# ylsung/vl-merging

Hardware: AMD Instinct MI355X
Metric: VL samples/sec (fwd+bwd) base_vl 384^2 at 1/2/4/8 GPUs; merge GB/s vs HBM peak (higher is better)
Workload: dtype bf16

## Files before the change

include/vlm_hip.h:

```cpp
#ifndef VLM_HIP_H
#define VLM_HIP_H
#include <stddef.h>
#include <stdint.h>

#ifdef __cplusplus
extern "C" {
#endif

#define VLM_OK 0
#define VLM_ERR_ARG (-1)
#define VLM_ERR_LAUNCH (-2)
#define VLM_ERR_WORKSPACE (-3)
#define VLM_ERR_UNSUPPORTED (-4)

#define VLM_ABI_VERSION 11
int vlm_abi_version(void);
int vlm_device_cus(void);
int vlm_set_cu_budget(int cus);
int vlm_debug_occupy(int workgroups, int threads, int lds_bytes, int microseconds, void* stream);

#define VLM_MERGE_LERP 0
#define VLM_MERGE_TASKVEC 1
#define VLM_MERGE_MEAN 2
#define VLM_MERGE_MAX_SRC 4
// ... 258 lines not shown

typedef struct {
  void* dst;
  const void* base;
  const void* src[VLM_MERGE_MAX_SRC];
  void* coef_out;
  double w[VLM_MERGE_MAX_SRC];
  uint64_t n_elem;
  uint32_t row_len;
  int32_t n_src;
  float lam;
  uint32_t reserved;
} vlm_sphere_job_t;

typedef struct {
  uint64_t n_jobs, n_chunks, n_tiles;
  uint64_t jobs_off;
  uint64_t chunks_off;
  uint64_t tiles_off;
  uint64_t first_off;
  uint64_t records_off;
  uint64_t results_off;
} vlm_sphere_header_t;

typedef struct {
  double sq[VLM_MERGE_MAX_SRC];
  double dot[6];
  double coef64[VLM_MERGE_MAX_SRC];
  double rho;
  double resid;
  float coef32[VLM_MERGE_MAX_SRC];
  uint32_t status;
  uint32_t reserved;
  uint64_t rows_linear;
  uint64_t rows_zero;
  double resid_max;
} vlm_sphere_result_t;

size_t vlm_sphere_plan_bytes(int n_jobs, uint64_t total_elems);
int vlm_sphere_plan_upload(const vlm_sphere_job_t* jobs_host, int n_jobs, void* workspace, size_t workspace_bytes, void* stream);
int vlm_sphere_run(void* workspace, void* stream);

#define VLM_TALL_CONSENSUS 0
#define VLM_TALL_RESTORE 1

typedef struct {
  void* dst;
  const void* base;
  const void* src[VLM_MERGE_MAX_SRC];
  void* mask[VLM_MERGE_MAX_SRC];
  uint64_t n_elem;
  int32_t n_src;
  int32_t op;
  int32_t k;
  float tall_lambda;
  float lam;
  uint32_t reserved;
} vlm_tall_job_t;

typedef struct {
  uint64_t n_jobs, n_chunks;
  uint64_t jobs_off;
  uint64_t chunks_off;
  uint64_t counters_off;
} vlm_tall_header_t;
#define VLM_TALL_COUNTERS (VLM_MERGE_MAX_SRC + 2)

size_t vlm_tall_plan_bytes(int n_jobs, uint64_t total_elems);
int vlm_tall_plan_upload(const vlm_tall_job_t* jobs_host, int n_jobs, void* workspace, size_t workspace_bytes, void* stream);
int vlm_tall_run(void* workspace, void* stream);

#define VLM_EMR_MERGE 0
#define VLM_EMR_RESTORE 1

typedef struct {
  void* dst;
  const void* base;
  const void* src[VLM_MERGE_MAX_SRC];
  void* mask[VLM_MERGE_MAX_SRC];
  uint64_t n_elem;
  int32_t n_src;
  int32_t op;
  float lam;
  float rescale;
} vlm_emr_job_t;

typedef struct {
  uint64_t n_jobs, n_chunks;
  uint64_t jobs_off;
  uint64_t chunks_off;
  uint64_t first_off;
  uint64_t records_off;
  uint64_t results_off;
} vlm_emr_header_t;
#define VLM_EMR_SUMS (3 * VLM_MERGE_MAX_SRC + 2)

typedef struct {
  double abs_sum[VLM_MERGE_MAX_SRC];
  double uni_sum[VLM_MERGE_MAX_SRC];
  uint64_t kept[VLM_MERGE_MAX_SRC];
  uint64_t zero;
  uint64_t conflict;
  float rescale[VLM_MERGE_MAX_SRC];
} vlm_emr_result_t;

size_t vlm_emr_plan_bytes(int n_jobs, uint64_t total_elems);
int vlm_emr_plan_upload(const vlm_emr_job_t* jobs_host, int n_jobs, void* workspace, size_t workspace_bytes, void* stream);
int vlm_emr_run(void* workspace, void* stream);

#define VLM_ACT_NONE 0
#define VLM_ACT_GELU 1
#define VLM_ACT_GELU_BWD 2
#define VLM_ACT_GELU_DERIV 3
#define VLM_ACT_MUL_AUX 4

typedef struct {
  const float* bias;
  const float* col_scale;
  const float* row_scale;
  const float* residual;
  int64_t ld_res;
  void* aux;
  int64_t ld_aux;
  int32_t act;
  float alpha;
  int32_t accumulate;
  int32_t reserved;
  float* col_sum;
  float* col_sum_ws;
  float* splitk_ws;
  uint64_t splitk_ws_bytes;
} vlm_epilogue_t;

int vlm_gemm_bf16(int ta, int tb, int M, int N, int K, const void* A, int lda, const void* B, int ldb, void* C,
                  int ldc, int c_is_f32, const vlm_epilogue_t* epi, void* stream);
int vlm_gemm_bf16_live(int ta, int tb, int M, int N, int K, const void* A, int lda, const void* B, int ldb, void* C,
                       int ldc, int c_is_f32, const vlm_epilogue_t* epi, const float* row_live, void* stream);
#define VLM_GEMM_MAX_GROUPS 4
typedef struct {
  int32_t row0, rows;
  const void* B;
  int32_t ldb;
  int32_t reserved;
  const float* bias;
  float* col_sum;
  float* col_sum_ws;
} vlm_gemm_group_t;
int vlm_gemm_bf16_grouped(int n_groups, const vlm_gemm_group_t* groups, int N, int K, const void* A, int lda, void* C,
                          int ldc, int c_is_f32, const vlm_epilogue_t* epi, void* stream);
typedef struct {
  int32_t row0, rows;
  float* C;
  int32_t accumulate;
  int32_t reserved;
} vlm_wgrad_group_t;
int vlm_gemm_wgrad_grouped(int n_groups, const vlm_wgrad_group_t* groups, int M, int N, const void* A, int lda,
                           const void* B, int ldb, int ldc, float* splitk_ws, uint64_t splitk_ws_bytes, void* stream);
typedef struct {
  const void* dy;
  int32_t ld_dy, M;
  const void* x;
  int32_t ld_x, N;
  float* dW;
  int32_t ldc, accumulate;
} vlm_wgrad_problem_t;
int vlm_gemm_wgrad_batch(int n, const vlm_wgrad_problem_t* problems, int T, float* splitk_ws, uint64_t splitk_ws_bytes,
                         void* stream);
int vlm_gemm_set_big_tile_mode(int mode);

int vlm_layernorm_fwd(const float* x, int ldx, int M, int D, const float* gamma, const float* beta, float eps,
                      void* y, int ldy, int y_is_f32, float* stats, void* stream);
#define VLM_ROW_WS_BYTES(D) ((size_t)1536 * 2 * (size_t)(D) * sizeof(float))
int vlm_layernorm_bwd(const void* dy, int lddy, int dy_is_f32, const float* x, int ldx, const float* stats,
                      const float* gamma, int M, int D, const float* dres, int lddres, float* dx, int lddx,
                      float* dgamma, float* dbeta, float* workspace, size_t workspace_bytes, int* deferred_blocks,
                      void* stream);
typedef struct {
  const void* y;
  int32_t ldy;
  const float* gamma;
  const float* row_scale;
  void* dy;
  int32_t lddy;
  float* dgamma;
  float* dbias;
  float* workspace;
  size_t workspace_bytes;
} vlm_layerscale_t;
int vlm_layernorm_bwd_scale(const void* dy, int lddy, int dy_is_f32, const float* x, int ldx, const float* stats,
                            const float* gamma, int M, int D, const float* dres, int lddres, float* dx, int lddx,
                            float* dgamma, float* dbeta, float* workspace, size_t workspace_bytes,
                            const vlm_layerscale_t* scale, int* deferred_blocks, void* stream);
#define VLM_MAX_FOLD_JOBS 16
typedef struct {
  const float* partials;
  int32_t nblocks;
  int32_t D;
  float* out0;
  float* out1;
} vlm_fold_job_t;
int vlm_colreduce_batch(const vlm_fold_job_t* jobs_host, int n_jobs, void* stream);
int vlm_layerscale_bwd(const float* dx, int lddx, const void* y_bf16, int ldy, const float* gamma,
                       const float* row_scale, int M, int D, void* dy_bf16, int lddy, float* dgamma, float* dbias,
                       float* workspace, size_t workspace_bytes, int* deferred_blocks, void* stream);
#define VLM_MAX_LAYERSCALE_JOBS 32
typedef struct {
  const float* weight;
  const float* gamma;
  const float* bias;
  void* shadow;
  float* bias_out;
  float* raw_w;
  float* raw_b;
  float* dweight;
  float* dbias;
  float* dgamma;
  int32_t N, K;
} vlm_layerscale_job_t;
int vlm_layerscale_fold(const vlm_layerscale_job_t* jobs_host, int n_jobs, void* stream);
int vlm_layerscale_finish(const vlm_layerscale_job_t* jobs_host, int n_jobs, void* stream);
int vlm_colsum_bf16(const void* a, int lda, int M, int N, float* out, void* stream);

int vlm_cross_entropy_fwd(const void* logits_bf16, int ld, int rows, int V, const int64_t* labels, int64_t ignore_index,
                          float* loss_rows, float* lse, void* stream);
int vlm_cross_entropy_bwd(const void* logits_bf16, int ld, int rows, int V, const int64_t* labels, int64_t ignore_index,
                          const float* lse, const float* scale_dev, void* dlogits_bf16, int ld_d, void* stream);

int vlm_l2norm_fwd(const void* x, int x_is_bf16, int ld, int rows, int D, float* y, float* inv_norm, void* stream);
int vlm_l2norm_bwd(const float* g, const float* y, const float* inv_norm, int rows, int D, void* dx, int dx_is_bf16, int ld, void* stream);
size_t vlm_contrastive_ws_floats(int n);
int vlm_contrastive(const float* all_img, const float* all_txt, int n, int B, int D, const float* log_scale, float* logits, float* out3,
                    float* d_img, float* d_txt, float* ws, void* stream);
int vlm_small_cross_entropy(const void* logits, int is_bf16, int ld, int rows, int V, const int64_t* labels, float* loss, float* dlogits,
                            void* stream);
int vlm_cross_entropy_reduce(const float* loss_rows, const int64_t* labels, int rows, int V, int64_t ignore_index, float* out2, void* stream);
int vlm_scale_by_scalar(const float* const* in, float* const* out, const int* n, int count, const float* scalar_dev, void* stream);

int vlm_text_rows_fwd(const int64_t* ids, int n, const float* word, int ld_word, const float* add0, const float* gamma, const float* beta,
                      float eps, const float* u, float p, float scale, const float* add1, float* out, int ld_out, float* stats, int D,
                      void* stream);
size_t vlm_text_rows_bwd_ws_floats(int D);
int vlm_text_rows_bwd(const float* g, int ld_g, const int64_t* ids, int n, const float* word, int ld_word, const float* add0,
                      const float* gamma, const float* stats, const float* u, float p, float scale, int D, float* d_word,
                      int64_t padding_idx, float* d_add1, float* d_beta, float* d_gamma, float* d_add0, float* ws, void* stream);
int vlm_image_rows_prep(const float* conv_bias, const float* type_row, const float* cls, int D, float* out2, void* stream);
int vlm_image_lead_rows(float* x, int ld_x, int B, int rows, int D, const float* lead, void* stream);
size_t vlm_image_rows_bwd_ws_floats(int D);
int vlm_image_rows_bwd(const float* g, int ld_g, int B, int rows, int D, void* g16, float* d_bias, float* d_type_row, float* d_cls, float* ws,
                       void* stream);
int vlm_tanh_fwd(const void* x_bf16, int ld_x, int M, int N, float* y, void* stream);
int vlm_act_bwd(const void* g, int g_is_f32, int ld_g, const void* saved, int ld_saved, int mode, int M, int N, int Np, void* dy_bf16,
                void* stream);
int vlm_colsum_small(const void* a_bf16, int lda, int M, int N, float* out, void* stream);
int vlm_sample_negatives(const float* sim_a, int a_row_stride, int a_col_stride, const float* sim_b, int b_row_stride, int b_col_stride, int B,
                         int n, const float* u, int64_t* idx, void* stream);
int vlm_weighted_sum(const float* const* terms, const float* weights, int count, float* out, void* stream);

typedef struct {
  const void* g;
  int g_is_f32;
  int ld;
  int first_row, row_step, count;
} vlm_scatter_src_t;
int vlm_scatter_rows(void* dx, int dx_is_f32, int ld_dx, int R, int D, const vlm_scatter_src_t* src, int n_src, void* stream);

int vlm_adamw_step(float* p, float* g, float* m, float* v, void* p_bf16, uint64_t n, float lr, float beta1,
                   float beta2, float eps, float weight_decay, float step_size, float grad_scale, int zero_grad,
                   void* stream);
int vlm_cast_f32_bf16(const float* src, void* dst_bf16, uint64_t n, void* stream);
int vlm_embedding_bwd(const float* gy, int ld, const int64_t* ids, int64_t n, int D, int64_t padding_idx, float* dW, int ld_w,
                      int64_t vocab, void* stream);
typedef struct {
  uint64_t src;
  uint64_t dst;
  int32_t rows, cols;
  int32_t tile_row, tile_col;
} vlm_transpose_tile_t;
int vlm_transpose_bf16_tiles(const vlm_transpose_tile_t* tiles_dev, int n_tiles, void* stream);

int vlm_droppath_rows(const float* u, float keep, int B, int n0, int n1, int base0, int base1, float* out, void* stream);
int vlm_droppath_sites(const float* u0, const float* u1, const float* keep, int n_sites, int B, int n0, int n1, int base0,
                       int base1, int rows, float* out, void* stream);
int vlm_patch_im2col(const float* image, void* patches_bf16, int B, int H, int W, int P, int lead_rows, void* stream);
int vlm_accumulate_f32_f64(const float* src, double* dst_f64, uint64_t n, void* stream);
int vlm_gram_f64(const void* x, int ldx, int M, int D, int x_is_f32, double* gram, void* stream);
int vlm_gemm_f64(int ta, int tb, int M, int N, int K, double alpha, const void* A, int lda, int a_is_f32, const double* B,
                 int ldb, double beta, double* C, int ldc, void* stream);
int vlm_scale_gram_f64(const double* src, double* dst, int n, double alpha, int accumulate, void* stream);
int vlm_cholesky_f64(double* A, int n, int* status, void* stream);
int vlm_solve_spd_right_f64(const double* chol, int n, double* rhs, int ld, int rows, void* stream);
int vlm_gemm_f64_batched(int ta, int tb, int M, int N, int K, double alpha, const void* const* A_list, int lda, int a_is_f32,
                         const double* const* B_list, int ldb, double beta, double* const* C_list, int ldc, int count, void* stream);
int vlm_cholesky_f64_batched(double* const* A_list, int count, int n, int* status, void* stream);
int vlm_solve_spd_right_f64_batched(double* const* chol_list, int n, double* const* rhs_list, int ld, int rows, int count, void* stream);

#define VLM_ISO_HEAD 64
#define VLM_ISO_MAX_STEPS 40
#define VLM_ISO_PHASE_NUCLEAR 1
#define VLM_ISO_PHASE_APPLY 2
int vlm_iso_parts(int m, int n);
int vlm_iso_delta(const float* const* c_list, const float* const* src_list, int S, int m, int n, double* const* work_list,
                  double* partials, int count, void* stream);
int vlm_iso_gram(double* const* work_list, int rows, int cols, int first, double c, double* const* Z_list, int count, void* stream);
int vlm_iso_step(double* const* work_list, int rows, int cols, int first, double p, double q, int k, double* partials, int count,
                 void* stream);
int vlm_iso_finish(double* const* work_list, const float* const* c_list, float* const* dst_list, int m, int n, double lam,
                   double* partials, int count, int phases, void* stream);

#define VLM_WUDI_HEAD 16
int vlm_wudi_parts(int m, int n);
size_t vlm_wudi_work_doubles(int m, int n);
size_t vlm_wudi_state_offset(int m, int n, int iters);
int vlm_wudi_prepare(const float* const* c_list, const float* const* src_list, int S, int m, int n, double* const* work_list,
                     double* partials, int count, void* stream);
int vlm_wudi_step(double* const* work_list, int m, int n, int t, double step, double bc2s, double beta1, double beta2, double eps,
                  double* partials, int count, void* stream);
int vlm_wudi_finish(double* const* work_list, const float* const* c_list, float* const* dst_list, int S, int m, int n, int iters,
                    double lam, double* partials, int count, void* stream);

#define VLM_SVD_HEAD 64
#define VLM_SVD_MAX_SWEEPS 30
size_t vlm_svd_work_doubles(int p, int q);
int vlm_svd_steps(int p);
int vlm_svd_reset(double* const* work_list, int p, int q, int count, void* stream);
int vlm_svd_sweep(double* const* work_list, int p, int q, int sweep, int count, void* stream);
int vlm_svd_finish(double* const* work_list, int p, int q, double floor_rel, int count, void* stream);
int vlm_tsv_delta(const float* const* c_list, const float* const* src_list, int m, int n, double* const* work_list, int count,
                  void* stream);
int vlm_tsv_gather(const double* const* src_work_list, int S, int p, int q, int k, int side, double* const* dst_work_list,
                   double* const* scat_list, int count, void* stream);
int vlm_tsv_apply(const double* const* pu_list, const double* const* pv_list, const double* const* scat_list,
                  const float* const* c_list, float* const* dst_list, double* const* t_list, int m, int n, int kS, double lam, int count,
                  void* stream);

#define VLM_ATTN_JOINT 0
#define VLM_ATTN_SEPARATE 1

typedef struct {
  const void* qkv;
  int32_t ld_qkv;
  int32_t H;
  int32_t total_rows;
  int32_t R;
  const float* bias_t;
  const int16_t* rel_index;
  const int16_t* rel_index_t;
  int32_t ld_index;
  int32_t index_rows;
  int32_t ld_index_t;
  int32_t index_t_rows;
  int32_t head_row0;
  int32_t mode;
  const uint8_t* keep0;
  const uint8_t* keep1;
  int32_t B, n0, n1, base0, base1, pos1;
  float scale;
  int32_t q_keep0;
  const void* bias_dense;
  const void* bias_dense_t;
  int32_t dense_tiles;
  int32_t q_keep1;
} vlm_attn_desc_t;

int vlm_attention_qkeep_served(const vlm_attn_desc_t* d, int with_dbias);

size_t vlm_bias_dense_bytes(int n0, int n1, int pos1, int mode);
int vlm_bias_dense(const float* bias_t, int n_cols, int R, const int16_t* index, int ld_index, int n0, int n1, int pos1,
                   int mode, int k_major, void* out_f16, void* stream);

int vlm_attention_fwd(const vlm_attn_desc_t* d, void* out_bf16, int ld_out, float* lse, void* stream);
typedef struct {
  float* dq[2];
  float* dv[2];
} vlm_attn_colsum_t;

size_t vlm_attention_bwd_ws_floats(const vlm_attn_desc_t* d, int with_dbias);
int vlm_attention_bwd(const vlm_attn_desc_t* d, const void* out_bf16, int ld_out, const void* dout_bf16, int ld_dout,
                      const float* lse, float* delta_ws, size_t ws_floats, void* dqkv_bf16, int ld_dqkv, float* dbias_t,
                      const vlm_attn_colsum_t* colsum, void* stream);
int vlm_attention_bwd_live(const vlm_attn_desc_t* d, const void* out_bf16, int ld_out, const void* dout_bf16, int ld_dout,
                           const float* lse, float* delta_ws, size_t ws_floats, void* dqkv_bf16, int ld_dqkv, float* dbias_t,
                           const vlm_attn_colsum_t* colsum, const float* row_live, void* stream);

#ifdef __cplusplus
}
#endif
#endif
```

vl-merging_amd/_lib.py:

```python
import ctypes
import os

_HERE = os.path.dirname(os.path.abspath(__file__))
LIB_PATH = os.environ.get("VLM_LIB_PATH") or os.path.join(_HERE, "lib", "libvlm_hip.so")
_lib = None

c_void_p = ctypes.c_void_p
c_int = ctypes.c_int
c_float = ctypes.c_float
c_size_t = ctypes.c_size_t
c_u64 = ctypes.c_uint64

MERGE_LERP, MERGE_TASKVEC, MERGE_MEAN = 0, 1, 2
MERGE_MAX_SRC = 4


class MergeJob(ctypes.Structure):
    _fields_ = [
        ("dst", c_void_p),
        ("base", c_void_p),
        ("src", c_void_p * MERGE_MAX_SRC),
        ("ratio", c_float * MERGE_MAX_SRC),
        ("n_src", ctypes.c_int32),
        ("mode", ctypes.c_int32),
# ... 146 lines not shown

class PairStatsJob(ctypes.Structure):
    _fields_ = [
        ("base", c_void_p),
        ("src", c_void_p * MERGE_MAX_SRC),
        ("n_elem", c_u64),
        ("tkey", ctypes.c_uint32 * MERGE_MAX_SRC),
        ("n_src", ctypes.c_int32),
        ("reserved", ctypes.c_int32),
    ]


class PairStatsHeader(ctypes.Structure):
    _fields_ = [(n, c_u64) for n in ("n_jobs", "n_chunks", "jobs_off", "chunks_off", "first_off", "records_off", "results_off")]


class PairStatsResult(ctypes.Structure):
    _fields_ = ([("sq", ctypes.c_double * MERGE_MAX_SRC)]
                + [(n, ctypes.c_double * PAIRSTATS_PAIRS) for n in ("dot", "dist2", "ssd", "tssd")]
                + [("nnz", c_u64 * MERGE_MAX_SRC)]
                + [(n, c_u64 * PAIRSTATS_PAIRS) for n in ("live", "conflict", "tlive", "tconflict")])


STOCK_SUMS = MERGE_MAX_SRC + PAIRSTATS_PAIRS


class StockJob(ctypes.Structure):
    _fields_ = [
        ("dst", c_void_p),
        ("base", c_void_p),
        ("src", c_void_p * MERGE_MAX_SRC),
        ("n_elem", c_u64),
        ("n_src", ctypes.c_int32),
        ("reserved", ctypes.c_int32),
    ]


class StockHeader(ctypes.Structure):
    _fields_ = list(PairStatsHeader._fields_)


class StockResult(ctypes.Structure):
    _fields_ = [("sq", ctypes.c_double * MERGE_MAX_SRC), ("dot", ctypes.c_double * PAIRSTATS_PAIRS),
                ("cos_pair", ctypes.c_double * PAIRSTATS_PAIRS), ("cos", ctypes.c_double), ("t", ctypes.c_double),
                ("scale", c_float), ("reserved", ctypes.c_uint32)]


EMR_MERGE, EMR_RESTORE = 0, 1
EMR_SUMS = 3 * MERGE_MAX_SRC + 2


class EmrJob(ctypes.Structure):
    _fields_ = [
        ("dst", c_void_p),
        ("base", c_void_p),
        ("src", c_void_p * MERGE_MAX_SRC),
        ("mask", c_void_p * MERGE_MAX_SRC),
        ("n_elem", c_u64),
        ("n_src", ctypes.c_int32),
        ("op", ctypes.c_int32),
        ("lam", c_float),
        ("rescale", c_float),
    ]


class EmrHeader(ctypes.Structure):
    _fields_ = list(PairStatsHeader._fields_)


class EmrResult(ctypes.Structure):
    _fields_ = [("abs_sum", ctypes.c_double * MERGE_MAX_SRC), ("uni_sum", ctypes.c_double * MERGE_MAX_SRC),
                ("kept", c_u64 * MERGE_MAX_SRC), ("zero", c_u64), ("conflict", c_u64), ("rescale", c_float * MERGE_MAX_SRC)]


SCE_COUNTERS = 3


class SceJob(ctypes.Structure):
    _fields_ = [
        ("dst", c_void_p),
        ("base", c_void_p),
        ("src", c_void_p * MERGE_MAX_SRC),
        ("k", c_u64),
        ("n_elem", c_u64),
        ("n_src", ctypes.c_int32),
        ("lam", c_float),
    ]


class SceHeader(ctypes.Structure):
    _fields_ = list(TiesHeader._fields_) + [(n, c_u64) for n in ("first_off", "records_off")]


class SceResult(ctypes.Structure):
    _fields_ = [("key", ctypes.c_uint32), ("reserved", ctypes.c_uint32), ("rank", c_u64), ("sq", ctypes.c_double * MERGE_MAX_SRC),
                ("tot", ctypes.c_double), ("w", c_float * MERGE_MAX_SRC)]


SPHERE_OK, SPHERE_LINEAR, SPHERE_ZERO = 0, 1, 2
SPHERE_ITERS = 24


class SphereJob(ctypes.Structure):
    _fields_ = [
        ("dst", c_void_p),
        ("base", c_void_p),
        ("src", c_void_p * MERGE_MAX_SRC),
        ("coef_out", c_void_p),
        ("w", ctypes.c_double * MERGE_MAX_SRC),
        ("n_elem", c_u64),
        ("row_len", ctypes.c_uint32),
        ("n_src", ctypes.c_int32),
        ("lam", c_float),
        ("reserved", ctypes.c_uint32),
    ]


class SphereHeader(ctypes.Structure):
    _fields_ = [(n, c_u64) for n in ("n_jobs", "n_chunks", "n_tiles", "jobs_off", "chunks_off", "tiles_off", "first_off",
                                     "records_off", "results_off")]


class SphereResult(ctypes.Structure):
    _fields_ = [("sq", ctypes.c_double * MERGE_MAX_SRC), ("dot", ctypes.c_double * PAIRSTATS_PAIRS),
                ("coef64", ctypes.c_double * MERGE_MAX_SRC), ("rho", ctypes.c_double), ("resid", ctypes.c_double),
                ("coef32", c_float * MERGE_MAX_SRC), ("status", ctypes.c_uint32), ("reserved", ctypes.c_uint32),
                ("rows_linear", c_u64), ("rows_zero", c_u64), ("resid_max", ctypes.c_double)]


class ScatterSrc(ctypes.Structure):
    _fields_ = [("g", c_void_p), ("g_is_f32", ctypes.c_int32), ("ld", ctypes.c_int32), ("first_row", ctypes.c_int32),
                ("row_step", ctypes.c_int32), ("count", ctypes.c_int32)]


class Epilogue(ctypes.Structure):
    _fields_ = [
        ("bias", c_void_p), ("col_scale", c_void_p), ("row_scale", c_void_p), ("residual", c_void_p),
        ("ld_res", ctypes.c_int64), ("aux", c_void_p), ("ld_aux", ctypes.c_int64), ("act", ctypes.c_int32),
        ("alpha", c_float), ("accumulate", ctypes.c_int32), ("reserved", ctypes.c_int32), ("col_sum", c_void_p),
        ("col_sum_ws", c_void_p), ("splitk_ws", c_void_p), ("splitk_ws_bytes", ctypes.c_uint64),
    ]


GEMM_MAX_GROUPS = 4


class GemmGroup(ctypes.Structure):
    _fields_ = [("row0", ctypes.c_int32), ("rows", ctypes.c_int32), ("B", c_void_p), ("ldb", ctypes.c_int32),
                ("reserved", ctypes.c_int32), ("bias", c_void_p), ("col_sum", c_void_p), ("col_sum_ws", c_void_p)]


class WgradGroup(ctypes.Structure):
    _fields_ = [("row0", ctypes.c_int32), ("rows", ctypes.c_int32), ("C", c_void_p), ("accumulate", ctypes.c_int32),
                ("reserved", ctypes.c_int32)]


class WgradProblem(ctypes.Structure):
    _fields_ = [("dy", c_void_p), ("ld_dy", ctypes.c_int32), ("M", ctypes.c_int32), ("x", c_void_p), ("ld_x", ctypes.c_int32),
                ("N", ctypes.c_int32), ("dW", c_void_p), ("ldc", ctypes.c_int32), ("accumulate", ctypes.c_int32)]


class FoldJob(ctypes.Structure):
    _fields_ = [("partials", c_void_p), ("nblocks", ctypes.c_int32), ("D", ctypes.c_int32), ("out0", c_void_p),
                ("out1", c_void_p)]


class LayerScale(ctypes.Structure):
    _fields_ = [("y", c_void_p), ("ldy", ctypes.c_int32), ("gamma", c_void_p), ("row_scale", c_void_p), ("dy", c_void_p),
                ("lddy", ctypes.c_int32), ("dgamma", c_void_p), ("dbias", c_void_p), ("workspace", c_void_p),
                ("workspace_bytes", c_size_t)]


class AttnColsum(ctypes.Structure):
    _fields_ = [("dq", c_void_p * 2), ("dv", c_void_p * 2)]


ACT_NONE, ACT_GELU, ACT_GELU_BWD, ACT_GELU_DERIV, ACT_MUL_AUX = 0, 1, 2, 3, 4
ATTN_JOINT, ATTN_SEPARATE = 0, 1


class AttnDesc(ctypes.Structure):
    _fields_ = [
        ("qkv", c_void_p), ("ld_qkv", ctypes.c_int32), ("H", ctypes.c_int32), ("total_rows", ctypes.c_int32),
        ("R", ctypes.c_int32), ("bias_t", c_void_p), ("rel_index", c_void_p), ("rel_index_t", c_void_p),
        ("ld_index", ctypes.c_int32), ("index_rows", ctypes.c_int32), ("ld_index_t", ctypes.c_int32),
        ("index_t_rows", ctypes.c_int32), ("head_row0", ctypes.c_int32), ("mode", ctypes.c_int32),
        ("keep0", c_void_p), ("keep1", c_void_p),
        ("B", ctypes.c_int32), ("n0", ctypes.c_int32), ("n1", ctypes.c_int32), ("base0", ctypes.c_int32),
        ("base1", ctypes.c_int32), ("pos1", ctypes.c_int32), ("scale", c_float), ("q_keep0", ctypes.c_int32),
        ("bias_dense", c_void_p), ("bias_dense_t", c_void_p), ("dense_tiles", ctypes.c_int32), ("q_keep1", ctypes.c_int32),
    ]


class LayerScaleJob(ctypes.Structure):
    _fields_ = [("weight", c_void_p), ("gamma", c_void_p), ("bias", c_void_p), ("shadow", c_void_p), ("bias_out", c_void_p),
                ("raw_w", c_void_p), ("raw_b", c_void_p), ("dweight", c_void_p), ("dbias", c_void_p), ("dgamma", c_void_p),
                ("N", ctypes.c_int32), ("K", ctypes.c_int32)]


MAX_LAYERSCALE_JOBS = 32


class VlmError(RuntimeError):
    pass


_ERR = {-1: "VLM_ERR_ARG", -2: "VLM_ERR_LAUNCH", -3: "VLM_ERR_WORKSPACE", -4: "VLM_ERR_UNSUPPORTED"}

SIGNATURES = {
    "vlm_abi_version": (c_int, []),
    "vlm_device_cus": (c_int, []),
    "vlm_set_cu_budget": (c_int, [c_int]),
    "vlm_debug_occupy": (c_int, [c_int, c_int, c_int, c_int, c_void_p]),
    "vlm_layerscale_fold": (c_int, [ctypes.POINTER(LayerScaleJob), c_int, c_void_p]),
    "vlm_layerscale_finish": (c_int, [ctypes.POINTER(LayerScaleJob), c_int, c_void_p]),
    "vlm_merge_plan_bytes": (c_size_t, [c_int, c_u64]),
    "vlm_merge_plan_upload": (c_int, [ctypes.POINTER(MergeJob), c_int, c_void_p, c_size_t, c_void_p]),
    "vlm_merge_run": (c_int, [c_void_p, c_void_p]),
    "vlm_ties_plan_bytes": (c_size_t, [c_int, c_u64]),
    "vlm_ties_plan_upload": (c_int, [ctypes.POINTER(TiesJob), c_int, c_void_p, c_size_t, c_void_p]),
    "vlm_ties_run": (c_int, [c_void_p, c_void_p]),
    "vlm_dare_plan_bytes": (c_size_t, [c_int, c_u64]),
    "vlm_dare_plan_upload": (c_int, [ctypes.POINTER(DareJob), c_int, c_void_p, c_size_t, c_void_p]),
    "vlm_dare_run": (c_int, [c_void_p, c_void_p]),
    "vlm_band_plan_bytes": (c_size_t, [c_int, c_u64]),
    "vlm_band_plan_upload": (c_int, [ctypes.POINTER(BandJob), c_int, c_void_p, c_size_t, c_void_p]),
    "vlm_band_run": (c_int, [c_void_p, c_void_p]),
    "vlm_della_plan_bytes": (c_size_t, [c_int, c_u64]),
    "vlm_della_plan_upload": (c_int, [ctypes.POINTER(DellaJob), c_int, c_void_p, c_size_t, c_void_p]),
    "vlm_della_run": (c_int, [c_void_p, c_void_p]),
    "vlm_pairstats_plan_bytes": (c_size_t, [c_int, c_u64]),
    "vlm_pairstats_plan_upload": (c_int, [ctypes.POINTER(PairStatsJob), c_int, c_void_p, c_size_t, c_void_p]),
    "vlm_pairstats_run": (c_int, [c_void_p, c_void_p]),
    "vlm_stock_plan_bytes": (c_size_t, [c_int, c_u64]),
    "vlm_stock_plan_upload": (c_int, [ctypes.POINTER(StockJob), c_int, c_void_p, c_size_t, c_void_p]),
    "vlm_stock_run": (c_int, [c_void_p, c_void_p]),
    "vlm_sce_plan_bytes": (c_size_t, [c_int, c_u64]),
    "vlm_sce_plan_upload": (c_int, [ctypes.POINTER(SceJob), c_int, c_void_p, c_size_t, c_void_p]),
    "vlm_sce_run": (c_int, [c_void_p, c_void_p]),
    "vlm_sphere_plan_bytes": (c_size_t, [c_int, c_u64]),
    "vlm_sphere_plan_upload": (c_int, [ctypes.POINTER(SphereJob), c_int, c_void_p, c_size_t, c_void_p]),
    "vlm_sphere_run": (c_int, [c_void_p, c_void_p]),
    "vlm_tall_plan_bytes": (c_size_t, [c_int, c_u64]),
    "vlm_tall_plan_upload": (c_int, [ctypes.POINTER(TallJob), c_int, c_void_p, c_size_t, c_void_p]),
    "vlm_tall_run": (c_int, [c_void_p, c_void_p]),
    "vlm_emr_plan_bytes": (c_size_t, [c_int, c_u64]),
    "vlm_emr_plan_upload": (c_int, [ctypes.POINTER(EmrJob), c_int, c_void_p, c_size_t, c_void_p]),
    "vlm_emr_run": (c_int, [c_void_p, c_void_p]),
    "vlm_gemm_bf16": (c_int, [c_int, c_int, c_int, c_int, c_int, c_void_p, c_int, c_void_p, c_int, c_void_p, c_int,
                              c_int, ctypes.POINTER(Epilogue), c_void_p]),
    "vlm_gemm_bf16_live": (c_int, [c_int, c_int, c_int, c_int, c_int, c_void_p, c_int, c_void_p, c_int, c_void_p, c_int,
                                   c_int, ctypes.POINTER(Epilogue), c_void_p, c_void_p]),
    "vlm_gemm_bf16_grouped": (c_int, [c_int, ctypes.POINTER(GemmGroup), c_int, c_int, c_void_p, c_int, c_void_p, c_int, c_int,
                                      ctypes.POINTER(Epilogue), c_void_p]),
    "vlm_gemm_wgrad_grouped": (c_int, [c_int, ctypes.POINTER(WgradGroup), c_int, c_int, c_void_p, c_int, c_void_p, c_int, c_int,
                                       c_void_p, c_u64, c_void_p]),
    "vlm_gemm_wgrad_batch": (c_int, [c_int, ctypes.POINTER(WgradProblem), c_int, c_void_p, c_u64, c_void_p]),
    "vlm_attention_fwd": (c_int, [ctypes.POINTER(AttnDesc), c_void_p, c_int, c_void_p, c_void_p]),
    "vlm_attention_bwd_ws_floats": (c_size_t, [ctypes.POINTER(AttnDesc), c_int]),
    "vlm_attention_qkeep_served": (c_int, [ctypes.POINTER(AttnDesc), c_int]),
    "vlm_attention_bwd": (c_int, [ctypes.POINTER(AttnDesc), c_void_p, c_int, c_void_p, c_int, c_void_p, c_void_p, c_size_t,
                                  c_void_p, c_int, c_void_p, c_void_p, c_void_p]),
    "vlm_attention_bwd_live": (c_int, [ctypes.POINTER(AttnDesc), c_void_p, c_int, c_void_p, c_int, c_void_p, c_void_p, c_size_t,
                                       c_void_p, c_int, c_void_p, c_void_p, c_void_p, c_void_p]),
    "vlm_layernorm_fwd": (c_int, [c_void_p, c_int, c_int, c_int, c_void_p, c_void_p, c_float, c_void_p, c_int, c_int,
                                  c_void_p, c_void_p]),
    "vlm_layernorm_bwd": (c_int, [c_void_p, c_int, c_int, c_void_p, c_int, c_void_p, c_void_p, c_int, c_int, c_void_p,
                                  c_int, c_void_p, c_int, c_void_p, c_void_p, c_void_p, c_size_t,
                                  ctypes.POINTER(c_int), c_void_p]),
    "vlm_layernorm_bwd_scale": (c_int, [c_void_p, c_int, c_int, c_void_p, c_int, c_void_p, c_void_p, c_int, c_int, c_void_p,
                                        c_int, c_void_p, c_int, c_void_p, c_void_p, c_void_p, c_size_t,
                                        ctypes.POINTER(LayerScale), ctypes.POINTER(c_int), c_void_p]),
    "vlm_layerscale_bwd": (c_int, [c_void_p, c_int, c_void_p, c_int, c_void_p, c_void_p, c_int, c_int, c_void_p, c_int,
                                   c_void_p, c_void_p, c_void_p, c_size_t, ctypes.POINTER(c_int), c_void_p]),
    "vlm_colreduce_batch": (c_int, [ctypes.POINTER(FoldJob), c_int, c_void_p]),
    "vlm_gemm_set_big_tile_mode": (c_int, [c_int]),
    "vlm_colsum_bf16": (c_int, [c_void_p, c_int, c_int, c_int, c_void_p, c_void_p]),
    "vlm_adamw_step": (c_int, [c_void_p, c_void_p, c_void_p, c_void_p, c_void_p, c_u64, c_float, c_float, c_float,
                               c_float, c_float, c_float, c_float, c_int, c_void_p]),
    "vlm_accumulate_f32_f64": (c_int, [c_void_p, c_void_p, c_u64, c_void_p]),
    "vlm_gram_f64": (c_int, [c_void_p, c_int, c_int, c_int, c_int, c_void_p, c_void_p]),
    "vlm_gemm_f64": (c_int, [c_int, c_int, c_int, c_int, c_int, ctypes.c_double, c_void_p, c_int, c_int, c_void_p, c_int,
                             ctypes.c_double, c_void_p, c_int, c_void_p]),
    "vlm_scale_gram_f64": (c_int, [c_void_p, c_void_p, c_int, ctypes.c_double, c_int, c_void_p]),
    "vlm_cholesky_f64": (c_int, [c_void_p, c_int, c_void_p, c_void_p]),
    "vlm_solve_spd_right_f64": (c_int, [c_void_p, c_int, c_void_p, c_int, c_int, c_void_p]),
    "vlm_gemm_f64_batched": (c_int, [c_int, c_int, c_int, c_int, c_int, ctypes.c_double, ctypes.POINTER(c_void_p), c_int, c_int,
                                     ctypes.POINTER(c_void_p), c_int, ctypes.c_double, ctypes.POINTER(c_void_p), c_int, c_int, c_void_p]),
    "vlm_cholesky_f64_batched": (c_int, [ctypes.POINTER(c_void_p), c_int, c_int, c_void_p, c_void_p]),
    "vlm_solve_spd_right_f64_batched": (c_int, [ctypes.POINTER(c_void_p), c_int, ctypes.POINTER(c_void_p), c_int, c_int, c_int, c_void_p]),
    "vlm_iso_parts": (c_int, [c_int, c_int]),
    "vlm_iso_delta": (c_int, [ctypes.POINTER(c_void_p), ctypes.POINTER(c_void_p), c_int, c_int, c_int, ctypes.POINTER(c_void_p),
                              c_void_p, c_int, c_void_p]),
    "vlm_iso_gram": (c_int, [ctypes.POINTER(c_void_p), c_int, c_int, c_int, ctypes.c_double, ctypes.POINTER(c_void_p), c_int, c_void_p]),
    "vlm_iso_step": (c_int, [ctypes.POINTER(c_void_p), c_int, c_int, c_int, ctypes.c_double, ctypes.c_double, c_int, c_void_p, c_int,
                             c_void_p]),
    "vlm_iso_finish": (c_int, [ctypes.POINTER(c_void_p), ctypes.POINTER(c_void_p), ctypes.POINTER(c_void_p), c_int, c_int,
                               ctypes.c_double, c_void_p, c_int, c_int, c_void_p]),
    "vlm_wudi_parts": (c_int, [c_int, c_int]),
    "vlm_wudi_work_doubles": (ctypes.c_size_t, [c_int, c_int]),
    "vlm_wudi_state_offset": (ctypes.c_size_t, [c_int, c_int, c_int]),
    "vlm_wudi_prepare": (c_int, [ctypes.POINTER(c_void_p), ctypes.POINTER(c_void_p), c_int, c_int, c_int, ctypes.POINTER(c_void_p),
                                 c_void_p, c_int, c_void_p]),
    "vlm_wudi_step": (c_int, [ctypes.POINTER(c_void_p), c_int, c_int, c_int, ctypes.c_double, ctypes.c_double, ctypes.c_double,
                              ctypes.c_double, ctypes.c_double, c_void_p, c_int, c_void_p]),
    "vlm_wudi_finish": (c_int, [ctypes.POINTER(c_void_p), ctypes.POINTER(c_void_p), ctypes.POINTER(c_void_p), c_int, c_int, c_int, c_int,
                                ctypes.c_double, c_void_p, c_int, c_void_p]),
    "vlm_svd_work_doubles": (ctypes.c_size_t, [c_int, c_int]),
    "vlm_svd_steps": (c_int, [c_int]),
    "vlm_svd_reset": (c_int, [ctypes.POINTER(c_void_p), c_int, c_int, c_int, c_void_p]),
    "vlm_svd_sweep": (c_int, [ctypes.POINTER(c_void_p), c_int, c_int, c_int, c_int, c_void_p]),
    "vlm_svd_finish": (c_int, [ctypes.POINTER(c_void_p), c_int, c_int, ctypes.c_double, c_int, c_void_p]),
    "vlm_tsv_delta": (c_int, [ctypes.POINTER(c_void_p), ctypes.POINTER(c_void_p), c_int, c_int, ctypes.POINTER(c_void_p), c_int, c_void_p]),
    "vlm_tsv_gather": (c_int, [ctypes.POINTER(c_void_p), c_int, c_int, c_int, c_int, c_int, ctypes.POINTER(c_void_p),
                               ctypes.POINTER(c_void_p), c_int, c_void_p]),
    "vlm_tsv_apply": (c_int, [ctypes.POINTER(c_void_p), ctypes.POINTER(c_void_p), ctypes.POINTER(c_void_p), ctypes.POINTER(c_void_p),
                              ctypes.POINTER(c_void_p), ctypes.POINTER(c_void_p), c_int, c_int, c_int, ctypes.c_double, c_int, c_void_p]),
    "vlm_cross_entropy_fwd": (c_int, [c_void_p, c_int, c_int, c_int, c_void_p, ctypes.c_int64, c_void_p, c_void_p, c_void_p]),
    "vlm_cross_entropy_bwd": (c_int, [c_void_p, c_int, c_int, c_int, c_void_p, ctypes.c_int64, c_void_p, c_void_p, c_void_p, c_int,
                                      c_void_p]),
    "vlm_l2norm_fwd": (c_int, [c_void_p, c_int, c_int, c_int, c_int, c_void_p, c_void_p, c_void_p]),
    "vlm_l2norm_bwd": (c_int, [c_void_p, c_void_p, c_void_p, c_int, c_int, c_void_p, c_int, c_int, c_void_p]),
    "vlm_contrastive_ws_floats": (c_size_t, [c_int]),
    "vlm_contrastive": (c_int, [c_void_p, c_void_p, c_int, c_int, c_int, c_void_p, c_void_p, c_void_p, c_void_p, c_void_p, c_void_p,
                                c_void_p]),
    "vlm_small_cross_entropy": (c_int, [c_void_p, c_int, c_int, c_int, c_int, c_void_p, c_void_p, c_void_p, c_void_p]),
    "vlm_cross_entropy_reduce": (c_int, [c_void_p, c_void_p, c_int, c_int, ctypes.c_int64, c_void_p, c_void_p]),
    "vlm_scale_by_scalar": (c_int, [ctypes.POINTER(c_void_p), ctypes.POINTER(c_void_p), ctypes.POINTER(c_int), c_int, c_void_p, c_void_p]),
    "vlm_text_rows_fwd": (c_int, [c_void_p, c_int, c_void_p, c_int, c_void_p, c_void_p, c_void_p, c_float, c_void_p, c_float, c_float,
                                  c_void_p, c_void_p, c_int, c_void_p, c_int, c_void_p]),
    "vlm_text_rows_bwd_ws_floats": (c_size_t, [c_int]),
    "vlm_text_rows_bwd": (c_int, [c_void_p, c_int, c_void_p, c_int, c_void_p, c_int, c_void_p, c_void_p, c_void_p, c_void_p, c_float, c_float,
                                  c_int, c_void_p, ctypes.c_int64, c_void_p, c_void_p, c_void_p, c_void_p, c_void_p, c_void_p]),
    "vlm_image_rows_prep": (c_int, [c_void_p, c_void_p, c_void_p, c_int, c_void_p, c_void_p]),
    "vlm_image_lead_rows": (c_int, [c_void_p, c_int, c_int, c_int, c_int, c_void_p, c_void_p]),
    "vlm_image_rows_bwd_ws_floats": (c_size_t, [c_int]),
    "vlm_image_rows_bwd": (c_int, [c_void_p, c_int, c_int, c_int, c_int, c_void_p, c_void_p, c_void_p, c_void_p, c_void_p, c_void_p]),
    "vlm_tanh_fwd": (c_int, [c_void_p, c_int, c_int, c_int, c_void_p, c_void_p]),
    "vlm_act_bwd": (c_int, [c_void_p, c_int, c_int, c_void_p, c_int, c_int, c_int, c_int, c_int, c_void_p, c_void_p]),
    "vlm_colsum_small": (c_int, [c_void_p, c_int, c_int, c_int, c_void_p, c_void_p]),
    "vlm_sample_negatives": (c_int, [c_void_p, c_int, c_int, c_void_p, c_int, c_int, c_int, c_int, c_void_p, c_void_p, c_void_p]),
    "vlm_weighted_sum": (c_int, [ctypes.POINTER(c_void_p), ctypes.POINTER(c_float), c_int, c_void_p, c_void_p]),
    "vlm_scatter_rows": (c_int, [c_void_p, c_int, c_int, c_int, c_int, c_void_p, c_int, c_void_p]),
    "vlm_cast_f32_bf16": (c_int, [c_void_p, c_void_p, c_u64, c_void_p]),
    "vlm_embedding_bwd": (c_int, [c_void_p, c_int, c_void_p, ctypes.c_int64, c_int, ctypes.c_int64, c_void_p, c_int,
                                  ctypes.c_int64, c_void_p]),
    "vlm_bias_dense_bytes": (c_size_t, [c_int, c_int, c_int, c_int]),
    "vlm_bias_dense": (c_int, [c_void_p, c_int, c_int, c_void_p, c_int, c_int, c_int, c_int, c_int, c_int, c_void_p,
                               c_void_p]),
    "vlm_transpose_bf16_tiles": (c_int, [c_void_p, c_int, c_void_p]),
    "vlm_droppath_sites": (c_int, [c_void_p, c_void_p, c_void_p, c_int, c_int, c_int, c_int, c_int, c_int, c_int, c_void_p,
                                   c_void_p]),
    "vlm_droppath_rows": (c_int, [c_void_p, c_float, c_int, c_int, c_int, c_int, c_int, c_void_p, c_void_p]),
    "vlm_patch_im2col": (c_int, [c_void_p, c_void_p, c_int, c_int, c_int, c_int, c_int, c_void_p]),
}


def get_lib():
    global _lib
    if _lib is None:
        if not os.path.exists(LIB_PATH):
            raise VlmError(
                f"{LIB_PATH} is missing: build it with `python -c 'import __graft_entry__ as g; g.build()'` "
                "(hipcc --offload-arch=gfx950).  There is no CPU fallback for the hot path.")
        import torch
        lib = ctypes.CDLL(LIB_PATH)
        for name, (res, args) in SIGNATURES.items():
            fn = getattr(lib, name)
            fn.restype = res
            fn.argtypes = args
        _lib = lib
    return _lib


def check(rc, what):
    if rc != 0:
        raise VlmError(f"{what} failed: {_ERR.get(rc, rc)}")


def stream_ptr():
    import torch
    return c_void_p(torch.cuda.current_stream().cuda_stream)


def ptr(t):
    return c_void_p(t.data_ptr()) if t is not None else c_void_p(0)


def require_cuda(*tensors):
    for t in tensors:
        if t is not None and not t.is_cuda:
            raise VlmError("vl_merging_amd ops run on the GPU only (tensor on %s); there is no CPU path" % t.device)
```

vl-merging_amd/csrc/elementwise.hip:

```cpp
#include "vlm_common.h"

#define EW_THREADS 256
#ifndef EW_NT
#define EW_NT true
#endif

static int ew_grid(size_t n_vec) {
  int cus = vlm_device_cus();
  if (cus <= 0) cus = 256;
  size_t want = (n_vec + EW_THREADS - 1) / EW_THREADS;
  size_t cap = (size_t)cus * 8;
  if (want < 1) want = 1;
  return (int)(want < cap ? want : cap);
}

__global__ __launch_bounds__(EW_THREADS) void adamw_kernel(float* __restrict__ p, float* __restrict__ g,
                                                           float* __restrict__ m, float* __restrict__ v,
                                                           bf16_t* __restrict__ pb, size_t n4, float lr, float b1,
                                                           float b2, float eps, float wd, float step_size,
                                                           float grad_scale, int zero_grad) {
  for (size_t i = (size_t)blockIdx.x * EW_THREADS + threadIdx.x; i < n4; i += (size_t)gridDim.x * EW_THREADS) {
    f32x4 pp = reinterpret_cast<f32x4*>(p)[i];
    f32x4 gg = EW_NT ? __builtin_nontemporal_load(reinterpret_cast<f32x4*>(g) + i) : reinterpret_cast<f32x4*>(g)[i];
    f32x4 mm = EW_NT ? __builtin_nontemporal_load(reinterpret_cast<f32x4*>(m) + i) : reinterpret_cast<f32x4*>(m)[i];
    f32x4 vv = EW_NT ? __builtin_nontemporal_load(reinterpret_cast<f32x4*>(v) + i) : reinterpret_cast<f32x4*>(v)[i];
#pragma unroll
    for (int r = 0; r < 4; ++r) {
      const float gr = gg[r] * grad_scale;
      mm[r] = b1 * mm[r] + (1.0f - b1) * gr;
      vv[r] = b2 * vv[r] + (1.0f - b2) * gr * gr;
      const float denom = sqrtf(vv[r]) + eps;
      float x = pp[r] - step_size * (mm[r] / denom);
      if (wd != 0.0f) x = x - lr * wd * x;
      pp[r] = x;
    }
    reinterpret_cast<f32x4*>(p)[i] = pp;
    if (EW_NT) {
      __builtin_nontemporal_store(mm, reinterpret_cast<f32x4*>(m) + i);
      __builtin_nontemporal_store(vv, reinterpret_cast<f32x4*>(v) + i);
    } else {
      reinterpret_cast<f32x4*>(m)[i] = mm;
      reinterpret_cast<f32x4*>(v)[i] = vv;
    }
    if (zero_grad) reinterpret_cast<f32x4*>(g)[i] = (f32x4){0.f, 0.f, 0.f, 0.f};
    if (pb) {
      bf16x4 h = {(bf16_t)pp[0], (bf16_t)pp[1], (bf16_t)pp[2], (bf16_t)pp[3]};
      reinterpret_cast<bf16x4*>(pb)[i] = h;
    }
  }
}

__global__ __launch_bounds__(EW_THREADS) void cast_kernel(const float* __restrict__ src, bf16_t* __restrict__ dst,
                                                          size_t n4) {
  for (size_t i = (size_t)blockIdx.x * EW_THREADS + threadIdx.x; i < n4; i += (size_t)gridDim.x * EW_THREADS) {
    const f32x4 s = reinterpret_cast<const f32x4*>(src)[i];
    bf16x4 h = {(bf16_t)s[0], (bf16_t)s[1], (bf16_t)s[2], (bf16_t)s[3]};
    reinterpret_cast<bf16x4*>(dst)[i] = h;
  }
}

__global__ __launch_bounds__(EW_THREADS) void im2col_kernel(const float* __restrict__ img, bf16_t* __restrict__ out,
                                                            int B, int H, int W, int P, int lead) {
  const int gh = H / P, gw = W / P;
  const int K = 3 * P * P;
  const int k8 = K / 8;
  const int rows = lead + gh * gw;
  const size_t total = (size_t)B * rows * k8;
  for (size_t i = (size_t)blockIdx.x * EW_THREADS + threadIdx.x; i < total; i += (size_t)gridDim.x * EW_THREADS) {
    const int kk = (int)(i % k8) * 8;
    const size_t rr = i / k8;
    const int r = (int)(rr % rows);
    const int b = (int)(rr / rows);
    bf16x8 h;
    if (r < lead) {
#pragma unroll
      for (int e = 0; e < 8; ++e) h[e] = (bf16_t)0.0f;
    } else {
      const int pidx = r - lead;
      const int py = pidx / gw, px = pidx % gw;
      const int c = kk / (P * P), ij = kk % (P * P);
      const int ii = ij / P, jj = ij % P;
      const float* s = img + (((size_t)b * 3 + c) * H + (py * P + ii)) * W + px * P + jj;
      const f32x4 a = *reinterpret_cast<const f32x4*>(s);
      const f32x4 c2 = *reinterpret_cast<const f32x4*>(s + 4);
      h = (bf16x8){(bf16_t)a[0], (bf16_t)a[1], (bf16_t)a[2], (bf16_t)a[3],
                   (bf16_t)c2[0], (bf16_t)c2[1], (bf16_t)c2[2], (bf16_t)c2[3]};
    }
    *reinterpret_cast<bf16x8*>(out + rr * K + kk) = h;
  }
}

__global__ __launch_bounds__(EW_THREADS) void acc_f64_kernel(const float* __restrict__ src, double* __restrict__ dst,
                                                             size_t n4) {
  for (size_t i = (size_t)blockIdx.x * EW_THREADS + threadIdx.x; i < n4; i += (size_t)gridDim.x * EW_THREADS) {
    const f32x4 s = reinterpret_cast<const f32x4*>(src)[i];
    double* d = dst + 4 * i;
    d[0] += (double)s[0];
    d[1] += (double)s[1];
    d[2] += (double)s[2];
    d[3] += (double)s[3];
  }
}

extern "C" int vlm_accumulate_f32_f64(const float* src, double* dst, uint64_t n, void* stream) {
  if (n == 0) return VLM_OK;
  if (!src || !dst || (n & 3) || ((uintptr_t)src & 15) || ((uintptr_t)dst & 31)) return VLM_ERR_ARG;
  const size_t n4 = n >> 2;
  hipLaunchKernelGGL(acc_f64_kernel, dim3(ew_grid(n4)), dim3(EW_THREADS), 0, (hipStream_t)stream, src, dst, n4);
  VLM_CHECK_LAUNCH();
  return VLM_OK;
}

extern "C" int vlm_adamw_step(float* p, float* g, float* m, float* v, void* p_bf16, uint64_t n, float lr,
                              float beta1, float beta2, float eps, float weight_decay, float step_size,
                              float grad_scale, int zero_grad, void* stream) {
  if (n == 0) return VLM_OK;
  if (!p || !g || !m || !v || (n & 3)) return VLM_ERR_ARG;
  if (((uintptr_t)p | (uintptr_t)g | (uintptr_t)m | (uintptr_t)v) & 15) return VLM_ERR_ARG;
  if (p_bf16 && ((uintptr_t)p_bf16 & 7)) return VLM_ERR_ARG;
  const size_t n4 = n >> 2;
  hipLaunchKernelGGL(adamw_kernel, dim3(ew_grid(n4)), dim3(EW_THREADS), 0, (hipStream_t)stream, p, g, m, v,
                     (bf16_t*)p_bf16, n4, lr, beta1, beta2, eps, weight_decay, step_size, grad_scale, zero_grad);
  VLM_CHECK_LAUNCH();
  return VLM_OK;
}

extern "C" int vlm_cast_f32_bf16(const float* src, void* dst, uint64_t n, void* stream) {
  if (n == 0) return VLM_OK;
  if (!src || !dst || (n & 3) || ((uintptr_t)src & 15) || ((uintptr_t)dst & 7)) return VLM_ERR_ARG;
  const size_t n4 = n >> 2;
  hipLaunchKernelGGL(cast_kernel, dim3(ew_grid(n4)), dim3(EW_THREADS), 0, (hipStream_t)stream, src, (bf16_t*)dst, n4);
  VLM_CHECK_LAUNCH();
  return VLM_OK;
}

__global__ __launch_bounds__(EW_THREADS) void embedding_bwd_kernel(const float* __restrict__ gy, int ld, const int64_t* __restrict__ ids,
                                                                   int64_t n, int D, int64_t pad, float* __restrict__ dW, int ld_w,
                                                                   int64_t vocab) {
  const int lane = threadIdx.x & 63, wave = threadIdx.x >> 6;
  for (int64_t t = (int64_t)blockIdx.x * (EW_THREADS / 64) + wave; t < n; t += (int64_t)gridDim.x * (EW_THREADS / 64)) {
    const int64_t id = ids[t];
    if (id == pad || id < 0 || id >= vocab) continue;
    const float* src = gy + t * ld;
    float* dst = dW + id * ld_w;
    for (int c = lane; c < D; c += 64) atomicAdd(dst + c, src[c]);
  }
}

extern "C" int vlm_embedding_bwd(const float* gy, int ld, const int64_t* ids, int64_t n, int D, int64_t padding_idx, float* dW,
                                 int ld_w, int64_t vocab, void* stream) {
  if (n == 0 || D == 0) return VLM_OK;
  if (!gy || !ids || !dW || n < 0 || D < 0 || ld < D || ld_w < D || vocab <= 0) return VLM_ERR_ARG;
  int64_t blocks = (n + (EW_THREADS / 64) - 1) / (EW_THREADS / 64);
  if (blocks > 4096) blocks = 4096;
  hipLaunchKernelGGL(embedding_bwd_kernel, dim3((unsigned)blocks), dim3(EW_THREADS), 0, (hipStream_t)stream, gy, ld, ids, n, D,
                     padding_idx, dW, ld_w, vocab);
  VLM_CHECK_LAUNCH();
  return VLM_OK;
}

__global__ __launch_bounds__(EW_THREADS) void droppath_rows_kernel(const float* __restrict__ u, float keep, float inv_keep,
                                                                   int B, int n0, int n1, int base0, int base1,
                                                                   float* __restrict__ out) {
  const int nt = B * n0, total = nt + B * n1;
  for (int i = blockIdx.x * EW_THREADS + threadIdx.x; i < total; i += gridDim.x * EW_THREADS) {
    int b, row;
    if (i < nt) {
      b = i / n0;
      row = base0 + i;
    } else {
      const int j = i - nt;
      b = j / n1;
      row = base1 + j;
    }
    out[row] = u[b] < keep ? inv_keep : 0.0f;
  }
}

extern "C" int vlm_droppath_rows(const float* u, float keep, int B, int n0, int n1, int base0, int base1, float* out,
                                 void* stream) {
  if (B <= 0 || n0 + n1 <= 0) return VLM_OK;
  if (!u || !out || n0 < 0 || n1 < 0 || base0 < 0 || base1 < 0 || !(keep > 0.0f) || keep > 1.0f) return VLM_ERR_ARG;
  const size_t total = (size_t)B * (n0 + n1);
  hipLaunchKernelGGL(droppath_rows_kernel, dim3(ew_grid(total)), dim3(EW_THREADS), 0, (hipStream_t)stream, u, keep,
                     1.0f / keep, B, n0, n1, base0, base1, out);
  VLM_CHECK_LAUNCH();
  return VLM_OK;
}

__global__ __launch_bounds__(EW_THREADS) void droppath_sites_kernel(const float* __restrict__ u0, const float* __restrict__ u1,
                                                                    const float* __restrict__ keep, int B, int n0, int n1,
                                                                    int base0, int base1, int rows, float* __restrict__ out) {
  const int site = blockIdx.y;
  const float kp = keep[site], inv = 1.0f / kp;
  const float* ua = u0 + (size_t)site * B;
  const float* ub = (u1 ? u1 : u0) + (size_t)site * B;
  float* o = out + (size_t)site * rows;
  const int nt = B * n0, total = nt + B * n1;
  for (int i = blockIdx.x * EW_THREADS + threadIdx.x; i < total; i += gridDim.x * EW_THREADS) {
    if (i < nt) {
      o[base0 + i] = ua[i / n0] < kp ? inv : 0.0f;
    } else {
      const int j = i - nt;
      o[base1 + j] = ub[j / n1] < kp ? inv : 0.0f;
    }
  }
}

extern "C" int vlm_droppath_sites(const float* u0, const float* u1, const float* keep, int n_sites, int B, int n0, int n1,
                                  int base0, int base1, int rows, float* out, void* stream) {
  if (n_sites <= 0 || B <= 0 || n0 + n1 <= 0) return VLM_OK;
  if (!u0 || !keep || !out || n0 < 0 || n1 < 0 || base0 < 0 || base1 < 0 || rows < base0 + B * n0 || rows < base1 + B * n1)
    return VLM_ERR_ARG;
  const size_t total = (size_t)B * (n0 + n1);
  int gx = (int)((total + EW_THREADS - 1) / EW_THREADS);
  if (gx > 64) gx = 64;
  hipLaunchKernelGGL(droppath_sites_kernel, dim3(gx, n_sites), dim3(EW_THREADS), 0, (hipStream_t)stream, u0, u1, keep, B,
                     n0, n1, base0, base1, rows, out);
  VLM_CHECK_LAUNCH();
  return VLM_OK;
}

__global__ __launch_bounds__(256) void transpose_tiles_kernel(const vlm_transpose_tile_t* __restrict__ tiles, int n_tiles) {
  __shared__ bf16_t tile[64][66];
  for (int t = blockIdx.x; t < n_tiles; t += gridDim.x) {
    const vlm_transpose_tile_t j = tiles[t];
    const bf16_t* src = reinterpret_cast<const bf16_t*>(j.src);
    bf16_t* dst = reinterpret_cast<bf16_t*>(j.dst);
    const int r0 = j.tile_row * 64, c0 = j.tile_col * 64;
    const int lr = threadIdx.x >> 2, lc = (threadIdx.x & 3) * 16;
    const bool fast = r0 + 64 <= j.rows && c0 + 64 <= j.cols && (j.cols & 7) == 0 && (j.rows & 7) == 0 &&
                      ((j.src | j.dst) & 15) == 0;
    if (fast) {
      const bf16x8* sp = reinterpret_cast<const bf16x8*>(src + (size_t)(r0 + lr) * j.cols + c0 + lc);
      const bf16x8 v0 = sp[0], v1 = sp[1];
#pragma unroll
      for (int e = 0; e < 8; ++e) {
        tile[lr][lc + e] = v0[e];
        tile[lr][lc + 8 + e] = v1[e];
      }
    } else {
      const int r = r0 + lr;
#pragma unroll
      for (int e = 0; e < 16; ++e) {
        const int c = c0 + lc + e;
        tile[lr][lc + e] = (r < j.rows && c < j.cols) ? src[(size_t)r * j.cols + c] : (bf16_t)0.0f;
      }
    }
    __syncthreads();
    const int c = c0 + lr;
    if (fast) {
      bf16x8 o0, o1;
#pragma unroll
      for (int e = 0; e < 8; ++e) {
        o0[e] = tile[lc + e][lr];
        o1[e] = tile[lc + 8 + e][lr];
      }
      bf16x8* dp = reinterpret_cast<bf16x8*>(dst + (size_t)c * j.rows + r0 + lc);
      dp[0] = o0;
      dp[1] = o1;
    } else if (c < j.cols) {
#pragma unroll
      for (int e = 0; e < 16; ++e) {
        const int r = r0 + lc + e;
        if (r < j.rows) dst[(size_t)c * j.rows + r] = tile[lc + e][lr];
      }
    }
    __syncthreads();
  }
}

extern "C" int vlm_transpose_bf16_tiles(const vlm_transpose_tile_t* tiles_dev, int n_tiles, void* stream) {
  if (n_tiles == 0) return VLM_OK;
  if (!tiles_dev || n_tiles < 0) return VLM_ERR_ARG;
  int cus = vlm_device_cus();
  if (cus <= 0) cus = 256;
  const int grid = n_tiles < cus * 16 ? n_tiles : cus * 16;
  hipLaunchKernelGGL(transpose_tiles_kernel, dim3(grid), dim3(256), 0, (hipStream_t)stream, tiles_dev, n_tiles);
  VLM_CHECK_LAUNCH();
  return VLM_OK;
}

extern "C" int vlm_patch_im2col(const float* image, void* patches, int B, int H, int W, int P, int lead_rows,
                                void* stream) {
  if (B == 0) return VLM_OK;
  if (!image || !patches || B < 0 || P <= 0 || (P & 7) || (H % P) || (W % P) || (W & 3) || lead_rows < 0)
    return VLM_ERR_ARG;
  if (((uintptr_t)image & 15) || ((uintptr_t)patches & 15)) return VLM_ERR_ARG;
  const size_t total = (size_t)B * (lead_rows + (H / P) * (W / P)) * (3 * P * P / 8);
  hipLaunchKernelGGL(im2col_kernel, dim3(ew_grid(total)), dim3(EW_THREADS), 0, (hipStream_t)stream, image,
                     (bf16_t*)patches, B, H, W, P, lead_rows);
  VLM_CHECK_LAUNCH();
  return VLM_OK;
}
```

vl-merging_amd/csrc/gemm.hip:

```cpp
#include "vlm_common.h"
#include "vlm_diag.h"
#include "wgrad_plan.h"
#include <atomic>

#define GEMM_BM 128
#define GEMM_BN 128
#define GEMM_BK 64
#define GEMM_THREADS 256
#define GEMM_TILE_BYTES (GEMM_BM * GEMM_BK * 2)

typedef __attribute__((address_space(3))) s16x4 lds_s16x4;

__device__ __forceinline__ float gelu_cdf(float x, float& ez2) {
  const float t = __builtin_amdgcn_rcpf(fmaf(0.3275911f * 0.70710678118654752440f, fabsf(x), 1.0f));
  ez2 = __builtin_amdgcn_exp2f((x * x) * (-0.5f * 1.4426950408889634f));
  float poly = fmaf(t, 0.5f * 1.061405429f, 0.5f * -1.453152027f);
  poly = fmaf(t, poly, 0.5f * 1.421413741f);
  poly = fmaf(t, poly, 0.5f * -0.284496736f);
  poly = fmaf(t, poly, 0.5f * 0.254829592f);
  const float e = fmaf(-(poly * t), ez2, 0.5f);
  return 0.5f + copysignf(e, x);
}
__device__ __forceinline__ float gelu_erf(float x) {
  float ez2;
  return x * gelu_cdf(x, ez2);
}
__device__ __forceinline__ float gelu_erf_grad(float x) {
  float ez2;
  const float cdf = gelu_cdf(x, ez2);
  return fmaf(x * 0.39894228040143267794f, ez2, cdf);
}
__device__ __forceinline__ float gelu_erf_both(float x, float& deriv) {
  float ez2;
  const float cdf = gelu_cdf(x, ez2);
  deriv = fmaf(x * 0.39894228040143267794f, ez2, cdf);
  return x * cdf;
}
__device__ __forceinline__ float act_bwd_factor(int act, float saved) {
  return act == VLM_ACT_MUL_AUX ? saved : gelu_erf_grad(saved);
}

template <bool KSTRIDED>
__device__ __forceinline__ void stage_load(u32x4 (&r)[4], __amdgpu_buffer_rsrc_t rsrc, uint32_t row0, uint32_t k0,
                                           uint32_t ld, int tid) {
#pragma unroll
  for (int u = 0; u < 4; ++u) {
    const uint32_t p = tid + 256 * u;
    uint32_t off;
    if (!KSTRIDED) {
      const uint32_t row = p >> 3, chunk = p & 7;
      off = ((row0 + row) * ld + k0 + chunk * 8) * 2;
    } else {
      const uint32_t krow = p >> 4, c16 = p & 15;
      off = ((k0 + krow) * ld + row0 + c16 * 8) * 2;
    }
    r[u] = __builtin_amdgcn_raw_buffer_load_b128(rsrc, off, 0, 0);
  }
}

template <bool KSTRIDED>
__device__ __forceinline__ void stage_store(const u32x4 (&r)[4], unsigned char* lds, int tid) {
#pragma unroll
  for (int u = 0; u < 4; ++u) {
    const uint32_t p = tid + 256 * u;
    uint32_t byte;
    if (!KSTRIDED) {
      const uint32_t row = p >> 3, chunk = p & 7;
      byte = row * 128 + ((chunk ^ (row & 7)) << 4);
    } else {
      const uint32_t krow = p >> 4, c16 = p & 15;
      const uint32_t c32 = (c16 >> 1) ^ (krow & 3) ^ (((krow >> 3) & 1) << 2);
      byte = krow * 256 + c32 * 32 + (c16 & 1) * 16;
    }
    *reinterpret_cast<u32x4*>(lds + byte) = r[u];
  }
}

typedef __attribute__((address_space(3))) void lds_void;
__device__ __forceinline__ void stage_dma(__amdgpu_buffer_rsrc_t rsrc, unsigned char* tile, uint32_t row0, uint32_t k0,
                                          uint32_t ld, int wave, int lane) {
#pragma unroll
  for (int u = 0; u < 4; ++u) {
    const int j = wave + 4 * u;
    const uint32_t row = j * 8 + (lane >> 3), chunk = (lane & 7) ^ (row & 7);
    const uint32_t off = ((row0 + row) * ld + k0 + chunk * 8) * 2;
    __builtin_amdgcn_raw_ptr_buffer_load_lds(rsrc, (lds_void*)(tile + j * 1024), 16, off, 0, 0, 0);
  }
}

template <bool KSTRIDED>
__device__ __forceinline__ bf16x8 frag_load(const unsigned char* lds, int xblk , int ksub,
                                            int lane) {
  if (!KSTRIDED) {
    const uint32_t row = xblk * 16 + (lane & 15);
    const uint32_t chunk = ksub * 4 + (lane >> 4);
    const uint32_t byte = row * 128 + ((chunk ^ (row & 7)) << 4);
    return *reinterpret_cast<const bf16x8*>(lds + byte);
  } else {
    const uint32_t g = lane >> 4, q = (lane & 15) >> 2, p = lane & 3;
    const uint32_t row = ksub * 32 + 8 * g + q;
    const uint32_t c32 = ((uint32_t)xblk ^ q ^ ((g & 1) << 2));
    const uint32_t byte = row * 256 + c32 * 32 + 8 * p;
    s16x4 lo = __builtin_amdgcn_ds_read_tr16_b64_v4i16((lds_s16x4*)(lds + byte));
    s16x4 hi = __builtin_amdgcn_ds_read_tr16_b64_v4i16((lds_s16x4*)(lds + byte + 4 * 256));
    s16x8 v = {lo[0], lo[1], lo[2], lo[3], hi[0], hi[1], hi[2], hi[3]};
    return __builtin_bit_cast(bf16x8, v);
  }
}

struct gemm_group_t {
  const void* B;
  const float* bias;
  float* col_sum;
  float* col_sum_ws;
  int ldb, row0, row_end, tile0;
};

struct gemmT_group_t {
  const void* A;
  const void* B;
  int lda, ldb, M, N, tiles_n, ntile;
  int row0, row_end, item0, kps;
  uint32_t ws_base;
};

struct gemm_params_t {
  const void* A;
  const void* B;
  void* C;
  int M, N, K;
  int lda, ldb, ldc;
  vlm_epilogue_t epi;
  int tiles_m, tiles_n;
  int group_m;
  int splits, ksteps_per_split;
  int n_groups;
  gemm_group_t grp[VLM_GEMM_MAX_GROUPS];
  gemmT_group_t grpT[VLM_GEMM_MAX_GROUPS];
  const float* row_live = nullptr;
  VLM_DIAG_GEMM_FIELD
};

__device__ __forceinline__ void lane16_swap(float& x, float& y) {
  asm volatile("s_nop 1\n\tv_permlane16_swap_b32 %0, %1" : "+v"(x), "+v"(y));
}

template <bool OUT_F32, bool LEAN = false>
__device__ __forceinline__ int gemm_epilogue(const gemm_params_t& p, const f32x4 (&acc)[4][4], int mw0, int nw0, int lane,
                                             float* red = nullptr, int red_off = 0) {
  const vlm_epilogue_t& e = p.epi;
  const bool vec_ok = ((p.ldc & 3) == 0) && (!e.aux || (e.ld_aux & 3) == 0) && (!e.residual || (e.ld_res & 3) == 0);
  const bool vec8_ok = vec_ok && (OUT_F32 || (p.ldc & 7) == 0) && (!e.aux || ((e.ld_aux & 7) == 0 && ((uintptr_t)e.aux & 15) == 0)) &&
                       (!e.residual || ((uintptr_t)e.residual & 15) == 0) && (!e.bias || ((uintptr_t)e.bias & 15) == 0) &&
                       (!e.col_scale || ((uintptr_t)e.col_scale & 15) == 0);
  if (vec8_ok && mw0 + 64 <= p.M && nw0 + 64 <= p.N) {
    const bool has_res = e.residual != nullptr, bwd = e.act == VLM_ACT_GELU_BWD || e.act == VLM_ACT_MUL_AUX, accum = OUT_F32 && e.accumulate;
    const int g = lane >> 4;
    const int nl = nw0 + (g & 1) * 16 + (g >> 1) * 8;
    float bia[2][8], gam[2][8], csum[2][8];
#pragma unroll
    for (int jp = 0; jp < 2; ++jp)
#pragma unroll
      for (int r = 0; r < 8; ++r) csum[jp][r] = 0.f;
#define EPI_LOAD_COL_VECTORS()                                                                                          \
  _Pragma("unroll") for (int jp = 0; jp < 2; ++jp) _Pragma("unroll") for (int q = 0; q < 2; ++q) {                    \
    const f32x4 b4 = e.bias ? *reinterpret_cast<const f32x4*>(e.bias + nl + jp * 32 + q * 4) : (f32x4){0.f, 0.f, 0.f, 0.f}; \
    const f32x4 g4 =                                                                                                    \
        e.col_scale ? *reinterpret_cast<const f32x4*>(e.col_scale + nl + jp * 32 + q * 4) : (f32x4){1.f, 1.f, 1.f, 1.f}; \
    _Pragma("unroll") for (int r = 0; r < 4; ++r) {                                                                     \
      bia[jp][q * 4 + r] = b4[r];                                                                                       \
      gam[jp][q * 4 + r] = g4[r];                                                                                       \
    }                                                                                                                   \
  }
    if (!LEAN) { EPI_LOAD_COL_VECTORS() }
#pragma unroll
    for (int hf = 0; hf < 4; ++hf) {
      f32x4 rsd[1][2][2], old[1][2][2];
      bf16x8 hx[1][2];
      float rs[1];
      if (LEAN) { EPI_LOAD_COL_VECTORS() }
#pragma unroll
      for (int ii = 0; ii < 1; ++ii) {
        const size_t m = mw0 + (hf + ii) * 16 + (lane & 15);
        rs[ii] = e.row_scale ? e.row_scale[m] : 1.0f;
#pragma unroll
        for (int jp = 0; jp < 2; ++jp) {
          const int n = nl + jp * 32;
          if (has_res) {
            rsd[ii][jp][0] = *reinterpret_cast<const f32x4*>(e.residual + m * e.ld_res + n);
            rsd[ii][jp][1] = *reinterpret_cast<const f32x4*>(e.residual + m * e.ld_res + n + 4);
          }
          if (bwd) hx[ii][jp] = *reinterpret_cast<const bf16x8*>(reinterpret_cast<const bf16_t*>(e.aux) + m * e.ld_aux + n);
          if (accum) {
            old[ii][jp][0] = *reinterpret_cast<const f32x4*>(reinterpret_cast<const float*>(p.C) + m * p.ldc + n);
            old[ii][jp][1] = *reinterpret_cast<const f32x4*>(reinterpret_cast<const float*>(p.C) + m * p.ldc + n + 4);
          }
        }
      }
#pragma unroll
      for (int ii = 0; ii < 1; ++ii) {
        const size_t m = mw0 + (hf + ii) * 16 + (lane & 15);
#pragma unroll
        for (int jp = 0; jp < 2; ++jp) {
          const int n = nl + jp * 32;
          float v[8];
#pragma unroll
          for (int r = 0; r < 4; ++r) {
            float x = acc[hf + ii][2 * jp][r] * e.alpha, y = acc[hf + ii][2 * jp + 1][r] * e.alpha;
            lane16_swap(x, y);
            v[r] = x;
            v[4 + r] = y;
          }
#pragma unroll
          for (int r = 0; r < 8; ++r) v[r] += bia[jp][r];
          if (bwd) {
#pragma unroll
            for (int r = 0; r < 8; ++r) v[r] *= act_bwd_factor(e.act, (float)hx[ii][jp][r]);
          } else if (e.act == VLM_ACT_GELU_DERIV) {
            bf16x8 h;
#pragma unroll
            for (int r = 0; r < 8; ++r) {
              float dg;
              v[r] = gelu_erf_both(v[r], dg);
              h[r] = (bf16_t)dg;
            }
            *reinterpret_cast<bf16x8*>(reinterpret_cast<bf16_t*>(e.aux) + m * e.ld_aux + n) = h;
          } else {
            if (e.aux) {
              bf16x8 h;
#pragma unroll
              for (int r = 0; r < 8; ++r) h[r] = (bf16_t)v[r];
              *reinterpret_cast<bf16x8*>(reinterpret_cast<bf16_t*>(e.aux) + m * e.ld_aux + n) = h;
            }
            if (e.act == VLM_ACT_GELU) {
#pragma unroll
              for (int r = 0; r < 8; ++r) v[r] = gelu_erf(v[r]);
            }
          }
          if (e.col_scale) {
#pragma unroll
            for (int r = 0; r < 8; ++r) v[r] *= gam[jp][r];
          }
          if (e.row_scale) {
#pragma unroll
            for (int r = 0; r < 8; ++r) v[r] *= rs[ii];
          }
          if (has_res) {
#pragma unroll
            for (int r = 0; r < 8; ++r) v[r] += rsd[ii][jp][r >> 2][r & 3];
          }
          if (OUT_F32 && accum) {
#pragma unroll
            for (int r = 0; r < 8; ++r) v[r] += old[ii][jp][r >> 2][r & 3];
          }
          if (!LEAN && e.col_sum) {
#pragma unroll
            for (int r = 0; r < 8; ++r) csum[jp][r] += v[r];
          }
          if (OUT_F32) {
            float* c = reinterpret_cast<float*>(p.C) + m * p.ldc + n;
            *reinterpret_cast<f32x4*>(c) = (f32x4){v[0], v[1], v[2], v[3]};
            *reinterpret_cast<f32x4*>(c + 4) = (f32x4){v[4], v[5], v[6], v[7]};
          } else {
            bf16x8 o;
#pragma unroll
            for (int r = 0; r < 8; ++r) o[r] = (bf16_t)v[r];
            *reinterpret_cast<bf16x8*>(reinterpret_cast<bf16_t*>(p.C) + m * p.ldc + n) = o;
          }
        }
      }
    }
    if (!LEAN && e.col_sum) {
#pragma unroll
      for (int jp = 0; jp < 2; ++jp)
#pragma unroll
        for (int r = 0; r < 8; ++r) {
// ... 554 lines not shown
      acc01[i][j] = (f32x4){0.f, 0.f, 0.f, 0.f};
      acc10[i][j] = (f32x4){0.f, 0.f, 0.f, 0.f};
      acc11[i][j] = (f32x4){0.f, 0.f, 0.f, 0.f};
    }

#define BIG_PIN_ACC()                                                                                   \
  _Pragma("unroll") for (int i = 0; i < 4; ++i) _Pragma("unroll") for (int j = 0; j < 4; ++j) {         \
    asm volatile("" : "+a"(acc00[i][j]), "+a"(acc01[i][j]), "+a"(acc10[i][j]), "+a"(acc11[i][j]));      \
  }
  constexpr bool DEEP = AUX == 2 && !RES;
  constexpr int AHEAD = 6;
  if constexpr (DEEP) { BIG_PIN_ACC() }

  const int nk = p.K / BIG_BK;
  const uint32_t mw0 = m0 + wm * 128, nw0 = n0 + wn * 128;
  unsigned char* const wl = epl + wave * EPIL_WAVE_BYTES;
#define EPIL_SETUP()                                       \
  big_epilogue_t<OUT_F32, RES, AUX> ep(p, wl, mw0, nw0, lane); \
  epil_in_t inA, inB;                                      \
  ep.load_inputs(inA, 0);
  bf16x8 fa0[8], fb0[8], fa1[8], fb1[8];

#define BIG_READ(FA, FB, SA, SB)                                                         \
  _Pragma("unroll") for (int i = 0; i < 8; ++i) {                                        \
    FA[i] = *reinterpret_cast<const bf16x8*>((SA) + rda + i * 1024);                     \
    FB[i] = *reinterpret_cast<const bf16x8*>((SB) + rdb + i * 1024);                     \
  }
#define BIG_MFMA_Q(ACC, FA, FB, I0, J0)                                                                                \
  _Pragma("unroll") for (int i = 0; i < 4; ++i) _Pragma("unroll") for (int j = 0; j < 4; ++j)                         \
      ACC[i][j] = __builtin_amdgcn_mfma_f32_16x16x32_bf16(FB[(J0) + j], FA[(I0) + i], ACC[i][j], 0, 0, 0);
#define BIG_MFMA(FA, FB)        \
  BIG_MFMA_Q(acc00, FA, FB, 0, 0) \
  BIG_MFMA_Q(acc01, FA, FB, 0, 4) \
  BIG_MFMA_Q(acc11, FA, FB, 4, 4) \
  BIG_MFMA_Q(acc10, FA, FB, 4, 0)
  uint32_t wr_off[4];
  {
    const uint32_t slot = (lane & 3) ^ big_swz(lane >> 4);
#pragma unroll
    for (int u = 0; u < 4; ++u) wr_off[u] = ((wave + 4 * u) * 16 + (lane >> 2)) * 64 + slot * 16;
  }
  {
    const uint32_t unswz = (((lane & 3) ^ big_swz(lane >> 4)) - (lane & 3)) * 16;
#pragma unroll
    for (int u = 0; u < 4; ++u) { offa[u] -= unswz; offb[u] -= unswz; }
  }
  u32x4 ra0[4], rb0[4], ra1[4], rb1[4];
#define BIG_GLOAD(RA_, RB_, S)                                                                        \
  _Pragma("unroll") for (int u = 0; u < 4; ++u) {                                                     \
    RA_[u] = __builtin_amdgcn_raw_buffer_load_b128(ra, offa[u], (S) * (BIG_BK * 2), 0);               \
    RB_[u] = __builtin_amdgcn_raw_buffer_load_b128(rb, offb[u], (S) * (BIG_BK * 2), 0);               \
  }
#define BIG_LWRITE(RA_, RB_, SA, SB)                                                                  \
  _Pragma("unroll") for (int u = 0; u < 4; ++u) {                                                     \
    *reinterpret_cast<u32x4*>((SA) + wr_off[u]) = RA_[u];                                             \
    *reinterpret_cast<u32x4*>((SB) + wr_off[u]) = RB_[u];                                             \
  }
#define BIG_STEP(K, GL, WR, RD, FCA, FCB, FNA, FNB, RSA, RSB, BUFA_W, BUFB_W, BUFA_R, BUFB_R)   \
  {                                                                                      \
    if (RD) {                                                                            \
      asm volatile("s_waitcnt lgkmcnt(0)" ::: "memory");                                 \
      __builtin_amdgcn_s_barrier();                                                      \
    }                                                                                    \
    __builtin_amdgcn_sched_barrier(0);                                                   \
    if (WR) { BIG_LWRITE(RSA, RSB, BUFA_W, BUFB_W) }                                     \
    if (GL) { BIG_GLOAD(RSA, RSB, (K) + 4) }                                             \
    if (RD) { BIG_READ(FNA, FNB, BUFA_R, BUFB_R) }                                       \
    BIG_MFMA(FCA, FCB)                                                                   \
    _Pragma("unroll") for (int g = 0; g < 16; ++g) {                                     \
      __builtin_amdgcn_sched_group_barrier(0x008, 2, 0);                                 \
      __builtin_amdgcn_sched_group_barrier(0x100, 1, 0);                                 \
    }                                                                                    \
    _Pragma("unroll") for (int g = 0; g < 8; ++g) {                                      \
      __builtin_amdgcn_sched_group_barrier(0x008, 2, 0);                                 \
      __builtin_amdgcn_sched_group_barrier(0x200, 1, 0);                                 \
      __builtin_amdgcn_sched_group_barrier(0x008, 2, 0);                                 \
      __builtin_amdgcn_sched_group_barrier(0x020, 1, 0);                                 \
    }                                                                                    \
    __builtin_amdgcn_sched_barrier(0);                                                   \
  }

  BIG_GLOAD(ra0, rb0, 0)
  BIG_GLOAD(ra1, rb1, 1)
  if (SKIPS && p.row_live && __builtin_amdgcn_ballot_w64(lv[0] != 0.0f || lv[1] != 0.0f || lv[2] != 0.0f || lv[3] != 0.0f) == 0) {
    int lane_d = lane;
    asm volatile("" : "+v"(lane_d));
    big_epilogue_t<OUT_F32, RES, AUX> ep(p, wl, mw0, nw0, lane_d);
    unsigned char* const wz = wl + (lane_d & 15) * EPIL_PITCH + (lane_d >> 4) * 16;
#pragma unroll
    for (int j = 0; j < 8; ++j) *reinterpret_cast<f32x4*>(wz + 64 * j) = (f32x4){0.f, 0.f, 0.f, 0.f};
#pragma unroll 1
    for (int i = 0; i < 8; ++i) {
      epil_in_t in;
      ep.load_inputs(in, i);
      ep.process(in, i, 0);
    }
    ep.finish(lane_d, (p.epi.col_sum_ws && mw0 + 128 <= (uint32_t)p.M) ? p.epi.col_sum_ws + ((size_t)(tm_ws * 2 + wm) * 2) * p.N : nullptr);
    GEMM_STAMP_END()
    return;
  }
  BIG_LWRITE(ra0, rb0, sA0, sB0)
  BIG_GLOAD(ra0, rb0, 2)
  BIG_LWRITE(ra1, rb1, sA1, sB1)
  BIG_GLOAD(ra1, rb1, 3)
  asm volatile("s_waitcnt lgkmcnt(0)" ::: "memory");
  __builtin_amdgcn_s_barrier();
  BIG_READ(fa0, fb0, sA0, sB0)
  GEMM_STAMP(1)

  int kt = 0;
  for (; kt < nk - 4; kt += 2) {
    BIG_STEP(kt + 0, 1, 1, 1, fa0, fb0, fa1, fb1, ra0, rb0, sA0, sB0, sA1, sB1)
    BIG_STEP(kt + 1, 1, 1, 1, fa1, fb1, fa0, fb0, ra1, rb1, sA1, sB1, sA0, sB0)
  }
#define BIG_TAIL_STEPS()                                                               \
  BIG_STEP(kt + 0, 0, 1, 1, fa0, fb0, fa1, fb1, ra0, rb0, sA0, sB0, sA1, sB1)          \
  BIG_STEP(kt + 1, 0, 1, 1, fa1, fb1, fa0, fb0, ra1, rb1, sA1, sB1, sA0, sB0)          \
  BIG_STEP(kt + 2, 0, 0, 1, fa0, fb0, fa1, fb1, ra0, rb0, sA0, sB0, sA1, sB1)          \
  BIG_STEP(kt + 3, 0, 0, 0, fa1, fb1, fa0, fb0, ra1, rb1, sA1, sB1, sA0, sB0)
  if constexpr (DEEP) {
    BIG_TAIL_STEPS()
    GEMM_STAMP(2)
    big_epilogue_t<OUT_F32, RES, AUX> ep(p, wl, mw0, nw0, lane);
    float* ws_row = (p.epi.col_sum_ws && mw0 + 128 <= (uint32_t)p.M) ? p.epi.col_sum_ws + ((size_t)(tm_ws * 2 + wm) * 2) * p.N : nullptr;
    BIG_EPILOGUE_LOOP_DEEP(AHEAD)
    ep.finish(lane, ws_row);
  } else {
    EPIL_SETUP()
    BIG_TAIL_STEPS()
    GEMM_STAMP(2)
    float* ws_row = (p.epi.col_sum_ws && mw0 + 128 <= (uint32_t)p.M) ? p.epi.col_sum_ws + ((size_t)(tm_ws * 2 + wm) * 2) * p.N : nullptr;
    BIG_EPILOGUE_LOOP()
    ep.finish(lane, ws_row);
  }
  GEMM_STAMP_END()
}

template <bool GROUPED = false>
__global__ __launch_bounds__(GEMM_THREADS, 1) void vlm_gemm_bigT_kernel(const gemm_params_t p) {
  __shared__ __attribute__((aligned(1024))) unsigned char sA0[BIG_OP_BYTES], sA1[BIG_OP_BYTES], sB0[BIG_OP_BYTES], sB1[BIG_OP_BYTES];
  __shared__ __attribute__((aligned(16))) unsigned char epl[4 * EPIL_WAVE_BYTES];
  const int tid = threadIdx.x;
  const int lane = tid & 63;
  const int wave = __builtin_amdgcn_readfirstlane(tid >> 6);
  const int wm = wave >> 1, wn = wave & 1;
  uint32_t ntile = p.tiles_m * p.tiles_n, tiles_n = (uint32_t)p.tiles_n;
  const uint32_t q8 = gridDim.x >> 3, r8 = gridDim.x & 7, xcd = blockIdx.x & 7;
  uint32_t item = (xcd < r8 ? xcd * (q8 + 1) : r8 * (q8 + 1) + (xcd - r8) * q8) + (blockIdx.x >> 3);
  uint32_t k_base = 0, k_end = (uint32_t)p.K, ws_base = 0;
  int nk = p.ksteps_per_split;
  const void *A = p.A, *B = p.B;
  uint32_t lda = (uint32_t)p.lda, ldb = (uint32_t)p.ldb;
  int M = p.M, N = p.N;
  if constexpr (GROUPED) {
    int g = 0;
#pragma unroll
    for (int i = 1; i < VLM_GEMM_MAX_GROUPS; ++i)
      if (i < p.n_groups && item >= (uint32_t)p.grpT[i].item0) g = i;
    const gemmT_group_t G = p.grpT[g];
    item -= (uint32_t)G.item0;
    k_base = (uint32_t)G.row0;
    k_end = (uint32_t)G.row_end;
    nk = G.kps;
    ws_base = G.ws_base;
    A = G.A; B = G.B;
    lda = (uint32_t)G.lda; ldb = (uint32_t)G.ldb;
    M = G.M; N = G.N;
    ntile = (uint32_t)G.ntile; tiles_n = (uint32_t)G.tiles_n;
  }
  const uint32_t split = item / ntile, tile = item - split * ntile;
  const uint32_t tm = tile / tiles_n, tn = tile - tm * tiles_n;
  const uint32_t m0 = tm * BIG_BM, n0 = tn * BIG_BN;
  const uint32_t k_first = k_base + split * (uint32_t)nk * BIG_BK;
  const __amdgpu_buffer_rsrc_t ra =
      __builtin_amdgcn_make_buffer_rsrc(const_cast<void*>(A), 0, (int)((uint64_t)k_end * lda * 2), 0x00020000);
  const __amdgpu_buffer_rsrc_t rb =
      __builtin_amdgcn_make_buffer_rsrc(const_cast<void*>(B), 0, (int)((uint64_t)k_end * ldb * 2), 0x00020000);

  uint32_t offa[4], offb[4], wr_off[4];
#pragma unroll
  for (int u = 0; u < 4; ++u) {
    const uint32_t row = 2 * (wave + 4 * u) + (lane >> 5), c16 = lane & 31;
    offa[u] = ((k_first + row) * lda + m0 + c16 * 8) * 2;
    offb[u] = ((k_first + row) * ldb + n0 + c16 * 8) * 2;
    wr_off[u] = row * 512 + (((c16 >> 1) ^ ((row & 3) | (((row >> 3) & 1) << 2))) << 5) + (c16 & 1) * 16;
  }
  uint32_t rda[8], rdb[8];
  {
    const uint32_t g = lane >> 4, q = (lane & 15) >> 2, pp = lane & 3, sw = q | ((g & 1) << 2);
#pragma unroll
    for (int i = 0; i < 8; ++i) {
      rda[i] = (8 * g + q) * 512 + wm * 256 + ((i ^ sw) << 5) + 8 * pp;
      rdb[i] = (8 * g + q) * 512 + wn * 256 + ((i ^ sw) << 5) + 8 * pp;
    }
  }
  f32x4 acc00[4][4], acc01[4][4], acc10[4][4], acc11[4][4];
#pragma unroll
  for (int i = 0; i < 4; ++i)
#pragma unroll
    for (int j = 0; j < 4; ++j) {
      acc00[i][j] = (f32x4){0.f, 0.f, 0.f, 0.f};
      acc01[i][j] = (f32x4){0.f, 0.f, 0.f, 0.f};
      acc10[i][j] = (f32x4){0.f, 0.f, 0.f, 0.f};
      acc11[i][j] = (f32x4){0.f, 0.f, 0.f, 0.f};
    }
  const uint32_t stepa = BIG_BK * lda * 2, stepb = BIG_BK * ldb * 2;
  bf16x8 fa0[8], fb0[8], fa1[8], fb1[8];
  u32x4 ra0[4], rb0[4], ra1[4], rb1[4];
#define BIGT_TR(PTR) __builtin_amdgcn_ds_read_tr16_b64_v4i16((lds_s16x4*)(PTR))
#define BIGT_READ(FA, FB, SA, SB)                                                                    \
  _Pragma("unroll") for (int i = 0; i < 8; ++i) {                                                    \
    const s16x4 al = BIGT_TR((SA) + rda[i]), ah = BIGT_TR((SA) + rda[i] + 4 * 512);                  \
    const s16x4 bl = BIGT_TR((SB) + rdb[i]), bh = BIGT_TR((SB) + rdb[i] + 4 * 512);                  \
    FA[i] = __builtin_bit_cast(bf16x8, (s16x8){al[0], al[1], al[2], al[3], ah[0], ah[1], ah[2], ah[3]}); \
    FB[i] = __builtin_bit_cast(bf16x8, (s16x8){bl[0], bl[1], bl[2], bl[3], bh[0], bh[1], bh[2], bh[3]}); \
  }
#define BIGT_GLOAD(RA_, RB_, S)                                                                      \
  _Pragma("unroll") for (int u = 0; u < 4; ++u) {                                                    \
    RA_[u] = __builtin_amdgcn_raw_buffer_load_b128(ra, offa[u], (S) * stepa, 0);                     \
    RB_[u] = __builtin_amdgcn_raw_buffer_load_b128(rb, offb[u], (S) * stepb, 0);                     \
  }
#define BIGT_LWRITE(RA_, RB_, SA, SB)                                                                \
  _Pragma("unroll") for (int u = 0; u < 4; ++u) {                                                    \
    *reinterpret_cast<u32x4*>((SA) + wr_off[u]) = RA_[u];                                            \
    *reinterpret_cast<u32x4*>((SB) + wr_off[u]) = RB_[u];                                            \
  }
#define BIGT_STEP(K, GL, WR, RD, FCA, FCB, FNA, FNB, RSA, RSB, BUFA_W, BUFB_W, BUFA_R, BUFB_R)      \
  {                                                                                      \
    if (RD) {                                                                            \
      asm volatile("s_waitcnt lgkmcnt(0)" ::: "memory");                                 \
      __builtin_amdgcn_s_barrier();                                                      \
    }                                                                                    \
    __builtin_amdgcn_sched_barrier(0);                                                   \
    if (WR) { BIGT_LWRITE(RSA, RSB, BUFA_W, BUFB_W) }                                    \
    if (GL) { BIGT_GLOAD(RSA, RSB, (K) + 4) }                                            \
    if (RD) { BIGT_READ(FNA, FNB, BUFA_R, BUFB_R) }                                      \
    BIG_MFMA(FCA, FCB)                                                                   \
    _Pragma("unroll") for (int g = 0; g < 32; ++g) {                                     \
      __builtin_amdgcn_sched_group_barrier(0x008, 1, 0);                                 \
      __builtin_amdgcn_sched_group_barrier(0x100, 1, 0);                                 \
    }                                                                                    \
    _Pragma("unroll") for (int g = 0; g < 8; ++g) {                                      \
      __builtin_amdgcn_sched_group_barrier(0x008, 2, 0);                                 \
      __builtin_amdgcn_sched_group_barrier(0x200, 1, 0);                                 \
      __builtin_amdgcn_sched_group_barrier(0x008, 2, 0);                                 \
      __builtin_amdgcn_sched_group_barrier(0x020, 1, 0);                                 \
    }                                                                                    \
    __builtin_amdgcn_sched_barrier(0);                                                   \
  }
  BIGT_GLOAD(ra0, rb0, 0)
  BIGT_GLOAD(ra1, rb1, 1)
  BIGT_LWRITE(ra0, rb0, sA0, sB0)
  BIGT_GLOAD(ra0, rb0, 2)
  BIGT_LWRITE(ra1, rb1, sA1, sB1)
  BIGT_GLOAD(ra1, rb1, 3)
  asm volatile("s_waitcnt lgkmcnt(0)" ::: "memory");
  __builtin_amdgcn_s_barrier();
  BIGT_READ(fa0, fb0, sA0, sB0)
  int kt = 0;
  for (; kt < nk - 4; kt += 2) {
    BIGT_STEP(kt + 0, 1, 1, 1, fa0, fb0, fa1, fb1, ra0, rb0, sA0, sB0, sA1, sB1)
    BIGT_STEP(kt + 1, 1, 1, 1, fa1, fb1, fa0, fb0, ra1, rb1, sA1, sB1, sA0, sB0)
  }
  BIGT_STEP(kt + 0, 0, 1, 1, fa0, fb0, fa1, fb1, ra0, rb0, sA0, sB0, sA1, sB1)
  BIGT_STEP(kt + 1, 0, 1, 1, fa1, fb1, fa0, fb0, ra1, rb1, sA1, sB1, sA0, sB0)
  BIGT_STEP(kt + 2, 0, 0, 1, fa0, fb0, fa1, fb1, ra0, rb0, sA0, sB0, sA1, sB1)
  BIGT_STEP(kt + 3, 0, 0, 0, fa1, fb1, fa0, fb0, ra1, rb1, sA1, sB1, sA0, sB0)

  gemm_params_t pl = p;
  pl.C = reinterpret_cast<float*>(p.C) + ws_base + (size_t)split * M * N;
  pl.M = M;
  pl.N = N;
  pl.ldc = N;
  const uint32_t mw0 = m0 + wm * 128, nw0 = n0 + wn * 128;
  unsigned char* const wl = epl + wave * EPIL_WAVE_BYTES;
  big_epilogue_t<true, false, 0, 128, 0, true> ep(pl, wl, mw0, nw0, lane);
  epil_in_t inA, inB;
  ep.load_inputs(inA, 0);
  BIG_EPILOGUE_LOOP()
}

__global__ __launch_bounds__(256) void splitk_reduce_kernel(const float* __restrict__ ws, int splits, int M, int N, float* __restrict__ C,
                                                            int ldc, int accumulate) {
  const size_t i = (size_t)blockIdx.x * 256 + threadIdx.x, per = (size_t)M * N / 4;
  if (i >= per) return;
  const size_t e = i * 4, m = e / N, n = e - m * N;
  f32x4 t = accumulate ? *reinterpret_cast<const f32x4*>(C + m * ldc + n) : (f32x4){0.f, 0.f, 0.f, 0.f};
  for (int s = 0; s < splits; ++s) t += *reinterpret_cast<const f32x4*>(ws + (size_t)s * M * N + e);
  *reinterpret_cast<f32x4*>(C + m * ldc + n) = t;
}

struct splitk_groups_t {
  float* C[VLM_GEMM_MAX_GROUPS];
  int M[VLM_GEMM_MAX_GROUPS], N[VLM_GEMM_MAX_GROUPS], ldc[VLM_GEMM_MAX_GROUPS];
  uint32_t ws_base[VLM_GEMM_MAX_GROUPS];
  int splits[VLM_GEMM_MAX_GROUPS], accumulate[VLM_GEMM_MAX_GROUPS];
};
__global__ __launch_bounds__(256) void splitk_reduce_grouped_kernel(const float* __restrict__ ws, const splitk_groups_t g) {
  const int gi = blockIdx.y;
  const int N = g.N[gi], ldc = g.ldc[gi];
  const size_t i = (size_t)blockIdx.x * 256 + threadIdx.x, mn = (size_t)g.M[gi] * N;
  if (i >= mn / 4) return;
  float* const C = g.C[gi];
  const float* const w = ws + g.ws_base[gi];
  const size_t e = i * 4, m = e / N, n = e - m * N;
  f32x4 t = g.accumulate[gi] ? *reinterpret_cast<const f32x4*>(C + m * ldc + n) : (f32x4){0.f, 0.f, 0.f, 0.f};
  for (int s = 0; s < g.splits[gi]; ++s) t += *reinterpret_cast<const f32x4*>(w + (size_t)s * mn + e);
  *reinterpret_cast<f32x4*>(C + m * ldc + n) = t;
}

static int plan_cus() {
  const int cus = vlm_device_cus();
  return cus > 0 ? cus : 256;
}

static bool epi_vec8(const vlm_epilogue_t* e, int ldc, int c_is_f32) {
  const bool v4 = ((ldc & 3) == 0) && (!e->aux || (e->ld_aux & 3) == 0) && (!e->residual || (e->ld_res & 3) == 0);
  return v4 && (c_is_f32 || (ldc & 7) == 0) && (!e->aux || ((e->ld_aux & 7) == 0 && ((uintptr_t)e->aux & 15) == 0)) &&
         (!e->residual || ((uintptr_t)e->residual & 15) == 0) && (!e->bias || ((uintptr_t)e->bias & 15) == 0) &&
         (!e->col_scale || ((uintptr_t)e->col_scale & 15) == 0);
}

static bool epi_off32(const vlm_epilogue_t* e, int M, int lda, int ldc) {
  return (uint64_t)M * ldc * 4 < (1ull << 31) && (!e->residual || (uint64_t)M * e->ld_res * 4 < (1ull << 31)) &&
         (!e->aux || (uint64_t)M * e->ld_aux * 2 < (1ull << 31)) && (uint64_t)M * lda * 2 < (1ull << 31);
}

static int launch_gemm_bigT(gemm_params_t p, const vlm_epilogue_t* epi, hipStream_t stream) {
  if (!epi->splitk_ws || (p.N % BIG_BN) || (p.ldc % 4)) return 1;
  if ((uint64_t)p.M * p.N * 4 >= (1ull << 31)) return 1;
  p.tiles_m = (p.M + BIG_BM - 1) / BIG_BM;
  p.tiles_n = (p.N + BIG_BN - 1) / BIG_BN;
  const int ntile = p.tiles_m * p.tiles_n, nk = (p.K + BIG_BK - 1) / BIG_BK;
  int splits = plan_cus() / ntile;
  if (splits < 1) splits = 1;
  if (splits > nk / 16) splits = nk / 16;
  if (splits < 1) return 1;
  int kps = (nk + splits - 1) / splits;
  kps += kps & 1;
  if (kps < 4) kps = 4;
  splits = (nk + kps - 1) / kps;
  if ((size_t)splits * p.M * p.N * 4 > (size_t)epi->splitk_ws_bytes) return 1;
  p.ksteps_per_split = kps;
  p.splits = splits;
  float* const out = reinterpret_cast<float*>(p.C);
  const int ldc = p.ldc;
  p.C = epi->splitk_ws;
  hipLaunchKernelGGL(vlm_gemm_bigT_kernel<false>, dim3(ntile * splits), dim3(GEMM_THREADS), 0, stream, p);
  VLM_CHECK_LAUNCH();
  const size_t per = (size_t)p.M * p.N / 4;
  hipLaunchKernelGGL(splitk_reduce_kernel, dim3((unsigned)((per + 255) / 256)), dim3(256), 0, stream,
                     reinterpret_cast<const float*>(epi->splitk_ws), splits, p.M, p.N, out, ldc, epi->accumulate);
  VLM_CHECK_LAUNCH();
  return VLM_OK;
}

template <bool OUT_F32, bool RES, int AUX, bool GROUPED = false>
static int launch_gemm_big(gemm_params_t p, hipStream_t stream) {
  if (!GROUPED) p.tiles_m = (p.M + BIG_BM - 1) / BIG_BM;
  p.tiles_n = (p.N + BIG_BN - 1) / BIG_BN;
  p.group_m = p.tiles_n >= 6 ? 4 : 1;
  GEMM_STAMP_ARM(p)
  hipLaunchKernelGGL((vlm_gemm_big_kernel<OUT_F32, RES, AUX, GROUPED>), dim3(p.tiles_m * p.tiles_n), dim3(GEMM_THREADS), 0, stream, p);
  VLM_CHECK_LAUNCH();
  return VLM_OK;
}

template <bool GROUPED = false>
static int launch_gemm_big_variant(const gemm_params_t& p, bool c_is_f32, hipStream_t s) {
  const vlm_epilogue_t& e = p.epi;
  const bool res = e.residual != nullptr;
  const int aux = e.aux ? ((e.act == VLM_ACT_GELU_BWD || e.act == VLM_ACT_MUL_AUX) ? 2 : 1) : 0;
  if (e.row_scale && !res) return 1;
  {
    bool any_cs = e.col_sum != nullptr;
    if (GROUPED)
      for (int g = 0; g < p.n_groups; ++g) any_cs = any_cs || p.grp[g].col_sum != nullptr;
    if (e.alpha != 1.0f || (e.col_scale && !res) || (any_cs && aux != 2)) return 1;
  }
  if (!c_is_f32 && !res) {
    if (aux == 0) return launch_gemm_big<false, false, 0, GROUPED>(p, s);
    if (aux == 1) return launch_gemm_big<false, false, 1, GROUPED>(p, s);
    return launch_gemm_big<false, false, 2, GROUPED>(p, s);
  }
  if (c_is_f32 && aux != 2) {
    if (res && aux) return launch_gemm_big<true, true, 1, GROUPED>(p, s);
    if (res) return launch_gemm_big<true, true, 0, GROUPED>(p, s);
    if (GROUPED) return 1;
    if (aux == 0) return launch_gemm_big<true, false, 0>(p, s);
  }
  return 1;
}

static std::atomic<int> g_big_mode{1};
static int gemm_big_mode() { return g_big_mode.load(std::memory_order_relaxed); }
extern "C" int vlm_gemm_set_big_tile_mode(int mode) {
  if (mode < -1 || mode > 2) return VLM_ERR_ARG;
  g_big_mode.store(mode < 0 ? 1 : mode, std::memory_order_relaxed);
  return VLM_OK;
}


static int gemm_bf16(int ta, int tb, int M, int N, int K, const void* A, int lda, const void* B, int ldb, void* C, int ldc,
                     int c_is_f32, const vlm_epilogue_t* epi, const float* row_live, void* stream) {
  if (M < 0 || N < 0 || K < 0 || !C) return VLM_ERR_ARG;
  if (M == 0 || N == 0) return VLM_OK;
  if (!A || !B || !epi) return VLM_ERR_ARG;
  if ((lda & 7) || (ldb & 7) || ((uintptr_t)A & 15) || ((uintptr_t)B & 15)) return VLM_ERR_ARG;
  if ((!ta || !tb) && (K % GEMM_BK)) return VLM_ERR_UNSUPPORTED;
  if (((ldc & 3) == 0) && ((uintptr_t)C & 15)) return VLM_ERR_ARG;
  if (epi->accumulate && !c_is_f32) return VLM_ERR_ARG;
  if ((epi->act == VLM_ACT_GELU_BWD || epi->act == VLM_ACT_MUL_AUX || epi->act == VLM_ACT_GELU_DERIV) && !epi->aux) return VLM_ERR_ARG;
  if (epi->act < VLM_ACT_NONE || epi->act > VLM_ACT_MUL_AUX) return VLM_ERR_ARG;
  if (epi->col_sum_ws && (!epi->col_sum || (N % GEMM_BN) != 0 || ta)) return VLM_ERR_ARG;
  const uint64_t a_bytes = (uint64_t)(ta ? K : M) * lda * 2, b_bytes = (uint64_t)(tb ? K : N) * ldb * 2;
  if (a_bytes >= (1ull << 31) || b_bytes >= (1ull << 31)) return VLM_ERR_UNSUPPORTED;
  gemm_params_t p;
  p.A = A; p.B = B; p.C = C;
  p.M = M; p.N = N; p.K = K;
  p.lda = lda; p.ldb = ldb; p.ldc = ldc;
  p.epi = *epi;
  p.epi.reserved = epi_vec8(epi, ldc, c_is_f32) ? 1 : 0;
  if (epi->col_sum_ws && !p.epi.reserved) return VLM_ERR_ARG;
  p.tiles_m = (M + GEMM_BM - 1) / GEMM_BM;
  p.tiles_n = (N + GEMM_BN - 1) / GEMM_BN;
  p.splits = 1;
  p.ksteps_per_split = 0;
  p.n_groups = 0;
  p.group_m = p.tiles_n >= 12 ? 8 : 1;
  GEMM_STAMP_ARM(p)
  hipStream_t s = (hipStream_t)stream;
  const int ntile = p.tiles_m * p.tiles_n, nk = (K + GEMM_BK - 1) / GEMM_BK;
  const bool plain_acc = epi->accumulate && c_is_f32 && !epi->bias && !epi->col_scale && !epi->row_scale &&
                         !epi->residual && !epi->aux && !epi->col_sum && epi->act == VLM_ACT_NONE;
  if (gemm_big_mode() > 0 && ta && tb && c_is_f32 && !epi->bias && !epi->col_scale && !epi->row_scale && !epi->residual &&
      !epi->aux && !epi->col_sum && epi->act == VLM_ACT_NONE && K >= 2048) {
    const int rc = launch_gemm_bigT(p, epi, s);
    if (rc <= 0) return rc;
  }
  if (tb && plain_acc && ntile < 512 && nk >= 32) {
    int splits = 2 * plan_cus() / ntile;
    if (splits < 1) splits = 1;
    if (splits > nk / 8) splits = nk / 8;
    if (splits > 1) {
      p.ksteps_per_split = (nk + splits - 1) / splits;
      p.splits = (nk + p.ksteps_per_split - 1) / p.ksteps_per_split;
      p.group_m = p.tiles_n >= 12 ? 1 : 4;
      if (ta) return launch_gemm<true, true, true, true>(p, s);
      return launch_gemm<false, true, true, true>(p, s);
    }
  }
  if (!ta && !tb && (K % (4 * BIG_BK)) == 0 && gemm_big_mode() > 0) {
    const long big_tiles = (long)((M + BIG_BM - 1) / BIG_BM) * ((N + BIG_BN - 1) / BIG_BN);
    const bool ws_ok = (N % BIG_BN) == 0 && p.epi.reserved == 1 && epi_off32(epi, M, lda, ldc) && !epi->accumulate;
    if (ws_ok && (gemm_big_mode() >= 2 || 2 * big_tiles >= plan_cus())) {
      p.row_live = row_live;
      const int rc = launch_gemm_big_variant<>(p, c_is_f32 != 0, s);
      if (rc <= 0) return rc;
      p.row_live = nullptr;
    }
  }
#ifdef GEMM_ONLY_BIG
  return VLM_ERR_UNSUPPORTED;
#endif
  const int key = (ta ? 4 : 0) | (tb ? 2 : 0) | (c_is_f32 ? 1 : 0);
  switch (key) {
    case 0: return launch_gemm<false, false, false, false>(p, s);
    case 1: return launch_gemm<false, false, true, false>(p, s);
    case 2: return launch_gemm<false, true, false, false>(p, s);
    case 3: return launch_gemm<false, true, true, false>(p, s);
    case 4: return launch_gemm<true, false, false, false>(p, s);
    case 5: return launch_gemm<true, false, true, false>(p, s);
    case 6: return launch_gemm<true, true, false, false>(p, s);
    default: return launch_gemm<true, true, true, false>(p, s);
  }
}

extern "C" int vlm_gemm_bf16(int ta, int tb, int M, int N, int K, const void* A, int lda, const void* B, int ldb,
                             void* C, int ldc, int c_is_f32, const vlm_epilogue_t* epi, void* stream) {
  return gemm_bf16(ta, tb, M, N, K, A, lda, B, ldb, C, ldc, c_is_f32, epi, nullptr, stream);
}

extern "C" int vlm_gemm_bf16_live(int ta, int tb, int M, int N, int K, const void* A, int lda, const void* B, int ldb,
                                  void* C, int ldc, int c_is_f32, const vlm_epilogue_t* epi, const float* row_live, void* stream) {
  if (row_live && ((uintptr_t)row_live & 3)) return VLM_ERR_ARG;
  return gemm_bf16(ta, tb, M, N, K, A, lda, B, ldb, C, ldc, c_is_f32, epi, row_live, stream);
}

extern "C" int vlm_gemm_bf16_grouped(int n_groups, const vlm_gemm_group_t* groups, int N, int K, const void* A, int lda, void* C,
                                     int ldc, int c_is_f32, const vlm_epilogue_t* epi, void* stream) {
  if (n_groups < 1 || n_groups > VLM_GEMM_MAX_GROUPS || !groups || N < 0 || K < 0 || !C || !epi) return VLM_ERR_ARG;
  if (epi->bias || epi->col_sum || epi->col_sum_ws || epi->splitk_ws) return VLM_ERR_ARG;
  int prev_end = 0;
  for (int g = 0; g < n_groups; ++g) {
    const vlm_gemm_group_t& G = groups[g];
    if (G.row0 < prev_end || G.rows < 0 || !G.B || (G.col_sum_ws && !G.col_sum)) return VLM_ERR_ARG;
    prev_end = G.row0 + G.rows;
  }
  const int M_total = prev_end;
  if (M_total == 0 || N == 0) return VLM_OK;
  if (!A) return VLM_ERR_ARG;
  hipStream_t s = (hipStream_t)stream;
  bool big = gemm_big_mode() > 0 && (K % (4 * BIG_BK)) == 0 && (N % BIG_BN) == 0 && !epi->accumulate && (lda & 7) == 0 &&
             ((uintptr_t)A & 15) == 0 && ((uintptr_t)C & 15) == 0 && epi_vec8(epi, ldc, c_is_f32) && epi_off32(epi, M_total, lda, ldc);
  gemm_params_t p;
  p.A = A; p.B = nullptr; p.C = C;
  p.M = M_total; p.N = N; p.K = K;
  p.lda = lda; p.ldb = 0; p.ldc = ldc;
  p.epi = *epi;
  p.epi.reserved = 1;
  p.splits = 1;
  p.ksteps_per_split = 0;
  p.n_groups = 0;
  int tiles = 0;
  for (int g = 0; g < n_groups && big; ++g) {
    const vlm_gemm_group_t& G = groups[g];
    if (G.rows == 0) continue;
    if ((G.ldb & 7) || ((uintptr_t)G.B & 15) || (uint64_t)N * G.ldb * 2 >= (1ull << 31) || (G.bias && ((uintptr_t)G.bias & 15))) big = false;
    gemm_group_t& D = p.grp[p.n_groups++];
    D.B = G.B; D.bias = G.bias; D.col_sum = G.col_sum; D.col_sum_ws = G.col_sum_ws;
    D.ldb = G.ldb; D.row0 = G.row0; D.row_end = G.row0 + G.rows; D.tile0 = tiles;
    tiles += (G.rows + BIG_BM - 1) / BIG_BM;
  }
  if (big && p.n_groups >= 1) {
    p.tiles_m = tiles;
    if (gemm_big_mode() >= 2 || 2l * tiles * (N / BIG_BN) >= plan_cus()) {
      const int rc = launch_gemm_big_variant<true>(p, c_is_f32 != 0, s);
      if (rc <= 0) return rc;
    }
  }
  for (int g = 0; g < n_groups; ++g) {
    const vlm_gemm_group_t& G = groups[g];
    if (G.rows == 0) continue;
    vlm_epilogue_t e = *epi;
    const size_t r0 = (size_t)G.row0;
    e.bias = G.bias; e.col_sum = G.col_sum; e.col_sum_ws = G.col_sum_ws;
    if (e.residual) e.residual += r0 * e.ld_res;
    if (e.aux) e.aux = reinterpret_cast<unsigned char*>(e.aux) + r0 * e.ld_aux * 2;
    if (e.row_scale) e.row_scale += r0;
    const int rc = vlm_gemm_bf16(0, 0, G.rows, N, K, reinterpret_cast<const unsigned char*>(A) + r0 * lda * 2, lda, G.B, G.ldb,
                                 reinterpret_cast<unsigned char*>(C) + r0 * ldc * (c_is_f32 ? 4 : 2), ldc, c_is_f32, &e, stream);
    if (rc) return rc;
  }
  return VLM_OK;
}

struct wgradT_problem_t {
  const void* A;
  const void* B;
  int lda, ldb, M, N, row0, row_end;
  float* C;
  int ldc, accumulate;
};
static int launch_gemm_bigT_grouped(int n, const wgradT_problem_t* pr, float* splitk_ws, uint64_t splitk_ws_bytes, hipStream_t s) {
  if (!splitk_ws || ((uintptr_t)splitk_ws & 15) || n < 1 || n > VLM_GEMM_MAX_GROUPS) return 1;
  wgrad_plan_in_t in[VLM_GEMM_MAX_GROUPS];
  for (int g = 0; g < n; ++g) {
    const wgradT_problem_t& P = pr[g];
    if (P.M < 1 || P.N < 1 || (P.N % BIG_BN) || (P.ldc % 4) || P.ldc < P.N || ((uintptr_t)P.C & 15) || ((uintptr_t)P.A & 15) ||
        ((uintptr_t)P.B & 15) || (P.lda & 7) || (P.ldb & 7) || P.lda < P.M || P.ldb < P.N || P.row0 < 0 || P.row_end <= P.row0)
      return 1;
    if ((uint64_t)P.M * P.N * 4 >= (1ull << 31) || (uint64_t)P.row_end * P.lda * 2 >= (1ull << 31) ||
        (uint64_t)P.row_end * P.ldb * 2 >= (1ull << 31))
      return 1;
    in[g] = wgrad_plan_in_t{((P.M + BIG_BM - 1) / BIG_BM) * (P.N / BIG_BN), (P.row_end - P.row0 + BIG_BK - 1) / BIG_BK,
                            (uint64_t)P.M * P.N};
  }
  wgrad_plan_t plan;
  if (wgrad_plan(n, in, plan_cus(), splitk_ws_bytes / 4, &plan)) return 1;
  if (plan.ws_floats >= (1ull << 32)) return 1;
  gemm_params_t p;
  p.A = nullptr; p.B = nullptr; p.C = splitk_ws;
  p.M = 0; p.N = 0; p.K = 0;
  p.lda = 0; p.ldb = 0; p.ldc = 0;
  p.epi = vlm_epilogue_t{};
  p.epi.alpha = 1.0f;
  p.epi.reserved = 1;
  p.tiles_m = 0; p.tiles_n = 0;
  p.group_m = 1;
  p.splits = 1;
  p.ksteps_per_split = 0;
  p.n_groups = n;
  splitk_groups_t rg{};
  size_t per = 0;
  for (int g = 0; g < n; ++g) {
    const wgradT_problem_t& P = pr[g];
    const wgrad_plan_group_t& G = plan.g[g];
    p.grpT[g] = gemmT_group_t{P.A, P.B, P.lda, P.ldb, P.M, P.N, P.N / BIG_BN, in[g].tiles, P.row0, P.row_end, G.item0, G.kps,
                              (uint32_t)G.ws_base};
    rg.C[g] = P.C; rg.M[g] = P.M; rg.N[g] = P.N; rg.ldc[g] = P.ldc;
    rg.ws_base[g] = (uint32_t)G.ws_base; rg.splits[g] = G.splits; rg.accumulate[g] = P.accumulate;
    if ((size_t)P.M * P.N / 4 > per) per = (size_t)P.M * P.N / 4;
  }
  hipLaunchKernelGGL(vlm_gemm_bigT_kernel<true>, dim3(plan.items), dim3(GEMM_THREADS), 0, s, p);
  VLM_CHECK_LAUNCH();
  hipLaunchKernelGGL(splitk_reduce_grouped_kernel, dim3((unsigned)((per + 255) / 256), n), dim3(256), 0, s,
                     reinterpret_cast<const float*>(splitk_ws), rg);
  VLM_CHECK_LAUNCH();
  return VLM_OK;
}

extern "C" int vlm_gemm_wgrad_batch(int n, const vlm_wgrad_problem_t* problems, int T, float* splitk_ws, uint64_t splitk_ws_bytes,
                                    void* stream) {
  if (n < 1 || n > VLM_GEMM_MAX_GROUPS || !problems || T < 1) return VLM_ERR_ARG;
  wgradT_problem_t pr[VLM_GEMM_MAX_GROUPS];
  for (int i = 0; i < n; ++i) {
    const vlm_wgrad_problem_t& P = problems[i];
    if (!P.dy || !P.x || !P.dW || P.M < 1 || P.N < 1) return VLM_ERR_ARG;
    pr[i] = wgradT_problem_t{P.dy, P.x, P.ld_dy, P.ld_x, P.M, P.N, 0, T, P.dW, P.ldc, P.accumulate};
  }
  if (gemm_big_mode() <= 0) return 1;
  return launch_gemm_bigT_grouped(n, pr, splitk_ws, splitk_ws_bytes, (hipStream_t)stream);
}

extern "C" int vlm_gemm_wgrad_grouped(int n_groups, const vlm_wgrad_group_t* groups, int M, int N, const void* A, int lda,
                                      const void* B, int ldb, int ldc, float* splitk_ws, uint64_t splitk_ws_bytes, void* stream) {
  if (n_groups < 1 || n_groups > VLM_GEMM_MAX_GROUPS || !groups || M < 0 || N < 0) return VLM_ERR_ARG;
  int prev_end = 0;
  for (int g = 0; g < n_groups; ++g) {
    if (groups[g].row0 < prev_end || groups[g].rows < 0 || !groups[g].C) return VLM_ERR_ARG;
    prev_end = groups[g].row0 + groups[g].rows;
  }
  if (M == 0 || N == 0) return VLM_OK;
  if (!A || !B || (lda & 7) || (ldb & 7) || ((uintptr_t)A & 15) || ((uintptr_t)B & 15)) return VLM_ERR_ARG;
  hipStream_t s = (hipStream_t)stream;
  for (int g = 0; g < n_groups; ++g)
    if (groups[g].rows == 0 && !groups[g].accumulate &&
        hipMemset2DAsync(groups[g].C, (size_t)ldc * 4, 0, (size_t)N * 4, M, s) != hipSuccess)
      return VLM_ERR_LAUNCH;
  const int K_total = prev_end;
  if (gemm_big_mode() > 0 && (uint64_t)K_total * lda * 2 < (1ull << 31) && (uint64_t)K_total * ldb * 2 < (1ull << 31)) {
    wgradT_problem_t pr[VLM_GEMM_MAX_GROUPS];
    int live = 0;
    for (int g = 0; g < n_groups; ++g) {
      const vlm_wgrad_group_t& G = groups[g];
      if (G.rows > 0) pr[live++] = wgradT_problem_t{A, B, lda, ldb, M, N, G.row0, G.row0 + G.rows, G.C, ldc, G.accumulate};
    }
    if (live == 0) return VLM_OK;
    const int rc = launch_gemm_bigT_grouped(live, pr, splitk_ws, splitk_ws_bytes, s);
    if (rc <= 0) return rc;
  }
  for (int g = 0; g < n_groups; ++g) {
    const vlm_wgrad_group_t& G = groups[g];
    if (G.rows == 0) continue;
    vlm_epilogue_t e{};
    e.alpha = 1.0f;
    e.accumulate = G.accumulate;
    e.splitk_ws = splitk_ws;
    e.splitk_ws_bytes = splitk_ws_bytes;
    const size_t r0 = (size_t)G.row0;
    const int rc = vlm_gemm_bf16(1, 1, M, N, G.rows, reinterpret_cast<const unsigned char*>(A) + r0 * lda * 2, lda,
                                 reinterpret_cast<const unsigned char*>(B) + r0 * ldb * 2, ldb, G.C, ldc, 1, &e, stream);
    if (rc) return rc;
  }
  return VLM_OK;
}
```

vl-merging_amd/engine.py:

```python
import itertools
import math
import os
import weakref
from typing import List, Optional

import torch

from . import _lib as L
from . import ops

BF16, F32 = torch.bfloat16, torch.float32
ALIGN = 64


def _touch_hook(p):
    p._vlm_flat.touched.add(p._vlm_name)


def touch(*params):
    for p in params:
        if p is not None:
            f = getattr(p, "_vlm_flat", None)
            if f is not None:
                f.touched.add(p._vlm_name)
# ... 71 lines not shown
        self._tr_table, self._tr_tiles = ops.transpose_table(pairs) if pairs else (None, 0)

    def refresh_transposed(self):
        self.refresh_folded()
        if getattr(self, "_tr_tiles", 0):
            ops.transpose_tiles(self._tr_table, self._tr_tiles)

    def enable_layerscale_fold(self, entries):
        if self.flat_b is None or not entries:
            return
        seen, total = set(), 0
        uniq = []
        for layer, w, b, g in entries:
            if id(w) in seen:
                continue
            seen.add(id(w))
            uniq.append((layer, w, b, g))
            total += (w.numel() + ALIGN - 1) // ALIGN * ALIGN + 2 * ((w.shape[0] + ALIGN - 1) // ALIGN * ALIGN)
        buf = torch.zeros(total, device=self.flat_p.device, dtype=F32)
        off = 0
        self._ls_jobs = {}

        def take(n, shape):
            nonlocal off
            t = buf[off:off + n].view(shape)
            off += (n + ALIGN - 1) // ALIGN * ALIGN
            return t

        for layer, w, b, g in uniq:
            w._vlm_raw = take(w.numel(), w.shape)
            raw_b = take(w.shape[0], (w.shape[0],))
            folded_b = take(w.shape[0], (w.shape[0],))
            if b is not None:
                b._vlm_raw, b._vlm_folded = raw_b, folded_b
            w._vlm_ls_gamma = g
            self._ls_jobs.setdefault(layer, []).append(dict(
                weight=w.data, gamma=g.data, bias=b.data if b is not None else None, shadow=w._vlm_bf16,
                bias_out=folded_b if b is not None else None, raw_w=w._vlm_raw, raw_b=raw_b if b is not None else None,
                dweight=w.grad, dbias=b.grad if b is not None else None, dgamma=g.grad))
        self._ls_buf = buf
        self.ls_pending = set()

    def shadow_reference(self):
        ref = self.flat_p[:self.numel].to(BF16)
        for jobs in getattr(self, "_ls_jobs", {}).values():
            for j in jobs:
                w = j["weight"]
                o = (w.data_ptr() - self.flat_p.data_ptr()) // 4
                ref[o:o + w.numel()] = (j["gamma"][:, None] * w).to(BF16).reshape(-1)
        return ref

    def refresh_folded(self):
        jobs = getattr(self, "_ls_jobs", None)
        if jobs:
            ops.layerscale_fold([j for layer in sorted(jobs) for j in jobs[layer]])

    def finish_layerscale(self, layer=None):
        pend = getattr(self, "ls_pending", None)
        if not pend:
            return
        layers = sorted(pend) if layer is None else ([layer] if layer in pend else [])
        if not layers:
            return
        jobs = [j for i in layers for j in self._ls_jobs.get(i, ())]
        side = wgrad_stream()
        if side is None:
            ops.layerscale_finish(jobs)
        else:
            side.wait_stream(torch.cuda.current_stream())
            with torch.cuda.stream(side):
                ops.layerscale_finish(jobs)
            if not _WGRAD["pending"]:
                torch.cuda.current_stream().wait_stream(side)
        for i in layers:
            pend.discard(i)

    def zero_grad(self):
        self.flat_g.zero_()
        if getattr(self, "ls_pending", None) or getattr(self, "_ls_armed", False):
            for jobs in getattr(self, "_ls_jobs", {}).values():
                for j in jobs:
                    j["raw_w"].zero_()
                    if j["raw_b"] is not None:
                        j["raw_b"].zero_()
            self.ls_pending.clear()
            self._ls_armed = False

    def slice_of(self, names):
        lo = min(self.offsets[n][0] for n in names)
        hi = max(self.offsets[n][0] + self.extent[n] for n in names)
        return lo, hi


_WGRAD = {"stream": None, "enabled": os.environ.get("VLM_WGRAD_STREAM", "1") != "0", "pending": False}


def wgrad_stream():
    if not _WGRAD["enabled"]:
        return None
    if _WGRAD["stream"] is None:
        _WGRAD["stream"] = torch.cuda.Stream()
    return _WGRAD["stream"]


def sync_wgrad():
    if _WGRAD["stream"] is not None:
        torch.cuda.current_stream().wait_stream(_WGRAD["stream"])
    _WGRAD["pending"] = False


def _arm_wgrad_join():
    if not _WGRAD["pending"]:
        _WGRAD["pending"] = True
        torch.autograd.Variable._execution_engine.queue_callback(sync_wgrad)


class _Side:

    def __init__(self, *tensors):
        self.s = wgrad_stream()
        self.tensors = tensors
        self.ctx = None

    def __enter__(self):
        if self.s is None:
            return self
        self.s.wait_stream(torch.cuda.current_stream())
        for t in self.tensors:
            t.record_stream(self.s)
        _arm_wgrad_join()
        self.ctx = torch.cuda.stream(self.s)
        self.ctx.__enter__()
        return self

    def __exit__(self, *a):
        if self.ctx is not None:
            self.ctx.__exit__(*a)
        return False


def wT16(p):
    s = getattr(p, "_vlm_bf16_t", None)
    if s is None:
        raise L.VlmError("weight has no transposed bf16 shadow: call model.setup_engine() on a CUDA model first")
    return s


_ROWSKIP = {"enabled": True}


_TAILROWS = {"enabled": True}


class KeepRows:

    def __init__(self, seq, q, span, parts):
        self.seq, self.q, self.span, self.parts = seq, q, span, parts
        self.count = sum(c for _, _, c in parts)

    @staticmethod
    def of(seq, keep):
        k0, k1 = min(int(keep[0]), seq.n0), min(int(keep[1]), seq.n1)
        if k0 <= 0 and k1 <= 0:
            return None
        B = seq.B
        if k1 <= 0 and k0 == seq.n0:
            return KeepRows(seq, (k0, 0), (seq.base0, seq.base0 + B * k0), [(seq.base0, 1, B * k0)])
        if k0 <= 0 and k1 == seq.n1:
            return KeepRows(seq, (0, k1), (seq.base1, seq.base1 + B * k1), [(seq.base1, 1, B * k1)])
        if k0 <= 1 and k1 <= 1:
            parts = ([(seq.base0, seq.n0, B)] if k0 else []) + ([(seq.base1, seq.n1, B)] if k1 else [])
            return KeepRows(seq, (max(k0, 0), max(k1, 0)), None, parts)
        return None

    def take(self, t):
        if t is None:
            return None
        if self.span is not None:
            return t[self.span[0]:self.span[1]]
        return torch.cat([t[first::step][:count] for first, step, count in self.parts])

    def put(self, g, rows, dtype):
        src, at = [], 0
        for first, step, count in self.parts:
            src.append((g[at:at + count], first, step))
            at += count
        return ops.scatter_rows(rows, g.shape[1], dtype, src, g.device)

    def ranges(self, ranges):
        out, at = [], 0
        for first, step, count in self.parts:
            last = first + (count - 1) * step
            for r0, r1, e in ranges:
                lo, hi = max(first, r0), min(last + 1, r1)
                if lo >= hi:
                    continue
                if step != 1 and not (r0 <= first and last < r1):
                    return None
                a = at + (lo - first if step == 1 else 0)
                b = at + (hi - first if step == 1 else count)
                if out and out[-1][1] == a and out[-1][2] is e:
                    out[-1] = (out[-1][0], b, e)
                else:
                    out.append((a, b, e))
            at += count
        return out

    def pieces(self, r0, r1):
        k0, k1 = self.span
        cuts = sorted({r0, r1, min(max(k0, r0), r1), min(max(k1, r0), r1)})
        return [(a, b, a - k0 if k0 <= a and b <= k1 else None) for a, b in zip(cuts, cuts[1:]) if a < b]


def _keep_rows(keep, plan, pc, rp, qkv, backward_follows):
    if keep is None or not _TAILROWS["enabled"] or pc.gram is not None:
        return None
    kr = KeepRows.of(pc.seq, keep)
    rg = kr.ranges(plan.ranges) if kr is not None else None
    if rg is None or (kr.span is None and len(rg) > 1):
        return None
    if not backward_follows:
        return kr
    served = pc.__dict__.setdefault("_qkeep_served", {})
    key = (plan.mode, rp is not None and rp.holder.get("dbias_t") is not None)
    if key not in served:
        served[key] = rp is not None and ops.attention_qkeep_served(
            qkv, pc.seq, pc.H, bias_t=rp.bias_t.detach(), head_row0=plan.layer * pc.H, rel_index=rp.index, rel_index_t=rp.index_t,
            keep0=pc.keep0, keep1=pc.keep1, mode=plan.mode, bias_dense=rp.dense_for(pc.seq, plan.mode), with_dbias=key[1])
    return kr if served[key] else None


def _live(rs, plan, pc):
    if not _ROWSKIP["enabled"] or pc.gram is not None or (pc.independent_segments and plan.mode == L.ATTN_JOINT):
        return None
    return rs


def _gemm_rows(a, groups, out, *, act=L.ACT_NONE, aux=None, col_scale=None, row_scale=None, residual=None, col_sum_fold=None,
               row_live=None):
    if len(groups) > 1:
        return ops.gemm_grouped(a, groups, out, act=act, aux=aux, col_scale=col_scale, row_scale=row_scale,
                                residual=residual, col_sum_fold=col_sum_fold)
    (r0, r1, w, bias, col_sum), = groups

    def rows(t):
        return t[r0:r1] if t is not None else None

    return ops.gemm(a[r0:r1], w, out[r0:r1], bias=bias, act=act, aux=rows(aux), col_scale=col_scale,
                    row_scale=rows(row_scale), residual=rows(residual), col_sum=col_sum, col_sum_fold=col_sum_fold,
                    row_live=rows(row_live))


def _wgrad_rows(dy, x, groups):
    if len(groups) > 1:
        return ops.gemm_wgrad_grouped(dy, x, groups)
    (r0, r1, dw), = groups
    return ops.gemm(dy[r0:r1], x[r0:r1], dw, ta=True, tb=True, accumulate=True)


def w16(p):
    s = getattr(p, "_vlm_bf16", None)
    if s is None:
        raise L.VlmError("parameter has no bf16 shadow: call model.setup_engine() on a CUDA model first")
    return s


class RelPos:

    def __init__(self, bias_t, index16, index16_t, holder, cache_tag=None, cache=None):
        self.bias_t = bias_t
        self.index = index16
        self.index_t = index16_t
        self.holder = holder
        self._dense = {}
        self.cache_tag = cache_tag
        self.cache = cache

    def dense_for(self, seq, mode):
        key = (seq.n0, seq.n1, seq.pos1, mode)
        d = self._dense.get(key)
        if d is None:
            ck = self.cache_tag + key if self.cache_tag is not None and self.cache is not None else None
            cache = self.cache
            d = cache.get(ck) if ck is not None else None
            if d is None:
                with torch.no_grad():
                    d = ops.bias_dense(self.bias_t.detach(), self.index, seq, mode)
                _DENSE_STATS["built"] += 1
                if ck is not None:
                    for k in [k for k in cache if k[:2] != ck[:2]]:
                        del cache[k]
                    while len(cache) >= 8:
                        del cache[next(iter(cache))]
                    cache[ck] = d
            else:
                _DENSE_STATS["hits"] += 1
            self._dense[key] = d
        return d

    @property
    def dbias_t(self):
        return self.holder["dbias_t"]


_CONSTS = {}
CONST_MAX = 64


def const(key, build):
    t = _CONSTS.get(key)
    if t is None:
        if len(_CONSTS) >= CONST_MAX:
            del _CONSTS[next(iter(_CONSTS))]
        t = _CONSTS[key] = build()
    return t


_ZERO = {}


def _zero_scalar(dev):
    z = _ZERO.get(str(dev))
    if z is None:
        z = _ZERO[str(dev)] = torch.zeros((), device=dev, dtype=F32)
    return z


class _TableT(torch.autograd.Function):

    @staticmethod
    def forward(ctx, table, holder):
        ctx.holder, ctx.table = holder, table
        flat = getattr(table, "_vlm_flat", None)
        if flat is None or flat.dirty:
            return table.detach().t().contiguous()
        key = (flat.version, table._version, table.data_ptr())
        ent = getattr(flat, "table_t", None)
        if ent is None or ent[0] != key:
            ent = flat.table_t = (key, table.detach().t().contiguous())
        return ent[1].view_as(ent[1])

    @staticmethod
    def backward(ctx, g):
        acc = ctx.holder.pop("dbias_t", None)
        ctx.holder.pop("routed", None)
        table = ctx.table
        z = _ZERO.get(str(g.device))
        placeholder = z is not None and g.data_ptr() == z.data_ptr()
        if acc is None:
            return (None if placeholder else g.t()), None
        if getattr(table, "_vlm_flat", None) is not None and table.requires_grad and table.grad is not None:
            touch(table)
            table.grad.add_(acc.t() if placeholder else (acc + g).t())
            return None, None
        return (acc if placeholder else acc + g).t(), None


_DENSE_STATS = {"built": 0, "hits": 0}


def make_relpos(table, index16, index16_t, index_tag=None):
    holder = {}
    bias_t = _TableT.apply(table, holder)
    if torch.is_grad_enabled() and table.requires_grad:
        holder["dbias_t"] = torch.zeros_like(bias_t)
    flat = getattr(table, "_vlm_flat", None)
    ok = flat is not None and not flat.dirty and index_tag is not None
    tag = (flat.version, table._version, index_tag) if ok else None
    return RelPos(bias_t, index16, index16_t, holder, tag, flat.dense_cache if ok else None)


class PassCtx:

    def __init__(self, seq: ops.Seq, num_heads: int, relpos: Optional[RelPos], keep0=None, keep1=None):
        self.seq = seq
        self.H = num_heads
        self.relpos = relpos
        self.keep0 = keep0
        self.keep1 = keep1
        self.gram = None
        self._row2sample = None
        self._dp_pool, self._dp_next = None, 0
        self._dp_sites, self._dp_all, self._dp_call = None, None, 0
        self.independent_segments = False
        self.uniform_source = None

    def row2sample(self, device):
        if self._row2sample is None:
            s = self.seq
            a = torch.arange(s.B, device=device).repeat_interleave(s.n0)
            b = torch.arange(s.B, device=device).repeat_interleave(s.n1)
            self._row2sample = torch.cat([a, b])
        return self._row2sample

    def plan_drop_path(self, probs):
        self._dp_sites = [float(p) for p in probs]

    def drop_path_rows(self, prob, training, device):
        if not training or prob <= 0.0:
            self._dp_call += 1
            return None
        s = self.seq
        rows = max(s.base0 + s.B * s.n0, s.base1 + s.B * s.n1)
        i = self._dp_call
        self._dp_call += 1
        if self._dp_sites is not None and i < len(self._dp_sites) and abs(self._dp_sites[i] - prob) < 1e-12:
            if self._dp_all is None:
                S = len(self._dp_sites)
                sites = tuple(self._dp_sites)
                keeps = const(("keeps", sites, str(device)),
                              lambda: torch.tensor([1.0 - p if p > 0.0 else 1.0 for p in sites], dtype=F32).to(device))
                streams = 2 if (self.independent_segments and s.n0 and s.n1) else 1
                if self.uniform_source is not None:
                    u = self.uniform_source(self, S, streams).to(device=device, dtype=F32).contiguous()
                    assert u.shape == (streams, S, s.B), (u.shape, streams, S, s.B)
                else:
                    u = torch.rand(streams, S, s.B, device=device, dtype=F32)
                self._dp_all = ops.droppath_sites(u[0], u[1] if u.shape[0] == 2 else None, keeps, s,
                                                  torch.empty(S, rows, device=device, dtype=F32))
            return self._dp_all[i]
        if self._dp_pool is None or self._dp_next + 2 > self._dp_pool.shape[0]:
            self._dp_pool = torch.rand(64, s.B, device=device, dtype=F32)
            self._dp_next = 0
        u = self._dp_pool[self._dp_next]
        self._dp_next += 1
        out = torch.empty(rows, device=device, dtype=F32)
        if self.independent_segments and s.n0 and s.n1:
            u1 = self._dp_pool[self._dp_next]
            self._dp_next += 1
            ops.droppath_rows(u, 1.0 - prob, ops.Seq(s.B, s.n0, 0, base0=s.base0, base1=s.base1), out)
            return ops.droppath_rows(u1, 1.0 - prob, ops.Seq(s.B, 0, s.n1, base0=s.base0, base1=s.base1), out)
        return ops.droppath_rows(u, 1.0 - prob, s, out)


class ExpertWeights:

    __slots__ = ("n1w", "n1b", "qkvw", "qb", "vb", "projw", "projb", "n2w", "n2b", "fc1w", "fc1b", "fc2w", "fc2b",
                 "gram_names")


class GramCapture:

    def __init__(self):
        self.grams = {}

    def add(self, name, x):
        if name is None or x.shape[0] == 0:
            return
        D = x.shape[1]
        g = self.grams.get(name)
        if g is None:
            g = self.grams[name] = torch.zeros(D, D, device=x.device, dtype=torch.float64)
        ops.gram_accumulate(x if x.stride(1) == 1 else x.contiguous(), g)

    def all_reduce(self, group=None):
        import torch.distributed as dist
        if not (dist.is_available() and dist.is_initialized()) or dist.get_world_size(group) == 1:
            return self
        mine = {k: int(v.shape[0]) for k, v in self.grams.items()}
        every = [None] * dist.get_world_size(group)
        dist.all_gather_object(every, mine, group=group)
        dev = next(iter(self.grams.values())).device if self.grams else torch.device("cuda", torch.cuda.current_device())
        for d in every:
            for k, D in d.items():
                if k not in self.grams:
                    self.grams[k] = torch.zeros(D, D, device=dev, dtype=torch.float64)
        for k in sorted(self.grams):
            dist.all_reduce(self.grams[k], group=group)
        return self

    def state_dict(self):
        return {k: v.cpu() for k, v in self.grams.items()}


_DENSE_BIAS = True


def _segment_bias_grads(ranges, seq):
    qb, vb = [None, None], [None, None]
    for sgm, (base, n) in enumerate(((seq.base0, seq.n0), (seq.base1, seq.n1))):
        if n == 0:
            continue
        lo, hi = base, base + seq.B * n
        owner = [e for r0, r1, e in ranges if r0 <= lo and hi <= r1]
        if len(owner) != 1:
            return None, None, False
        if owner[0].qb is not None:
            qb[sgm], vb[sgm] = owner[0].qb.grad, owner[0].vb.grad
    return qb, vb, True


class BlockPlan:

    def __init__(self, ranges, mode, gamma1, gamma2, layer, drop_prob, eps):
        self.ranges = ranges
        self.mode = mode
        self.gamma1, self.gamma2 = gamma1, gamma2
        self.layer = layer
        self.drop_prob = drop_prob
        self.eps = eps


def _qkv_bias(e):
    if e.qb is None:
        return None
    view = getattr(e.qb, "_vlm_qkv_bias", None)
    if view is not None:
        return view
    return torch.cat((e.qb.detach(), torch.zeros_like(e.vb), e.vb.detach()))


_FOLD_LS = os.environ.get("VLM_FOLD_LAYERSCALE", "1") != "0"


def _folded(ranges):
    return _FOLD_LS and all(getattr(e.projw, "_vlm_raw", None) is not None and getattr(e.fc2w, "_vlm_raw", None) is not None
                            for _, _, e in ranges)


def _fb(b):
    return b._vlm_folded if b is not None else None


def _rb(b):
    return b._vlm_raw if b is not None else None


def _arm_layerscale_finish(flat):
    if getattr(flat, "_ls_armed", False):
        return
    flat._ls_armed = True

    def done():
        flat._ls_armed = False
        flat.finish_layerscale()
        sync_wgrad()

    torch.autograd.Variable._execution_engine.queue_callback(done)


def _ln2_bwd_scale1(dln, x1, st2, e, dx1, dx2, y1, g1, rs1, dy1, fold):
    sgamma, dsgamma, dsbias = (None, None, _rb(e.projb)) if y1 is None else (g1, g1.grad, e.projb.grad)
    if x1.shape[1] <= 768:
        ops.layernorm_bwd_scale(dln, x1, st2, e.n2w, dx1, dx2, e.n2w.grad, e.n2b.grad, y=y1, sgamma=sgamma, row_scale=rs1,
                                sdy=dy1, dsgamma=dsgamma, dsbias=dsbias, fold=fold)
    else:
        ops.layernorm_bwd(dln, x1, st2, e.n2w, dx1, dres=dx2, dgamma=e.n2w.grad, dbeta=e.n2b.grad, fold=fold)
        ops.layerscale_bwd(dx1, y1, sgamma, rs1, dy1, dsgamma, dsbias, fold=fold)


class _BlockFn(torch.autograd.Function):

    @staticmethod
    def forward(ctx, x, bias_t, plan: BlockPlan, pc: PassCtx, training: bool, hook, keep=None, recorded=True):
        M, D = x.shape
        dev = x.device
        H = pc.H
        Fdim = plan.ranges[0][2].fc1w.shape[0]
        x = x.contiguous()
        ln1 = torch.empty(M, D, device=dev, dtype=BF16)
        st1 = torch.empty(M, 2, device=dev, dtype=F32)
        qkv = torch.empty(M, 3 * D, device=dev, dtype=BF16)
        rs1 = pc.drop_path_rows(plan.drop_prob, training, dev)
        rs2 = pc.drop_path_rows(plan.drop_prob, training, dev)
        live1, live2 = _live(rs1, plan, pc), _live(rs2, plan, pc)
        rg = plan.ranges
        for r0, r1, e in rg:
            ops.layernorm_fwd(x[r0:r1], e.n1w, e.n1b, plan.eps, ln1[r0:r1], st1[r0:r1])
        _gemm_rows(ln1, [(r0, r1, w16(e.qkvw), _qkv_bias(e), None) for r0, r1, e in rg], qkv, row_live=live1)
        o = torch.empty(M, D, device=dev, dtype=BF16)
        lse = torch.empty(H, M, device=dev, dtype=F32)
        rp = pc.relpos
        kr = _keep_rows(keep, plan, pc, rp, qkv, recorded) if bias_t is not None else None
        ops.attention_fwd(qkv, o, lse, pc.seq, H, bias_t=bias_t, head_row0=plan.layer * H,
                          rel_index=rp.index if rp is not None else None,
                          rel_index_t=rp.index_t if rp is not None else None, keep0=pc.keep0, keep1=pc.keep1,
                          mode=plan.mode, bias_dense=rp.dense_for(pc.seq, plan.mode) if rp is not None else None,
                          q_keep=kr.q if kr is not None else None)
        M_all, x_all, o_all, rs1_all, rs2_all = M, x, o, rs1, rs2
        if kr is not None:
            M, rg = kr.count, kr.ranges(rg)
            x, o, rs1, rs2, live1, live2 = (kr.take(t) for t in (x, o, rs1, rs2, live1, live2))
        x1 = torch.empty(M, D, device=dev, dtype=F32)
        folded = _folded(plan.ranges)
        y1 = torch.empty(M, D, device=dev, dtype=BF16) if not folded else None
        ln2 = torch.empty(M, D, device=dev, dtype=BF16)
        st2 = torch.empty(M, 2, device=dev, dtype=F32)
        h = torch.empty(M, Fdim, device=dev, dtype=BF16)
        a = torch.empty(M, Fdim, device=dev, dtype=BF16)
        x2 = torch.empty(M, D, device=dev, dtype=F32)
        y2 = torch.empty(M, D, device=dev, dtype=BF16) if not folded else None
        cs1, cs2 = (None, None) if folded else (plan.gamma1, plan.gamma2)
        pb = (lambda e: _fb(e.projb)) if folded else (lambda e: e.projb)
        fb2 = (lambda e: _fb(e.fc2b)) if folded else (lambda e: e.fc2b)
        _gemm_rows(o, [(r0, r1, w16(e.projw), pb(e), None) for r0, r1, e in rg], x1, col_scale=cs1, row_scale=rs1,
                   residual=x, aux=y1, row_live=live1)
        for r0, r1, e in rg:
            ops.layernorm_fwd(x1[r0:r1], e.n2w, e.n2b, plan.eps, ln2[r0:r1], st2[r0:r1])
        _gemm_rows(ln2, [(r0, r1, w16(e.fc1w), e.fc1b, None) for r0, r1, e in rg], a, act=L.ACT_GELU_DERIV, aux=h,
                   row_live=live2)
        _gemm_rows(a, [(r0, r1, w16(e.fc2w), fb2(e), None) for r0, r1, e in rg], x2, col_scale=cs2, row_scale=rs2,
                   residual=x1, aux=y2, row_live=live2)
        if pc.gram is not None:
            for r0, r1, e in plan.ranges:
                gn = e.gram_names
                if gn.get("qkv") or gn.get("fc1"):
                    t32 = torch.empty(r1 - r0, D, device=dev, dtype=F32)
                    st = torch.empty(r1 - r0, 2, device=dev, dtype=F32)
                    if gn.get("qkv"):
                        ops.layernorm_fwd(x[r0:r1], e.n1w, e.n1b, plan.eps, t32, st)
                        pc.gram.add(gn.get("qkv"), t32)
                    if gn.get("fc1"):
                        ops.layernorm_fwd(x1[r0:r1], e.n2w, e.n2b, plan.eps, t32, st)
                        pc.gram.add(gn.get("fc1"), t32)
                pc.gram.add(gn.get("proj"), o[r0:r1])
                pc.gram.add(gn.get("fc2"), a[r0:r1])
        ctx.plan, ctx.pc, ctx.hook = plan, pc, hook
        ctx.has_bias = bias_t is not None
        ctx.folded = folded
        ctx.kr = kr
        if kr is None and keep is not None and KeepRows.of(pc.seq, keep) is not None:
            ctx.kr_out = KeepRows.of(pc.seq, keep)
            x2_out = ctx.kr_out.take(x2)
        else:
            ctx.kr_out, x2_out = None, x2
        ctx.save_for_backward(x_all, st1, ln1, qkv, o_all, lse, y1 if y1 is not None else x.new_empty(0), x1, st2, ln2, h, a,
                              y2 if y2 is not None else x.new_empty(0),
                              rs1_all if rs1_all is not None else x.new_empty(0),
                              rs2_all if rs2_all is not None else x.new_empty(0),
                              bias_t if bias_t is not None else x.new_empty(0),
                              o if (kr is not None and kr.span is None) else x.new_empty(0))
        return x2_out

    @staticmethod
    def backward(ctx, dx2):
        plan, pc = ctx.plan, ctx.pc
        x, st1, ln1, qkv, o, lse, y1, x1, st2, ln2, h, a, y2, rs1, rs2, bias_t, ok = ctx.saved_tensors
        kr = ctx.kr
        rs1 = rs1 if rs1.numel() else None
        rs2 = rs2 if rs2.numel() else None
        live_all = _live(rs1, plan, pc)
        if kr is not None:
            rs1, rs2 = kr.take(rs1), kr.take(rs2)
        live1, live2 = _live(rs1, plan, pc), _live(rs2, plan, pc)
        bias_t = bias_t if ctx.has_bias else None
        M_all, D = x.shape
        M = x1.shape[0]
        dev = x.device
        H = pc.H
        Fdim = h.shape[1]
        if ctx.kr_out is not None:
            dx2 = ctx.kr_out.put(dx2.contiguous(), M_all, F32)
        dx2 = dx2.contiguous()
        g1, g2 = plan.gamma1, plan.gamma2
        folded = ctx.folded
        if folded:
            y1 = y2 = None
            flat = plan.ranges[0][2].projw._vlm_flat
            _arm_layerscale_finish(flat)
        wg = (lambda w: w._vlm_raw) if folded else (lambda w: w.grad)
        touch(g1, g2)
        for _, _, e in plan.ranges:
            _touch_expert(e)
        dy2 = torch.empty(M, D, device=dev, dtype=BF16)
        dy1 = torch.empty(M, D, device=dev, dtype=BF16)
        dh = torch.empty(M, Fdim, device=dev, dtype=BF16)
        dln = torch.empty(M, D, device=dev, dtype=BF16)
        dx1 = torch.empty(M, D, device=dev, dtype=F32)
        fold = ops.FoldBatch(dev, D)
        rg_all = plan.ranges
        rg = kr.ranges(rg_all) if kr is not None else rg_all
        if kr is None:
            ok, do_all = o, torch.empty(M_all, D, device=dev, dtype=BF16)
            do = do_all
        elif kr.span is not None:
            ok, do_all = kr.take(o), torch.empty(M_all, D, device=dev, dtype=BF16)
            do = kr.take(do_all)
        else:
            do_all, do = None, torch.empty(M, D, device=dev, dtype=BF16)
        for r0, r1, e in rg:
            rr = slice(r0, r1)
            if folded:
                ops.layerscale_bwd(dx2[rr], None, None, rs2[rr] if rs2 is not None else None, dy2[rr], None, _rb(e.fc2b), fold=fold)
            else:
                ops.layerscale_bwd(dx2[rr], y2[rr], g2, rs2[rr] if rs2 is not None else None, dy2[rr], g2.grad, e.fc2b.grad,
                                   fold=fold)
        _gemm_rows(dy2, [(r0, r1, wT16(e.fc2w), None, e.fc1b.grad) for r0, r1, e in rg], dh, act=L.ACT_MUL_AUX, aux=h,
                   col_sum_fold=fold, row_live=live2)
        tail3 = [(D, Fdim), (Fdim, D), (D, D)]
        batch = wgrad_stream() is not None and len(rg) == 1 and ops.wgrad_batch_serves(
            rg[0][1] - rg[0][0], tail3 + ([(3 * D, D)] if kr is None else []))
        if not batch:
            with _Side(dy2, a, dh, ln2):
                _wgrad_rows(dy2, a, [(r0, r1, wg(e.fc2w)) for r0, r1, e in rg])
                _wgrad_rows(dh, ln2, [(r0, r1, e.fc1w.grad) for r0, r1, e in rg])
        _gemm_rows(dh, [(r0, r1, wT16(e.fc1w), None, None) for r0, r1, e in rg], dln, row_live=live2)
        for r0, r1, e in rg:
            rr = slice(r0, r1)
            _ln2_bwd_scale1(dln[rr], x1[rr], st2[rr], e, dx1[rr], dx2[rr], y1[rr] if y1 is not None else None, g1,
                            rs1[rr] if rs1 is not None else None, dy1[rr], fold)
        _gemm_rows(dy1, [(r0, r1, wT16(e.projw), None, None) for r0, r1, e in rg], do, row_live=live1)
        if not batch:
            with _Side(dy1, ok):
                _wgrad_rows(dy1, ok, [(r0, r1, wg(e.projw)) for r0, r1, e in rg])
        if do_all is None:
            do_all = kr.put(do, M_all, BF16)
        dqkv = torch.empty(M_all, 3 * D, device=dev, dtype=BF16)
        dln1 = torch.empty(M_all, D, device=dev, dtype=BF16)
        rp = pc.relpos
        qb_grads, vb_grads, fused_qv = _segment_bias_grads(rg_all, pc.seq)
        dbias_acc = rp.holder.get("dbias_t") if rp is not None else None
        if kr is not None and dbias_acc is None:
            dbias_acc = torch.zeros_like(bias_t)
        ops.attention_bwd(qkv, o, do_all, lse, dqkv, pc.seq, H, bias_t=bias_t, head_row0=plan.layer * H,
                          rel_index=rp.index if rp is not None else None,
                          rel_index_t=rp.index_t if rp is not None else None, keep0=pc.keep0, keep1=pc.keep1,
                          mode=plan.mode, dbias_t=dbias_acc,
                          dq_colsum=qb_grads, dv_colsum=vb_grads,
                          bias_dense=rp.dense_for(pc.seq, plan.mode) if rp is not None else None, row_live=live_all,
                          q_keep=kr.q if kr is not None else None)
        dx = torch.empty(M_all, D, device=dev, dtype=F32)
        for r0, r1, e in rg_all:
            if e.qb is not None and not fused_qv:
                ops.colsum(dqkv[r0:r1, :D], e.qb.grad)
                ops.colsum(dqkv[r0:r1, 2 * D:], e.vb.grad)
        if batch:
            (r0, r1, e), = rg
            rr = slice(r0, r1)
            with _Side(dy2, a, dh, ln2, dy1, ok, dqkv, ln1):
                tail = [(dy2[rr], a[rr], wg(e.fc2w)), (dh[rr], ln2[rr], e.fc1w.grad), (dy1[rr], ok[rr], wg(e.projw))]
                if kr is None:
                    ops.gemm_wgrad_batch(tail + [(dqkv[rr], ln1[rr], e.qkvw.grad)])
                else:
                    ops.gemm_wgrad_batch(tail)
                    _wgrad_rows(dqkv, ln1, [(q0, q1, eq.qkvw.grad) for q0, q1, eq in rg_all])
        else:
            with _Side(dqkv, ln1):
                _wgrad_rows(dqkv, ln1, [(r0, r1, e.qkvw.grad) for r0, r1, e in rg_all])
        _gemm_rows(dqkv, [(r0, r1, wT16(e.qkvw), None, None) for r0, r1, e in rg_all], dln1, row_live=live_all)
        if kr is not None and kr.span is None:
            dx1 = kr.put(dx1, M_all, F32)
        for r0, r1, e in rg_all:
            for p0, p1, at in ([(r0, r1, r0)] if kr is None or kr.span is None else kr.pieces(r0, r1)):
                rr = slice(p0, p1)
                ops.layernorm_bwd(dln1[rr], x[rr], st1[rr], e.n1w, dx[rr], dres=dx1[at:at + p1 - p0] if at is not None else None,
                                  dgamma=e.n1w.grad, dbeta=e.n1b.grad, fold=fold)
        fold.flush()
        if folded:
            flat.ls_pending.add(plan.layer)
        if ctx.hook is not None:
            ctx.hook(plan.layer)
        dbias = None
        if bias_t is not None and ctx.needs_input_grad[1] and rp is not None and not rp.holder.get("routed"):
            rp.holder["routed"] = True
            dbias = _zero_scalar(dev).expand_as(bias_t)
        return dx, dbias, None, None, None, None, None, None


def run_block(x, plan: BlockPlan, pc: PassCtx, training: bool, hook=None, keep=None):
    bias_t = pc.relpos.bias_t if pc.relpos is not None else None
    if keep is not None and KeepRows.of(pc.seq, keep) is None:
        raise L.VlmError("run_block: keep must name whole segments or first rows, got %r" % (keep,))
    recorded = torch.is_grad_enabled() and (x.requires_grad or (bias_t is not None and bias_t.requires_grad))
    return _BlockFn.apply(x, bias_t, plan, pc, training, hook, keep, recorded)


def _kernel_rows(t, dtypes=(BF16, F32), row_align=1, ptr_align=1, layout=True):
    if not (torch.is_tensor(t) and t.is_cuda and t.dtype in dtypes):
        return False
    return not layout or (t.dim() == 2 and t.stride(1) == 1 and t.stride(0) % row_align == 0 and t.data_ptr() % ptr_align == 0)


def _rows2d(g, D, dtypes=(BF16, F32), contiguous=False):
    g2 = g.reshape(-1, D)
    if g2.dtype not in dtypes:
        g2 = g2.float()
    return g2.contiguous() if contiguous or g2.stride(1) != 1 else g2


class _LinearFn(torch.autograd.Function):

    @staticmethod
    def forward(ctx, x, weight, bias, act):
        x2 = x.reshape(-1, x.shape[-1])
        if x2.dtype != BF16:
            x2 = x2.to(BF16)
        if x2.stride(1) != 1 or (x2.shape[0] > 1 and x2.stride(0) < x2.shape[1]):
            x2 = x2.contiguous()
        M, K = x2.shape
        N = weight.shape[0]
        Np = (N + 63) // 64 * 64
        gelu = act == "gelu"
        buf = torch.empty(M, Np, device=x.device, dtype=BF16)
        pre = torch.empty(M, Np, device=x.device, dtype=BF16) if gelu else None
        ops.gemm(x2, w16(weight), buf[:, :N], bias=bias, act=L.ACT_GELU if gelu else L.ACT_NONE,
                 aux=pre[:, :N] if gelu else None)
        y = ops.tanh_fwd(buf[:, :N]) if act == "tanh" else None
        ctx.save_for_backward(x2, pre if gelu else (y if y is not None else x2.new_empty(0)))
        ctx.weight, ctx.bias, ctx.act, ctx.shape, ctx.N, ctx.Np = weight, bias, act, x.shape, N, Np
        return (y if y is not None else buf[:, :N]).view(*x.shape[:-1], N)

    @staticmethod
    def backward(ctx, gy):
        x2, saved = ctx.saved_tensors
        weight, bias, N, Np, act = ctx.weight, ctx.bias, ctx.N, ctx.Np, ctx.act
        M, K = x2.shape
        gy2 = _rows2d(gy, N)
        if (act is None and gy2.dtype == BF16 and gy2.stride() == (Np, 1) and gy2.storage_offset() == 0
                and _is_padded_grad(gy2, M, Np)):
            dy = torch.as_strided(gy2, (M, Np), (Np, 1))
        elif act is None and Np == N and gy2.dtype == BF16:
            dy = gy2
        else:
            mode = {"gelu": ops.ACT_BWD_GELU, "tanh": ops.ACT_BWD_TANH, None: ops.ACT_BWD_NONE}[act]
            dy = ops.act_bwd(gy2, saved[:, :N] if act is not None else None, mode, Np)
        touch(weight if weight.requires_grad else None, bias if bias is not None and bias.requires_grad else None)
        if bias is not None and bias.requires_grad:
            if N % 8 == 0:
                ops.colsum(dy[:, :N], bias.grad)
            elif N <= 64:
                ops.colsum_small(dy[:, :N], bias.grad)
            elif bias.grad.is_contiguous():
                N8 = N // 8 * 8
                ops.colsum(dy[:, :N8], bias.grad[:N8])
                ops.colsum_small(dy[:, N8:N], bias.grad[N8:])
            else:
                bias.grad.add_(dy[:, :N].float().sum(0))
        if weight.requires_grad:
            ops.gemm(dy[:, :N], x2, weight.grad, ta=True, tb=True, accumulate=True)
        dx = None
        if ctx.needs_input_grad[0]:
            wpad = w16(weight) if Np == N else torch.as_strided(w16(weight), (Np, K), (K, 1))
            if Np >= 8192 and ((M + 127) // 128) * ((K + 127) // 128) <= 128:
                dx32 = torch.zeros(M, K, device=x2.device, dtype=F32)
                ops.gemm(dy, wpad, dx32, tb=True, accumulate=True)
                dx = dx32.to(BF16)
            else:
                dx = torch.empty(M, K, device=x2.device, dtype=BF16)
                ops.gemm(dy, wpad, dx, tb=True)
            dx = dx.view(ctx.shape)
        return dx, None, None, None


def linear(x, weight, bias=None, gelu=False, act=None):
    return _LinearFn.apply(x, weight, bias, "gelu" if gelu else act)


class _L2NormFn(torch.autograd.Function):

    @staticmethod
    def forward(ctx, x):
        y, inv = ops.l2norm_fwd(_rows2d(x, x.shape[-1]))
        ctx.save_for_backward(y, inv)
        ctx.dtype, ctx.shape = x.dtype, x.shape
        return y.view(x.shape)

    @staticmethod
    def backward(ctx, g):
        y, inv = ctx.saved_tensors
        return ops.l2norm_bwd(_rows2d(g, y.shape[1], (F32,), contiguous=True), y, inv, ctx.dtype).view(ctx.shape)


def l2_normalize(x):
    if _kernel_rows(x, layout=False):
        return _L2NormFn.apply(x)
    x = x.float()
    return x / x.norm(dim=-1, keepdim=True)


class _ContrastiveFn(torch.autograd.Function):

    @staticmethod
    def forward(ctx, img, txt, log_scale, gather):
        B = img.shape[0]
        all_img, all_txt = (img, txt) if gather is None else (gather(img), gather(txt))
        ls = log_scale.detach().reshape(1).float()
        out3, logits, d_img, d_txt = ops.contrastive(all_img.contiguous(), all_txt.contiguous(), B, ls)
        ctx.save_for_backward(out3, d_img, d_txt)
        ctx.ls_shape = log_scale.shape
        ctx.mark_non_differentiable(logits)
        ctx.set_materialize_grads(False)
        return out3[0], logits, out3[2]

    @staticmethod
    def backward(ctx, g_loss, _g_logits, g_scale):
        out3, d_img, d_txt = ctx.saved_tensors
        if g_loss is None:
            g_loss = torch.zeros((), device=out3.device, dtype=F32)
        gi, gt, gs = ops.scale_by_scalar([d_img, d_txt, out3[1:2]], g_loss.reshape(1).float())
        gs = gs.view(ctx.ls_shape)
        if g_scale is not None:
# ... 334 lines not shown
```

vl-merging_amd/ops.py:

```python
import ctypes

import torch

from . import _lib as L

BF16 = torch.bfloat16
F32 = torch.float32


def _ld(t):
    if t.dim() != 2 or t.stride(1) != 1:
        raise L.VlmError("expected a 2-D tensor with unit inner stride, got shape %s strides %s"
                         % (tuple(t.shape), t.stride()))
    return t.stride(0) if t.shape[0] > 1 else max(t.stride(0), t.shape[1])


_SCRATCH = {}


def _scratch(kind, floats, device):
    key = (kind, device.index, torch.cuda.current_stream().cuda_stream)
    ws = _SCRATCH.get(key)
    if ws is None or ws.numel() < floats:
        ws = _SCRATCH[key] = torch.empty(floats, device=device, dtype=F32)
    return ws


SPLITK_WS_BYTES = 96 << 20


def _epilogue(N, *, bias=None, col_scale=None, row_scale=None, residual=None, aux=None, act=L.ACT_NONE, alpha=1.0, accumulate=False,
              col_sum=None):
    e = L.Epilogue()
    e.bias = bias.data_ptr() if bias is not None else 0
    e.col_scale = col_scale.data_ptr() if col_scale is not None else 0
    e.row_scale = row_scale.data_ptr() if row_scale is not None else 0
    e.residual = residual.data_ptr() if residual is not None else 0
    e.ld_res = _ld(residual) if residual is not None else 0
    e.aux = aux.data_ptr() if aux is not None else 0
    e.ld_aux = _ld(aux) if aux is not None else 0
    e.act = act
    e.alpha = alpha
    e.accumulate = 1 if accumulate else 0
    e.col_sum = col_sum.data_ptr() if col_sum is not None else 0
    if col_sum is not None and (col_sum.numel() < N or not col_sum.is_contiguous()):
        raise L.VlmError("gemm: col_sum must be a contiguous f32 vector of at least N elements")
    for t, dt in ((bias, F32), (col_scale, F32), (row_scale, F32), (residual, F32), (aux, BF16), (col_sum, F32)):
        if t is not None and t.dtype != dt:
            raise L.VlmError("gemm epilogue tensor has dtype %s, expected %s" % (t.dtype, dt))
    return e


def gemm(a, b, out, ta=False, tb=False, *, bias=None, act=L.ACT_NONE, aux=None, col_scale=None, row_scale=None,
         residual=None, alpha=1.0, accumulate=False, col_sum=None, col_sum_fold=None, row_live=None):
    L.require_cuda(a, b, out, bias, aux, col_scale, row_scale, residual, col_sum, row_live)
    if a.dtype != BF16 or b.dtype != BF16:
        raise L.VlmError("gemm operands must be bfloat16")
    M, N = out.shape
    K = a.shape[0] if ta else a.shape[1]
    if (a.shape[1] if ta else a.shape[0]) != M:
        raise L.VlmError("gemm: A rows %s do not match M=%d" % (tuple(a.shape), M))
    kb, nb = (b.shape[0], b.shape[1]) if tb else (b.shape[1], b.shape[0])
    if nb != N or kb != K:
        raise L.VlmError("gemm: B shape %s incompatible with N=%d K=%d" % (tuple(b.shape), N, K))
    e = _epilogue(N, bias=bias, col_scale=col_scale, row_scale=row_scale, residual=residual, aux=aux, act=act, alpha=alpha,
                  accumulate=accumulate, col_sum=col_sum)
    region = None
    if col_sum is not None and col_sum_fold is not None and not ta and N % 128 == 0 and M >= 128:
        region = col_sum_fold.next_region()
        if region.numel() >= (M // 128) * 2 * N:
            e.col_sum_ws = region.data_ptr()
        else:
            region = None
    if ta and tb and out.dtype == F32 and K >= 2048 and bias is None and col_sum is None:
        ws = _scratch("splitk", SPLITK_WS_BYTES // 4, out.device)
        e.splitk_ws = ws.data_ptr()
        e.splitk_ws_bytes = ws.numel() * 4
    if out.dtype not in (BF16, F32):
        raise L.VlmError("gemm output must be bf16 or f32")
    if row_live is not None:
        if row_live.dtype != F32 or row_live.dim() != 1 or row_live.shape[0] != M or row_live.stride(0) != 1:
            raise L.VlmError("gemm: row_live must be a dense f32 vector of M=%d elements" % M)
        rc = L.get_lib().vlm_gemm_bf16_live(int(ta), int(tb), M, N, K, L.ptr(a), _ld(a), L.ptr(b), _ld(b), L.ptr(out), _ld(out),
                                            int(out.dtype == F32), ctypes.byref(e), L.ptr(row_live), L.stream_ptr())
    else:
        rc = L.get_lib().vlm_gemm_bf16(int(ta), int(tb), M, N, K, L.ptr(a), _ld(a), L.ptr(b), _ld(b), L.ptr(out), _ld(out),
                                       int(out.dtype == F32), ctypes.byref(e), L.stream_ptr())
    L.check(rc, "vlm_gemm_bf16")
    if region is not None:
        col_sum_fold.add(region, M // 128, N, col_sum, None)
    return out


def gemm_grouped(a, groups, out, *, act=L.ACT_NONE, aux=None, col_scale=None, row_scale=None, residual=None, alpha=1.0,
                 col_sum_fold=None):
    L.require_cuda(a, out, aux, col_scale, row_scale, residual)
    if a.dtype != BF16:
        raise L.VlmError("gemm operands must be bfloat16")
    if len(groups) < 1 or len(groups) > L.GEMM_MAX_GROUPS:
        raise L.VlmError("gemm_grouped: 1..%d groups" % L.GEMM_MAX_GROUPS)
    M, N = out.shape
    K = a.shape[1]
    if a.shape[0] != M:
        raise L.VlmError("gemm_grouped: A rows %s do not match M=%d" % (tuple(a.shape), M))
    e = _epilogue(N, col_scale=col_scale, row_scale=row_scale, residual=residual, aux=aux, act=act, alpha=alpha)
    if out.dtype not in (BF16, F32):
        raise L.VlmError("gemm output must be bf16 or f32")
    arr = (L.GemmGroup * len(groups))()
    folds = []
    prev = 0
    if col_sum_fold is not None and len(col_sum_fold.jobs) + len(groups) > col_sum_fold.MAX:
        col_sum_fold.flush()
    for g, (r0, r1, w, bias, col_sum) in zip(arr, groups):
        L.require_cuda(w, bias, col_sum)
        if w.dtype != BF16 or tuple(w.shape) != (N, K) or r0 < prev or r1 < r0 or r1 > M:
            raise L.VlmError("gemm_grouped: group (%d, %d) weight %s for N=%d K=%d M=%d" % (r0, r1, tuple(w.shape), N, K, M))
        prev = r1
        for t in (bias, col_sum):
            if t is not None and (t.dtype != F32 or t.numel() < N or not t.is_contiguous()):
                raise L.VlmError("gemm_grouped: bias / col_sum must be contiguous f32 vectors of at least N elements")
        g.row0, g.rows, g.B, g.ldb = r0, r1 - r0, w.data_ptr(), _ld(w)
        g.bias = bias.data_ptr() if bias is not None else None
        g.col_sum = col_sum.data_ptr() if col_sum is not None else None
        rows = r1 - r0
        if col_sum is not None and col_sum_fold is not None and N % 128 == 0 and rows >= 128:
            region = col_sum_fold.next_region()
            if region.numel() >= (rows // 128) * 2 * N:
                g.col_sum_ws = region.data_ptr()
                col_sum_fold.add(region, rows // 128, N, col_sum, None)
                folds.append(region)
    rc = L.get_lib().vlm_gemm_bf16_grouped(len(groups), arr, N, K, L.ptr(a), _ld(a), L.ptr(out), _ld(out),
                                           int(out.dtype == F32), ctypes.byref(e), L.stream_ptr())
    L.check(rc, "vlm_gemm_bf16_grouped")
    return out


def gemm_wgrad_grouped(dy, x, groups, accumulate=True):
    L.require_cuda(dy, x)
    if dy.dtype != BF16 or x.dtype != BF16 or dy.shape[0] != x.shape[0]:
        raise L.VlmError("gemm_wgrad_grouped: bf16 dy [tokens, M] and x [tokens, N]")
    M, N = dy.shape[1], x.shape[1]
    arr = (L.WgradGroup * len(groups))()
    prev, ldc = 0, None
    for g, (r0, r1, dW) in zip(arr, groups):
        L.require_cuda(dW)
        if dW.dtype != F32 or tuple(dW.shape) != (M, N) or r0 < prev or r1 < r0 or r1 > dy.shape[0]:
            raise L.VlmError("gemm_wgrad_grouped: group (%d, %d) gradient %s for M=%d N=%d" % (r0, r1, tuple(dW.shape), M, N))
        if ldc is not None and _ld(dW) != ldc:
            raise L.VlmError("gemm_wgrad_grouped: the groups' gradients must share one leading dimension")
        ldc = _ld(dW)
        prev = r1
        g.row0, g.rows, g.C, g.accumulate = r0, r1 - r0, dW.data_ptr(), int(bool(accumulate))
    ws = _scratch("splitk", SPLITK_WS_BYTES // 4, dy.device)
    rc = L.get_lib().vlm_gemm_wgrad_grouped(len(groups), arr, M, N, L.ptr(dy), _ld(dy), L.ptr(x), _ld(x), ldc, L.ptr(ws),
                                            ws.numel() * 4, L.stream_ptr())
    L.check(rc, "vlm_gemm_wgrad_grouped")


def wgrad_batch_serves(T, shapes):
    cus = L.get_lib().vlm_device_cus()
    return (T >= 2048 and 1 <= len(shapes) <= L.GEMM_MAX_GROUPS and all(N % 256 == 0 for _, N in shapes)
            and sum(-(-M // 256) * (N // 256) for M, N in shapes) <= (cus if cus > 0 else 256))


def gemm_wgrad_batch(problems, accumulate=True):
    n = len(problems)
    if n < 1 or n > L.GEMM_MAX_GROUPS:
        raise L.VlmError("gemm_wgrad_batch: 1..%d problems" % L.GEMM_MAX_GROUPS)
    acc = [bool(accumulate)] * n if isinstance(accumulate, (bool, int)) else [bool(f) for f in accumulate]
    if len(acc) != n:
        raise L.VlmError("gemm_wgrad_batch: one accumulate flag, or one per problem")
    T = problems[0][0].shape[0]
    arr = (L.WgradProblem * n)()
    for g, (dy, x, dW), f in zip(arr, problems, acc):
        L.require_cuda(dy, x, dW)
        if dy.dtype != BF16 or x.dtype != BF16 or dW.dtype != F32 or dy.dim() != 2 or x.dim() != 2 or dW.dim() != 2:
            raise L.VlmError("gemm_wgrad_batch: bf16 dy [T, M] and x [T, N], f32 dW [M, N]")
        if dy.shape[0] != T or x.shape[0] != T or tuple(dW.shape) != (dy.shape[1], x.shape[1]):
            raise L.VlmError("gemm_wgrad_batch: dy %s, x %s, dW %s over T=%d rows" % (tuple(dy.shape), tuple(x.shape),
                                                                                      tuple(dW.shape), T))
        g.dy, g.ld_dy, g.M = dy.data_ptr(), _ld(dy), dy.shape[1]
        g.x, g.ld_x, g.N = x.data_ptr(), _ld(x), x.shape[1]
        g.dW, g.ldc, g.accumulate = dW.data_ptr(), _ld(dW), int(f)
    rc = 1
    if T >= 2048:
        ws = _scratch("splitk", SPLITK_WS_BYTES // 4, problems[0][0].device)
        rc = L.get_lib().vlm_gemm_wgrad_batch(n, arr, T, L.ptr(ws), ws.numel() * 4, L.stream_ptr())
    if rc == 1:
        for (dy, x, dW), f in zip(problems, acc):
            gemm(dy, x, dW, ta=True, tb=True, accumulate=f)
        return
    L.check(rc, "vlm_gemm_wgrad_batch")


def layernorm_fwd(x, gamma, beta, eps, out, stats=None):
    L.require_cuda(x, gamma, beta, out, stats)
    M, D = x.shape
    rc = L.get_lib().vlm_layernorm_fwd(L.ptr(x), _ld(x), M, D, L.ptr(gamma), L.ptr(beta), eps, L.ptr(out), _ld(out),
                                       int(out.dtype == F32), L.ptr(stats), L.stream_ptr())
    L.check(rc, "vlm_layernorm_fwd")
    return out


def _row_ws_floats(D):
    return 1536 * 2 * max(D, 1024)


class FoldBatch:

    MAX = 16

    def __init__(self, device, D=1024):
        self.region = _row_ws_floats(D)
        self.ws = _scratch("fold", self.MAX * self.region, device)
        self.jobs = []
        self.taken = 0

    def next_region(self):
        return self.next_regions(1)[0]

    def next_regions(self, n):
        if self.taken + n > self.MAX:
            self.flush()
        i = self.taken
        self.taken += n
        return [self.ws[(i + k) * self.region:(i + k + 1) * self.region] for k in range(n)]

    def add(self, region, nblocks, D, out0, out1):
        if nblocks > 0:
            self.jobs.append((region, nblocks, D, out0, out1))

    def flush(self):
        self.taken = 0
        if not self.jobs:
            return
        arr = (L.FoldJob * len(self.jobs))()
        for a, (region, nblocks, D, out0, out1) in zip(arr, self.jobs):
            a.partials, a.nblocks, a.D = region.data_ptr(), nblocks, D
            a.out0 = out0.data_ptr() if out0 is not None else None
            a.out1 = out1.data_ptr() if out1 is not None else None
        L.check(L.get_lib().vlm_colreduce_batch(arr, len(self.jobs), L.stream_ptr()), "vlm_colreduce_batch")
        self.jobs = []


def _row_bwd(name, fold, device, D, head, pairs, sc=None):
    ws = (fold.next_regions(len(pairs)) if fold is not None
          else [_scratch("row%d" % k, _row_ws_floats(D), device) for k in range(len(pairs))])
    nb = ctypes.c_int(0)
    tail = (ctypes.byref(nb) if fold is not None else None, L.stream_ptr())
    if sc is not None:
        sc.workspace, sc.workspace_bytes = L.ptr(ws[1]), ws[1].numel() * 4
        tail = (ctypes.byref(sc),) + tail
    L.check(getattr(L.get_lib(), name)(*head, L.ptr(ws[0]), ws[0].numel() * 4, *tail), name)
    if fold is not None:
        for region, outs in zip(ws, pairs):
            fold.add(region, nb.value if any(o is not None for o in outs) else 0, D, *outs)


def _layernorm_bwd(name, fold, dy, x, stats, gamma, dx, dres, dgamma, dbeta, more_pairs=(), sc=None):
    M, D = x.shape
    _row_bwd(name, fold, x.device, D,
             (L.ptr(dy), _ld(dy), int(dy.dtype == F32), L.ptr(x), _ld(x), L.ptr(stats), L.ptr(gamma), M, D, L.ptr(dres),
              _ld(dres) if dres is not None else 0, L.ptr(dx), _ld(dx), L.ptr(dgamma), L.ptr(dbeta)),
             [(dgamma, dbeta), *more_pairs], sc)
    return dx


def layernorm_bwd(dy, x, stats, gamma, dx, dres=None, dgamma=None, dbeta=None, fold=None):
    L.require_cuda(dy, x, stats, gamma, dx, dres, dgamma, dbeta)
    return _layernorm_bwd("vlm_layernorm_bwd", fold, dy, x, stats, gamma, dx, dres, dgamma, dbeta)


def layernorm_bwd_scale(dy, x, stats, gamma, dx, dres, dgamma, dbeta, *, y, sgamma, row_scale, sdy, dsgamma=None, dsbias=None,
                        fold=None):
    L.require_cuda(dy, x, stats, gamma, dx, dres, dgamma, dbeta, y, sgamma, row_scale, sdy, dsgamma, dsbias)
    sc = L.LayerScale()
    sc.y, sc.ldy, sc.gamma, sc.row_scale = L.ptr(y), _ld(y) if y is not None else 0, L.ptr(sgamma), L.ptr(row_scale)
    sc.dy, sc.lddy, sc.dgamma, sc.dbias = L.ptr(sdy), _ld(sdy), L.ptr(dsgamma), L.ptr(dsbias)
    return _layernorm_bwd("vlm_layernorm_bwd_scale", fold, dy, x, stats, gamma, dx, dres, dgamma, dbeta, [(dsgamma, dsbias)], sc)


def layerscale_bwd(dx, y, gamma, row_scale, dy, dgamma=None, dbias=None, fold=None):
    L.require_cuda(dx, y, gamma, row_scale, dy, dgamma, dbias)
    M, D = dx.shape
    _row_bwd("vlm_layerscale_bwd", fold, dx.device, D,
             (L.ptr(dx), _ld(dx), L.ptr(y), _ld(y) if y is not None else 0, L.ptr(gamma), L.ptr(row_scale), M, D, L.ptr(dy),
              _ld(dy), L.ptr(dgamma), L.ptr(dbias)), [(dgamma, dbias)])
    return dy


def embedding_bwd(gy, ids, dW, padding_idx=-1):
    L.require_cuda(gy, ids, dW)
    n, D = gy.shape
    assert gy.dtype == F32 and dW.dtype == F32 and ids.dtype == torch.int64 and ids.numel() == n and gy.stride(1) == 1
    L.check(L.get_lib().vlm_embedding_bwd(L.ptr(gy), _ld(gy), L.ptr(ids), n, D, int(padding_idx), L.ptr(dW), _ld(dW),
                                          dW.shape[0], L.stream_ptr()), "vlm_embedding_bwd")
    return dW


def cross_entropy_fwd(logits, labels, ignore_index=-100):
    L.require_cuda(logits, labels)
    rows, V = logits.shape
    if logits.dtype != BF16 or labels.dtype != torch.int64 or labels.numel() != rows or not labels.is_contiguous():
        raise L.VlmError("cross_entropy: bf16 logits [rows, V], contiguous int64 labels [rows]")
    loss_rows = torch.empty(rows, device=logits.device, dtype=F32)
    lse = torch.empty(rows, device=logits.device, dtype=F32)
    L.check(L.get_lib().vlm_cross_entropy_fwd(L.ptr(logits), _ld(logits), rows, V, L.ptr(labels), int(ignore_index), L.ptr(loss_rows),
                                              L.ptr(lse), L.stream_ptr()), "vlm_cross_entropy_fwd")
    return loss_rows, lse


def cross_entropy_bwd(logits, labels, lse, scale, ignore_index=-100):
    L.require_cuda(logits, labels, lse, scale)
    rows, V = logits.shape
    Vp = (V + 63) // 64 * 64
    buf = torch.empty(rows, Vp, device=logits.device, dtype=BF16)
    L.check(L.get_lib().vlm_cross_entropy_bwd(L.ptr(logits), _ld(logits), rows, V, L.ptr(labels), int(ignore_index), L.ptr(lse),
                                              L.ptr(scale), L.ptr(buf), Vp, L.stream_ptr()), "vlm_cross_entropy_bwd")
    return buf[:, :V]


def l2norm_fwd(x):
    L.require_cuda(x)
    rows, D = x.shape
    if x.dtype not in (BF16, F32) or x.stride(1) != 1:
        raise L.VlmError("l2norm: bf16 / fp32 [rows, D] with unit column stride")
    y = torch.empty(rows, D, device=x.device, dtype=F32)
    inv = torch.empty(rows, device=x.device, dtype=F32)
    L.check(L.get_lib().vlm_l2norm_fwd(L.ptr(x), int(x.dtype == BF16), _ld(x), rows, D, L.ptr(y), L.ptr(inv), L.stream_ptr()), "vlm_l2norm_fwd")
    return y, inv


def l2norm_bwd(g, y, inv, dtype):
    L.require_cuda(g, y, inv)
    rows, D = y.shape
    if g.dtype != F32 or not g.is_contiguous() or g.shape != y.shape:
# ... 114 lines not shown
    L.check(L.get_lib().vlm_image_lead_rows(L.ptr(x), _ld(x), B, rows, D, _rowvec(lead, D, "lead"), L.stream_ptr()), "vlm_image_lead_rows")


def image_rows_bwd(g, B, rows, d_bias, d_type_row, d_cls):
    L.require_cuda(g, d_bias, d_type_row, d_cls)
    n, D = g.shape
    if g.dtype != F32 or g.stride(1) != 1 or n != B * rows:
        raise L.VlmError("image_rows_bwd: fp32 [B * rows, D] gradient rows")
    g16 = torch.empty(n, D, device=g.device, dtype=BF16)
    ws = _scratch("image_rows", max(1, L.get_lib().vlm_image_rows_bwd_ws_floats(D)), g.device)
    L.check(L.get_lib().vlm_image_rows_bwd(L.ptr(g), _ld(g), B, rows, D, L.ptr(g16), _rowvec(d_bias, D, "d_bias"),
                                           _rowvec(d_type_row, D, "d_type_row"), _rowvec(d_cls.reshape(-1) if d_cls is not None else None, D, "d_cls"),
                                           L.ptr(ws), L.stream_ptr()), "vlm_image_rows_bwd")
    return g16


def tanh_fwd(x):
    L.require_cuda(x)
    M, N = x.shape
    if x.dtype != BF16 or x.stride(1) != 1:
        raise L.VlmError("tanh_fwd: bf16 [M, N] with unit column stride")
    y = torch.empty(M, N, device=x.device, dtype=F32)
    L.check(L.get_lib().vlm_tanh_fwd(L.ptr(x), _ld(x), M, N, L.ptr(y), L.stream_ptr()), "vlm_tanh_fwd")
    return y


ACT_BWD_GELU, ACT_BWD_TANH, ACT_BWD_NONE = 0, 1, 2


def act_bwd(g, saved, mode, Np=None):
    L.require_cuda(g, saved)
    M, N = g.shape
    Np = N if Np is None else Np
    if g.dtype not in (BF16, F32) or g.stride(1) != 1:
        raise L.VlmError("act_bwd: bf16 / fp32 gradient [M, N] with unit column stride")
    if mode != ACT_BWD_NONE:
        if saved.stride(1) != 1 or saved.shape[0] != M or saved.shape[1] < N:
            raise L.VlmError("act_bwd: saved [M, >= N] with unit column stride")
        if saved.dtype != (BF16 if mode == ACT_BWD_GELU else F32):
            raise L.VlmError("act_bwd: saved pre-activation is bf16 (GELU) / saved output is fp32 (tanh)")
    dy = torch.empty(M, Np, device=g.device, dtype=BF16)
    L.check(L.get_lib().vlm_act_bwd(L.ptr(g), int(g.dtype == F32), _ld(g), L.ptr(saved) if saved is not None else 0,
                                    _ld(saved) if saved is not None else 0, mode, M, N, Np, L.ptr(dy), L.stream_ptr()), "vlm_act_bwd")
    return dy


def colsum_small(a, out):
    L.require_cuda(a, out)
    M, N = a.shape
    if a.dtype != BF16 or a.stride(1) != 1 or out.dtype != F32 or out.numel() < N or not out.is_contiguous():
        raise L.VlmError("colsum_small: bf16 [M, N <= 64], fp32 out")
    L.check(L.get_lib().vlm_colsum_small(L.ptr(a), _ld(a), M, N, L.ptr(out), L.stream_ptr()), "vlm_colsum_small")
    return out


def sample_negatives(sim_a, sim_b, B, u):
    L.require_cuda(sim_a, sim_b, u)
    n = sim_a.shape[1]
    for t in (sim_a, sim_b):
        if t.dtype != F32 or t.dim() != 2 or t.shape[0] < B or t.shape[1] != n:
            raise L.VlmError("sample_negatives: two fp32 similarity matrices [>= B, n]")
    if u.dtype != F32 or u.numel() != 2 * B or not u.is_contiguous():
        raise L.VlmError("sample_negatives: u is fp32 [2, B]")
    idx = torch.empty(2, B, device=sim_a.device, dtype=torch.int64)
    L.check(L.get_lib().vlm_sample_negatives(L.ptr(sim_a), sim_a.stride(0), sim_a.stride(1), L.ptr(sim_b), sim_b.stride(0), sim_b.stride(1), B, n,
                                             L.ptr(u), L.ptr(idx), L.stream_ptr()), "vlm_sample_negatives")
    return idx


def scatter_rows(R, D, dtype, sources, device):
    if dtype not in (BF16, F32) or len(sources) > 4:
        raise L.VlmError("scatter_rows: bf16 / fp32 output, at most four sources")
    dx = torch.empty(R, D, device=device, dtype=dtype)
    arr = (L.ScatterSrc * max(1, len(sources)))()
    for a, (g, first, step) in zip(arr, sources):
        L.require_cuda(g)
        if g.dim() != 2 or g.shape[1] != D or g.dtype not in (BF16, F32) or g.stride(1) != 1:
            raise L.VlmError("scatter_rows: sources are bf16 / fp32 [count, D] with unit column stride")
        if first + (g.shape[0] - 1) * step >= R and g.shape[0]:
            raise L.VlmError("scatter_rows: source rows %d + %d * j (j < %d) leave the %d output rows" % (first, step, g.shape[0], R))
        a.g, a.g_is_f32, a.ld, a.first_row, a.row_step, a.count = L.ptr(g), int(g.dtype == F32), _ld(g), first, step, g.shape[0]
    L.check(L.get_lib().vlm_scatter_rows(L.ptr(dx), int(dtype == F32), D, R, D, ctypes.cast(arr, ctypes.c_void_p), len(sources), L.stream_ptr()),
            "vlm_scatter_rows")
    return dx


def weighted_sum(terms, weights):
    L.require_cuda(*terms)
    k = len(terms)
    if k == 0 or k > 8 or len(weights) != k or any(t.dtype != F32 or t.numel() != 1 for t in terms):
        raise L.VlmError("weighted_sum: 1..8 fp32 device scalars with one host weight each")
    out = torch.empty((), device=terms[0].device, dtype=F32)
    P = ctypes.c_void_p * k
    W = ctypes.c_float * k
    L.check(L.get_lib().vlm_weighted_sum(P(*[L.ptr(t) for t in terms]), W(*[float(w) for w in weights]), k, L.ptr(out), L.stream_ptr()),
            "vlm_weighted_sum")
    return out


def colsum(a, out):
    L.require_cuda(a, out)
    M, N = a.shape
    L.check(L.get_lib().vlm_colsum_bf16(L.ptr(a), _ld(a), M, N, L.ptr(out), L.stream_ptr()), "vlm_colsum_bf16")
    return out


def adamw_step(p, g, m, v, p_bf16, lr, beta1, beta2, eps, weight_decay, step, grad_scale=1.0, zero_grad=True):
    L.require_cuda(p, g, m, v, p_bf16)
    bc1 = 1.0 - beta1 ** step
    bc2 = 1.0 - beta2 ** step
    step_size = lr * (bc2 ** 0.5) / bc1
    rc = L.get_lib().vlm_adamw_step(L.ptr(p), L.ptr(g), L.ptr(m), L.ptr(v), L.ptr(p_bf16), p.numel(), lr, beta1, beta2,
                                    eps, weight_decay, step_size, grad_scale, int(zero_grad), L.stream_ptr())
    L.check(rc, "vlm_adamw_step")


def cast_bf16(src, dst):
    L.require_cuda(src, dst)
    L.check(L.get_lib().vlm_cast_f32_bf16(L.ptr(src), L.ptr(dst), src.numel(), L.stream_ptr()), "vlm_cast_f32_bf16")
    return dst


def transpose_table(pairs):
    import numpy as np
    recs = []
    for src, dst in pairs:
        L.require_cuda(src, dst)
        if src.dtype != BF16 or dst.dtype != BF16 or not src.is_contiguous() or not dst.is_contiguous() \
                or src.dim() != 2 or tuple(dst.shape) != (src.shape[1], src.shape[0]):
            raise L.VlmError("transpose_table: contiguous bf16 [rows, cols] -> [cols, rows] pairs")
        rows, cols = src.shape
        for tr in range((rows + 63) // 64):
            for tc in range((cols + 63) // 64):
                recs.append((src.data_ptr(), dst.data_ptr(), rows | (cols << 32), tr | (tc << 32)))
    arr = np.array(recs, dtype=np.uint64).reshape(-1, 4)
    dev = pairs[0][0].device if pairs else "cuda"
    return torch.from_numpy(arr.view(np.int64)).to(dev), len(recs)


def transpose_tiles(table, n_tiles):
    if n_tiles:
        L.check(L.get_lib().vlm_transpose_bf16_tiles(L.ptr(table), n_tiles, L.stream_ptr()), "vlm_transpose_bf16_tiles")


def droppath_sites(u0, u1, keeps, seq, out):
    L.require_cuda(u0, u1, keeps, out)
    S = keeps.numel()
    if u0.dtype != F32 or keeps.dtype != F32 or out.dtype != F32 or tuple(u0.shape) != (S, seq.B) or not out.is_contiguous() \
            or out.shape[0] != S or (u1 is not None and tuple(u1.shape) != (S, seq.B)):
        raise L.VlmError("droppath_sites: u [S, B] f32, keeps [S] f32, out [S, rows] f32")
    L.check(L.get_lib().vlm_droppath_sites(L.ptr(u0), L.ptr(u1), L.ptr(keeps), S, seq.B, seq.n0, seq.n1, seq.base0, seq.base1,
                                           out.shape[1], L.ptr(out), L.stream_ptr()), "vlm_droppath_sites")
    return out


def droppath_rows(u, keep, seq, out):
    L.require_cuda(u, out)
    if u.dtype != F32 or out.dtype != F32 or u.numel() < seq.B or not out.is_contiguous():
        raise L.VlmError("droppath_rows: u f32 [B], out contiguous f32 [rows]")
    L.check(L.get_lib().vlm_droppath_rows(L.ptr(u), float(keep), seq.B, seq.n0, seq.n1, seq.base0, seq.base1, L.ptr(out),
                                          L.stream_ptr()), "vlm_droppath_rows")
    return out


def gram_accumulate(x, gram64, tmp32=None):
    L.require_cuda(x, gram64)
    M, D = x.shape
    if gram64.dtype != torch.float64 or tuple(gram64.shape) != (D, D) or not gram64.is_contiguous():
        raise L.VlmError("gram accumulator must be a contiguous float64 [D,D] tensor")
    if x.dtype not in (BF16, F32):
        raise L.VlmError("gram_accumulate: bf16 or fp32 activations")
    L.check(L.get_lib().vlm_gram_f64(L.ptr(x), _ld(x), M, D, int(x.dtype == F32), L.ptr(gram64), L.stream_ptr()), "vlm_gram_f64")
    return gram64


F64 = torch.float64


def gemm_f64(a, b, c, ta=False, tb=False, alpha=1.0, beta=0.0):
    L.require_cuda(a, b, c)
    if b.dtype != F64 or c.dtype != F64 or a.dtype not in (F64, F32):
        raise L.VlmError("gemm_f64: a float64/float32, b and c float64")
    M, N = c.shape
    K = a.shape[0] if ta else a.shape[1]
    if (a.shape[1] if ta else a.shape[0]) != M or (b.shape[1] if tb else b.shape[0]) != K or (b.shape[0] if tb else b.shape[1]) != N:
        raise L.VlmError("gemm_f64: shapes %s %s -> %s" % (tuple(a.shape), tuple(b.shape), tuple(c.shape)))
    if K == 0:
        if beta == 0.0:
            c.zero_()
        return c
    L.check(L.get_lib().vlm_gemm_f64(int(ta), int(tb), M, N, K, float(alpha), L.ptr(a), _ld(a), int(a.dtype == F32), L.ptr(b),
                                     _ld(b), float(beta), L.ptr(c), _ld(c), L.stream_ptr()), "vlm_gemm_f64")
    return c


def scale_gram(src, dst, alpha, accumulate=False):
    L.require_cuda(src, dst)
    n = src.shape[0]
    if src.dtype != F64 or dst.dtype != F64 or tuple(src.shape) != (n, n) or tuple(dst.shape) != (n, n) \
            or not src.is_contiguous() or not dst.is_contiguous():
        raise L.VlmError("scale_gram: contiguous float64 [n,n] matrices")
    L.check(L.get_lib().vlm_scale_gram_f64(L.ptr(src), L.ptr(dst), n, float(alpha), int(accumulate), L.stream_ptr()),
            "vlm_scale_gram_f64")
    return dst


F64_MAX_BATCH = 64


def _ptr_list(ts):
    arr = (ctypes.c_void_p * len(ts))()
    for i, t in enumerate(ts):
        arr[i] = t.data_ptr()
    return arr


def _f64_chunks(*lists):
    for i in range(0, len(lists[0]), F64_MAX_BATCH):
        yield [x[i:i + F64_MAX_BATCH] for x in lists]


def _f64_squares(mats, who):
    n = mats[0].shape[0]
    for m in mats:
        if m.dtype != F64 or tuple(m.shape) != (n, n) or not m.is_contiguous():
            raise L.VlmError(who + ": contiguous float64 [n,n] matrices of one size")
    return n


def _f64_rhs(rhs, n, who):
    rows, ld = rhs[0].shape[0], _ld(rhs[0])
    for r in rhs:
        if r.dtype != F64 or tuple(r.shape) != (rows, n) or _ld(r) != ld:
            raise L.VlmError(who + ": float64 right-hand sides [rows, n] of one shape")
    return rows, ld


def gemm_f64_batched(a_list, b_list, c_list, alpha=1.0, beta=0.0, ta=False):
    if not (len(a_list) == len(b_list) == len(c_list)):
        raise L.VlmError("gemm_f64_batched: three lists of one length")
    if not a_list:
        return c_list
    L.require_cuda(*a_list, *b_list, *c_list)
    a0, b0, c0 = a_list[0], b_list[0], c_list[0]
    M, K = (a0.shape[1], a0.shape[0]) if ta else a0.shape
    N = b0.shape[1]
    for a, b, c in zip(a_list, b_list, c_list):
        if a.dtype != a0.dtype or a.dtype not in (F64, F32) or b.dtype != F64 or c.dtype != F64 or tuple(a.shape) != tuple(a0.shape) \
                or tuple(b.shape) != (K, N) or tuple(c.shape) != (M, N) or not (a.is_contiguous() and b.is_contiguous() and c.is_contiguous()):
            raise L.VlmError("gemm_f64_batched: contiguous a [M,K] (one of float64/float32), float64 b [K,N], c [M,N] of one shape")
    if K == 0:
        if beta == 0.0:
            for c in c_list:
                c.zero_()
        return c_list
    for a, b, c in _f64_chunks(a_list, b_list, c_list):
        L.check(L.get_lib().vlm_gemm_f64_batched(int(bool(ta)), 0, M, N, K, float(alpha), _ptr_list(a), M if ta else K, int(a0.dtype == F32), _ptr_list(b), N,
                                                 float(beta), _ptr_list(c), N, len(a), L.stream_ptr()), "vlm_gemm_f64_batched")
    return c_list


def cholesky_batched_(mats, status):
    L.require_cuda(status, *mats)
    n = _f64_squares(mats, "cholesky_batched_")
    for m, st in _f64_chunks(mats, status):
        L.check(L.get_lib().vlm_cholesky_f64_batched(_ptr_list(m), len(m), n, L.ptr(st), L.stream_ptr()), "vlm_cholesky_f64_batched")
    return mats


def solve_spd_right_batched_(rhs, chols):
    L.require_cuda(*rhs, *chols)
    n = _f64_squares(chols, "solve_spd_right_batched_")
    rows, ld = _f64_rhs(rhs, n, "solve_spd_right_batched_")
    for r, c in _f64_chunks(rhs, chols):
        L.check(L.get_lib().vlm_solve_spd_right_f64_batched(_ptr_list(c), n, _ptr_list(r), ld, rows, len(r), L.stream_ptr()),
                "vlm_solve_spd_right_f64_batched")
    return rhs


def cholesky_(s, status=None):
    own = status is None
    if own:
        status = torch.zeros(1, device=s.device, dtype=torch.int32)
    cholesky_batched_([s], status)
    if own:
        bad = int(status.item())
        if bad:
            raise L.VlmError("cholesky_: matrix is not positive definite (pivot %d)" % (bad - 1))
    return s


def solve_spd_right_(rhs, chol):
    solve_spd_right_batched_([rhs], [chol])
    return rhs


def _f64_work(work, m, n, size, who, shape_ok=True, shape="a positive shape", what=None):
    if not 1 <= len(work) <= F64_MAX_BATCH or m < 1 or n < 1 or not shape_ok:
        raise L.VlmError("%s: 1 .. %d matrices of %s" % (who, F64_MAX_BATCH, shape))
    for w in work:
        if w.dtype != F64 or w.dim() != 1 or w.numel() != size or not w.is_contiguous():
            raise L.VlmError("%s: a working set is a contiguous float64 %s" % (who, what or "[%d] tensor for a [%d, %d] matrix" % (size, m, n)))


def _iso_work(work, m, n, who):
    _f64_work(work, m, n, L.ISO_HEAD + 3 * m * n, who, what="[%d + 3 * %d * %d] tensor" % (L.ISO_HEAD, m, n))
# ... 392 lines not shown
```

Before: 365.8.

## Skip dropped-path row blocks in weight-gradient GEMM K loop via live masks

Builds per-site bitmasks marking which 32-row K steps have any surviving drop-path rows, and passes them into the grouped/batched weight-gradient GEMM. The kernel iterates only over live K steps using a cursor, shrinking the K trip count when whole row blocks are zeroed by stochastic depth. This removes redundant loads and MFMA work on rows whose gradient is zero. The cost is an extra mask kernel per step, some scalar cursor logic in the inner loop, and a minimum trip count that pads short ranges.

```diff
diff --git a/include/vlm_hip.h b/include/vlm_hip.h
--- a/include/vlm_hip.h
+++ b/include/vlm_hip.h
@@ -434,7 +434,8 @@
   int32_t row0, rows;
   float* C;
   int32_t accumulate;
-  int32_t reserved;
+  int32_t live_bit0;
+  const uint64_t* live;
 } vlm_wgrad_group_t;
 int vlm_gemm_wgrad_grouped(int n_groups, const vlm_wgrad_group_t* groups, int M, int N, const void* A, int lda,
                            const void* B, int ldb, int ldc, float* splitk_ws, uint64_t splitk_ws_bytes, void* stream);
@@ -445,6 +446,8 @@
   int32_t ld_x, N;
   float* dW;
   int32_t ldc, accumulate;
+  const uint64_t* live;
+  int32_t live_bit0, reserved;
 } vlm_wgrad_problem_t;
 int vlm_gemm_wgrad_batch(int n, const vlm_wgrad_problem_t* problems, int T, float* splitk_ws, uint64_t splitk_ws_bytes,
                          void* stream);
@@ -563,6 +566,7 @@
 int vlm_droppath_rows(const float* u, float keep, int B, int n0, int n1, int base0, int base1, float* out, void* stream);
 int vlm_droppath_sites(const float* u0, const float* u1, const float* keep, int n_sites, int B, int n0, int n1, int base0,
                        int base1, int rows, float* out, void* stream);
+int vlm_droppath_step_masks(const float* table, int sites, int rows, uint64_t* masks, void* stream);
 int vlm_patch_im2col(const float* image, void* patches_bf16, int B, int H, int W, int P, int lead_rows, void* stream);
 int vlm_accumulate_f32_f64(const float* src, double* dst_f64, uint64_t n, void* stream);
 int vlm_gram_f64(const void* x, int ldx, int M, int D, int x_is_f32, double* gram, void* stream);
diff --git a/vl-merging_amd/_lib.py b/vl-merging_amd/_lib.py
--- a/vl-merging_amd/_lib.py
+++ b/vl-merging_amd/_lib.py
@@ -322,12 +322,13 @@
 
 class WgradGroup(ctypes.Structure):
     _fields_ = [("row0", ctypes.c_int32), ("rows", ctypes.c_int32), ("C", c_void_p), ("accumulate", ctypes.c_int32),
-                ("reserved", ctypes.c_int32)]
+                ("live_bit0", ctypes.c_int32), ("live", c_void_p)]
 
 
 class WgradProblem(ctypes.Structure):
     _fields_ = [("dy", c_void_p), ("ld_dy", ctypes.c_int32), ("M", ctypes.c_int32), ("x", c_void_p), ("ld_x", ctypes.c_int32),
-                ("N", ctypes.c_int32), ("dW", c_void_p), ("ldc", ctypes.c_int32), ("accumulate", ctypes.c_int32)]
+                ("N", ctypes.c_int32), ("dW", c_void_p), ("ldc", ctypes.c_int32), ("accumulate", ctypes.c_int32),
+                ("live", c_void_p), ("live_bit0", ctypes.c_int32), ("reserved", ctypes.c_int32)]
 
 
 class FoldJob(ctypes.Structure):
@@ -521,6 +522,7 @@
     "vlm_transpose_bf16_tiles": (c_int, [c_void_p, c_int, c_void_p]),
     "vlm_droppath_sites": (c_int, [c_void_p, c_void_p, c_void_p, c_int, c_int, c_int, c_int, c_int, c_int, c_int, c_void_p,
                                    c_void_p]),
+    "vlm_droppath_step_masks": (c_int, [c_void_p, c_int, c_int, c_void_p, c_void_p]),
     "vlm_droppath_rows": (c_int, [c_void_p, c_float, c_int, c_int, c_int, c_int, c_int, c_void_p, c_void_p]),
     "vlm_patch_im2col": (c_int, [c_void_p, c_void_p, c_int, c_int, c_int, c_int, c_int, c_void_p]),
 }
diff --git a/vl-merging_amd/csrc/elementwise.hip b/vl-merging_amd/csrc/elementwise.hip
--- a/vl-merging_amd/csrc/elementwise.hip
+++ b/vl-merging_amd/csrc/elementwise.hip
@@ -1,4 +1,5 @@
 #include "vlm_common.h"
+#include "wgrad_live.h"
 
 #define EW_THREADS 256
 #ifndef EW_NT
@@ -221,6 +222,32 @@
   return VLM_OK;
 }
 
+__global__ __launch_bounds__(EW_THREADS) void droppath_step_masks_kernel(const float* __restrict__ table, int rows, int words,
+                                                                         unsigned long long* __restrict__ masks) {
+  const int lane = threadIdx.x & 63, w = blockIdx.x * (EW_THREADS / 64) + (threadIdx.x >> 6);
+  if (w >= words) return;
+  const float* t = table + (size_t)blockIdx.y * rows;
+  unsigned long long word = 0;
+#pragma unroll 8
+  for (int i = 0; i < 32; ++i) {
+    const long row = ((long)w * 64 + 2 * i) * WGRAD_LIVE_ROWS + lane;
+    const unsigned long long b = __ballot(row < rows && t[row] != 0.0f);
+    word |= (unsigned long long)((b & 0xffffffffull) != 0) << (2 * i);
+    word |= (unsigned long long)((b >> 32) != 0) << (2 * i + 1);
+  }
+  if (lane == 0) masks[(size_t)blockIdx.y * words + w] = word;
+}
+
+extern "C" int vlm_droppath_step_masks(const float* table, int sites, int rows, uint64_t* masks, void* stream) {
+  if (sites <= 0 || rows <= 0) return VLM_OK;
+  if (!table || !masks) return VLM_ERR_ARG;
+  const int words = wgrad_live_words(wgrad_live_steps(rows)), per = EW_THREADS / 64;
+  hipLaunchKernelGGL(droppath_step_masks_kernel, dim3((words + per - 1) / per, sites), dim3(EW_THREADS), 0, (hipStream_t)stream,
+                     table, rows, words, reinterpret_cast<unsigned long long*>(masks));
+  VLM_CHECK_LAUNCH();
+  return VLM_OK;
+}
+
 __global__ __launch_bounds__(256) void transpose_tiles_kernel(const vlm_transpose_tile_t* __restrict__ tiles, int n_tiles) {
   __shared__ bf16_t tile[64][66];
   for (int t = blockIdx.x; t < n_tiles; t += gridDim.x) {
diff --git a/vl-merging_amd/csrc/gemm.hip b/vl-merging_amd/csrc/gemm.hip
--- a/vl-merging_amd/csrc/gemm.hip
+++ b/vl-merging_amd/csrc/gemm.hip
@@ -1,5 +1,6 @@
 #include "vlm_common.h"
 #include "vlm_diag.h"
+#include "wgrad_live.h"
 #include "wgrad_plan.h"
 #include <atomic>
 
@@ -122,6 +123,8 @@
   int lda, ldb, M, N, tiles_n, ntile;
   int row0, row_end, item0, kps;
   uint32_t ws_base;
+  int live_bit0;
+  const uint64_t* live;
 };
 
 struct gemm_params_t {
@@ -982,6 +985,8 @@
   const void *A = p.A, *B = p.B;
   uint32_t lda = (uint32_t)p.lda, ldb = (uint32_t)p.ldb;
   int M = p.M, N = p.N;
+  const uint64_t* live = nullptr;
+  int live_bit0 = 0;
   if constexpr (GROUPED) {
     int g = 0;
 #pragma unroll
@@ -997,11 +1002,20 @@
     lda = (uint32_t)G.lda; ldb = (uint32_t)G.ldb;
     M = G.M; N = G.N;
     ntile = (uint32_t)G.ntile; tiles_n = (uint32_t)G.tiles_n;
+    live = G.live; live_bit0 = G.live_bit0;
   }
   const uint32_t split = item / ntile, tile = item - split * ntile;
   const uint32_t tm = tile / tiles_n, tn = tile - tm * tiles_n;
   const uint32_t m0 = tm * BIG_BM, n0 = tn * BIG_BN;
-  const uint32_t k_first = k_base + split * (uint32_t)nk * BIG_BK;
+  uint32_t k_first = k_base + split * (uint32_t)nk * BIG_BK;
+  wgrad_live_cursor_t cur;
+  uint32_t soa = 0, sob = 0;
+  if constexpr (GROUPED) {
+    const int ksteps = (int)((k_end - k_base + BIG_BK - 1) / BIG_BK);
+    const int s0 = (int)split * nk, s1 = s0 + nk < ksteps ? s0 + nk : ksteps;
+    nk = wgrad_live_trips(wgrad_live_open(cur, live, live_bit0, s0, s1, ksteps));
+    k_first = k_base;
+  }
   const __amdgpu_buffer_rsrc_t ra =
       __builtin_amdgcn_make_buffer_rsrc(const_cast<void*>(A), 0, (int)((uint64_t)k_end * lda * 2), 0x00020000);
   const __amdgpu_buffer_rsrc_t rb =
@@ -1045,10 +1059,16 @@
     FA[i] = __builtin_bit_cast(bf16x8, (s16x8){al[0], al[1], al[2], al[3], ah[0], ah[1], ah[2], ah[3]}); \
     FB[i] = __builtin_bit_cast(bf16x8, (s16x8){bl[0], bl[1], bl[2], bl[3], bh[0], bh[1], bh[2], bh[3]}); \
   }
+#define BIGT_NEXT()                                                                                  \
+  if constexpr (GROUPED) {                                                                           \
+    const uint32_t step_i = (uint32_t)wgrad_live_next(cur);                                          \
+    soa = step_i * stepa;                                                                            \
+    sob = step_i * stepb;                                                                            \
+  }
 #define BIGT_GLOAD(RA_, RB_, S)                                                                      \
   _Pragma("unroll") for (int u = 0; u < 4; ++u) {                                                    \
-    RA_[u] = __builtin_amdgcn_raw_buffer_load_b128(ra, offa[u], (S) * stepa, 0);                     \
-    RB_[u] = __builtin_amdgcn_raw_buffer_load_b128(rb, offb[u], (S) * stepb, 0);                     \
+    RA_[u] = __builtin_amdgcn_raw_buffer_load_b128(ra, offa[u], GROUPED ? soa : (S) * stepa, 0);     \
+    RB_[u] = __builtin_amdgcn_raw_buffer_load_b128(rb, offb[u], GROUPED ? sob : (S) * stepb, 0);     \
   }
 #define BIGT_LWRITE(RA_, RB_, SA, SB)                                                                \
   _Pragma("unroll") for (int u = 0; u < 4; ++u) {                                                    \
@@ -1061,6 +1081,7 @@
       asm volatile("s_waitcnt lgkmcnt(0)" ::: "memory");                                 \
       __builtin_amdgcn_s_barrier();                                                      \
     }                                                                                    \
+    if (GL) { BIGT_NEXT() }                                                              \
     __builtin_amdgcn_sched_barrier(0);                                                   \
     if (WR) { BIGT_LWRITE(RSA, RSB, BUFA_W, BUFB_W) }                                    \
     if (GL) { BIGT_GLOAD(RSA, RSB, (K) + 4) }                                            \
@@ -1078,15 +1099,20 @@
     }                                                                                    \
     __builtin_amdgcn_sched_barrier(0);                                                   \
   }
+  BIGT_NEXT()
   BIGT_GLOAD(ra0, rb0, 0)
+  BIGT_NEXT()
   BIGT_GLOAD(ra1, rb1, 1)
   BIGT_LWRITE(ra0, rb0, sA0, sB0)
+  BIGT_NEXT()
   BIGT_GLOAD(ra0, rb0, 2)
   BIGT_LWRITE(ra1, rb1, sA1, sB1)
+  BIGT_NEXT()
   BIGT_GLOAD(ra1, rb1, 3)
   asm volatile("s_waitcnt lgkmcnt(0)" ::: "memory");
   __builtin_amdgcn_s_barrier();
   BIGT_READ(fa0, fb0, sA0, sB0)
+  if constexpr (GROUPED) { BIG_PIN_ACC() }
   int kt = 0;
   for (; kt < nk - 4; kt += 2) {
     BIGT_STEP(kt + 0, 1, 1, 1, fa0, fb0, fa1, fb1, ra0, rb0, sA0, sB0, sA1, sB1)
@@ -1381,6 +1407,8 @@
   int lda, ldb, M, N, row0, row_end;
   float* C;
   int ldc, accumulate;
+  const uint64_t* live;
+  int live_bit0;
 };
 static int launch_gemm_bigT_grouped(int n, const wgradT_problem_t* pr, float* splitk_ws, uint64_t splitk_ws_bytes, hipStream_t s) {
   if (!splitk_ws || ((uintptr_t)splitk_ws & 15) || n < 1 || n > VLM_GEMM_MAX_GROUPS) return 1;
@@ -1417,7 +1445,7 @@
     const wgradT_problem_t& P = pr[g];
     const wgrad_plan_group_t& G = plan.g[g];
     p.grpT[g] = gemmT_group_t{P.A, P.B, P.lda, P.ldb, P.M, P.N, P.N / BIG_BN, in[g].tiles, P.row0, P.row_end, G.item0, G.kps,
-                              (uint32_t)G.ws_base};
+                              (uint32_t)G.ws_base, P.live_bit0, P.live};
     rg.C[g] = P.C; rg.M[g] = P.M; rg.N[g] = P.N; rg.ldc[g] = P.ldc;
     rg.ws_base[g] = (uint32_t)G.ws_base; rg.splits[g] = G.splits; rg.accumulate[g] = P.accumulate;
     if ((size_t)P.M * P.N / 4 > per) per = (size_t)P.M * P.N / 4;
@@ -1437,7 +1465,8 @@
   for (int i = 0; i < n; ++i) {
     const vlm_wgrad_problem_t& P = problems[i];
     if (!P.dy || !P.x || !P.dW || P.M < 1 || P.N < 1) return VLM_ERR_ARG;
-    pr[i] = wgradT_problem_t{P.dy, P.x, P.ld_dy, P.ld_x, P.M, P.N, 0, T, P.dW, P.ldc, P.accumulate};
+    if (P.live && P.live_bit0 < 0) return VLM_ERR_ARG;
+    pr[i] = wgradT_problem_t{P.dy, P.x, P.ld_dy, P.ld_x, P.M, P.N, 0, T, P.dW, P.ldc, P.accumulate, P.live, P.live_bit0};
   }
   if (gemm_big_mode() <= 0) return 1;
   return launch_gemm_bigT_grouped(n, pr, splitk_ws, splitk_ws_bytes, (hipStream_t)stream);
@@ -1448,7 +1477,8 @@
   if (n_groups < 1 || n_groups > VLM_GEMM_MAX_GROUPS || !groups || M < 0 || N < 0) return VLM_ERR_ARG;
   int prev_end = 0;
   for (int g = 0; g < n_groups; ++g) {
-    if (groups[g].row0 < prev_end || groups[g].rows < 0 || !groups[g].C) return VLM_ERR_ARG;
+    if (groups[g].row0 < prev_end || groups[g].rows < 0 || !groups[g].C || (groups[g].live && groups[g].live_bit0 < 0))
+      return VLM_ERR_ARG;
     prev_end = groups[g].row0 + groups[g].rows;
   }
   if (M == 0 || N == 0) return VLM_OK;
@@ -1464,7 +1494,8 @@
     int live = 0;
     for (int g = 0; g < n_groups; ++g) {
       const vlm_wgrad_group_t& G = groups[g];
-      if (G.rows > 0) pr[live++] = wgradT_problem_t{A, B, lda, ldb, M, N, G.row0, G.row0 + G.rows, G.C, ldc, G.accumulate};
+      if (G.rows > 0) pr[live++] = wgradT_problem_t{A, B, lda, ldb, M, N, G.row0, G.row0 + G.rows, G.C, ldc, G.accumulate,
+                                                        G.live, G.live_bit0};
     }
     if (live == 0) return VLM_OK;
     const int rc = launch_gemm_bigT_grouped(live, pr, splitk_ws, splitk_ws_bytes, s);
diff --git a/vl-merging_amd/csrc/wgrad_live.h b/vl-merging_amd/csrc/wgrad_live.h
--- /dev/null
+++ b/vl-merging_amd/csrc/wgrad_live.h
@@ -0,0 +1,70 @@
+#pragma once
+#include <stdint.h>
+
+#if defined(__HIPCC__)
+#define WGRAD_LIVE_FN __host__ __device__ static inline
+#else
+#define WGRAD_LIVE_FN static inline
+#endif
+#if defined(__HIP_DEVICE_COMPILE__)
+typedef const __attribute__((address_space(4))) uint64_t* wgrad_live_ptr_t;
+#else
+typedef const uint64_t* wgrad_live_ptr_t;
+#endif
+
+#define WGRAD_LIVE_ROWS 32
+
+WGRAD_LIVE_FN int wgrad_live_steps(int rows) { return (rows + WGRAD_LIVE_ROWS - 1) / WGRAD_LIVE_ROWS; }
+WGRAD_LIVE_FN int wgrad_live_words(int steps) { return (steps + 63) >> 6; }
+
+WGRAD_LIVE_FN int wgrad_live_count(const uint64_t* mask_, int b0, int b1) {
+  if (b1 <= b0) return 0;
+  if (!mask_) return b1 - b0;
+  const wgrad_live_ptr_t mask = (wgrad_live_ptr_t)mask_;
+  const int w0 = b0 >> 6, w1 = (b1 - 1) >> 6;
+  int n = 0;
+  for (int w = w0; w <= w1; ++w) {
+    uint64_t v = mask[w];
+    if (w == w0) v &= ~0ull << (b0 & 63);
+    if (w == w1 && (b1 & 63)) v &= ~0ull >> (64 - (b1 & 63));
+    n += __builtin_popcountll(v);
+  }
+  return n;
+}
+
+WGRAD_LIVE_FN int wgrad_live_trips(int live) {
+  const int n = live + (live & 1);
+  return n < 4 ? 4 : n;
+}
+
+struct wgrad_live_cursor_t {
+  wgrad_live_ptr_t word;
+  uint64_t win;
+  int base;
+  int left;
+  int pad;
+};
+
+WGRAD_LIVE_FN int wgrad_live_open(wgrad_live_cursor_t& c, const uint64_t* mask, int bit0, int s0, int s1, int ksteps) {
+  const int b0 = bit0 + s0, b1 = bit0 + s1;
+  c.left = wgrad_live_count(mask, b0, b1);
+  c.pad = ksteps;
+  c.word = mask ? (wgrad_live_ptr_t)mask + (b0 >> 6) : nullptr;
+  c.base = (b0 & ~63) - bit0;
+  c.win = 0;
+  if (c.left > 0) c.win = (mask ? *c.word : ~0ull) & (~0ull << (b0 & 63));
+  return c.left;
+}
+
+WGRAD_LIVE_FN int wgrad_live_next(wgrad_live_cursor_t& c) {
+  if (c.left <= 0) return c.pad;
+  --c.left;
+  while (c.win == 0) {
+    c.base += 64;
+    if (c.word) c.win = *++c.word;
+    else c.win = ~0ull;
+  }
+  const int b = __builtin_ctzll(c.win);
+  c.win &= c.win - 1;
+  return c.base + b;
+}
diff --git a/vl-merging_amd/engine.py b/vl-merging_amd/engine.py
--- a/vl-merging_amd/engine.py
+++ b/vl-merging_amd/engine.py
@@ -247,6 +247,9 @@
 _TAILROWS = {"enabled": True}
 
 
+_WGRADLIVE = {"enabled": True}
+
+
 class KeepRows:
 
     def __init__(self, seq, q, span, parts):
@@ -346,10 +349,19 @@
                     row_live=rows(row_live))
 
 
-def _wgrad_rows(dy, x, groups):
+def _live_steps(steps, row_at, r0):
+    if steps is None or row_at is None or (row_at + r0) % 32:
+        return None
+    return (steps, (row_at + r0) // 32)
+
+
+def _wgrad_rows(dy, x, groups, steps=None, row_at=0):
+    live = [_live_steps(steps, row_at, r0) for r0, _, _ in groups]
     if len(groups) > 1:
-        return ops.gemm_wgrad_grouped(dy, x, groups)
+        return ops.gemm_wgrad_grouped(dy, x, groups, live=live if any(lv is not None for lv in live) else None)
     (r0, r1, dw), = groups
+    if live[0] is not None and ops.wgrad_batch_serves(r1 - r0, [tuple(dw.shape)]):
+        return ops.gemm_wgrad_grouped(dy, x, groups, live=live)
     return ops.gemm(dy[r0:r1], x[r0:r1], dw, ta=True, tb=True, accumulate=True)
 
 
@@ -477,6 +489,7 @@
         self._row2sample = None
         self._dp_pool, self._dp_next = None, 0
         self._dp_sites, self._dp_all, self._dp_call = None, None, 0
+        self._dp_masks, self.last_steps = None, None
         self.independent_segments = False
         self.uniform_source = None
 
@@ -492,6 +505,7 @@
         self._dp_sites = [float(p) for p in probs]
 
     def drop_path_rows(self, prob, training, device):
+        self.last_steps = None
         if not training or prob <= 0.0:
             self._dp_call += 1
             return None
@@ -513,6 +527,8 @@
                     u = torch.rand(streams, S, s.B, device=device, dtype=F32)
                 self._dp_all = ops.droppath_sites(u[0], u[1] if u.shape[0] == 2 else None, keeps, s,
                                                   torch.empty(S, rows, device=device, dtype=F32))
+                self._dp_masks = ops.droppath_step_masks(self._dp_all) if _WGRADLIVE["enabled"] else None
+            self.last_steps = self._dp_masks[i] if self._dp_masks is not None else None
             return self._dp_all[i]
         if self._dp_pool is None or self._dp_next + 2 > self._dp_pool.shape[0]:
             self._dp_pool = torch.rand(64, s.B, device=device, dtype=F32)
@@ -657,7 +673,9 @@
         st1 = torch.empty(M, 2, device=dev, dtype=F32)
         qkv = torch.empty(M, 3 * D, device=dev, dtype=BF16)
         rs1 = pc.drop_path_rows(plan.drop_prob, training, dev)
+        steps1 = pc.last_steps
         rs2 = pc.drop_path_rows(plan.drop_prob, training, dev)
+        steps2 = pc.last_steps
         live1, live2 = _live(rs1, plan, pc), _live(rs2, plan, pc)
         rg = plan.ranges
         for r0, r1, e in rg:
@@ -714,6 +732,7 @@
         ctx.has_bias = bias_t is not None
         ctx.folded = folded
         ctx.kr = kr
+        ctx.steps = tuple(m if _live(m, plan, pc) is not None and _WGRADLIVE["enabled"] else None for m in (steps1, steps2))
         if kr is None and keep is not None and KeepRows.of(pc.seq, keep) is not None:
             ctx.kr_out = KeepRows.of(pc.seq, keep)
             x2_out = ctx.kr_out.take(x2)
@@ -765,6 +784,8 @@
         fold = ops.FoldBatch(dev, D)
         rg_all = plan.ranges
         rg = kr.ranges(rg_all) if kr is not None else rg_all
+        steps1, steps2 = ctx.steps
+        at = 0 if kr is None else (kr.span[0] if kr.span is not None else None)
         if kr is None:
             ok, do_all = o, torch.empty(M_all, D, device=dev, dtype=BF16)
             do = do_all
@@ -787,8 +808,8 @@
             rg[0][1] - rg[0][0], tail3 + ([(3 * D, D)] if kr is None else []))
         if not batch:
             with _Side(dy2, a, dh, ln2):
-                _wgrad_rows(dy2, a, [(r0, r1, wg(e.fc2w)) for r0, r1, e in rg])
-                _wgrad_rows(dh, ln2, [(r0, r1, e.fc1w.grad) for r0, r1, e in rg])
+                _wgrad_rows(dy2, a, [(r0, r1, wg(e.fc2w)) for r0, r1, e in rg], steps2, at)
+                _wgrad_rows(dh, ln2, [(r0, r1, e.fc1w.grad) for r0, r1, e in rg], steps2, at)
         _gemm_rows(dh, [(r0, r1, wT16(e.fc1w), None, None) for r0, r1, e in rg], dln, row_live=live2)
         for r0, r1, e in rg:
             rr = slice(r0, r1)
@@ -797,7 +818,7 @@
         _gemm_rows(dy1, [(r0, r1, wT16(e.projw), None, None) for r0, r1, e in rg], do, row_live=live1)
         if not batch:
             with _Side(dy1, ok):
-                _wgrad_rows(dy1, ok, [(r0, r1, wg(e.projw)) for r0, r1, e in rg])
+                _wgrad_rows(dy1, ok, [(r0, r1, wg(e.projw)) for r0, r1, e in rg], steps1, at)
         if do_all is None:
             do_all = kr.put(do, M_all, BF16)
         dqkv = torch.empty(M_all, 3 * D, device=dev, dtype=BF16)
@@ -824,14 +845,15 @@
             rr = slice(r0, r1)
             with _Side(dy2, a, dh, ln2, dy1, ok, dqkv, ln1):
                 tail = [(dy2[rr], a[rr], wg(e.fc2w)), (dh[rr], ln2[rr], e.fc1w.grad), (dy1[rr], ok[rr], wg(e.projw))]
+                lv1, lv2 = _live_steps(steps1, at, r0), _live_steps(steps2, at, r0)
                 if kr is None:
-                    ops.gemm_wgrad_batch(tail + [(dqkv[rr], ln1[rr], e.qkvw.grad)])
+                    ops.gemm_wgrad_batch(tail + [(dqkv[rr], ln1[rr], e.qkvw.grad)], live=[lv2, lv2, lv1, lv1])
                 else:
-                    ops.gemm_wgrad_batch(tail)
-                    _wgrad_rows(dqkv, ln1, [(q0, q1, eq.qkvw.grad) for q0, q1, eq in rg_all])
+                    ops.gemm_wgrad_batch(tail, live=[lv2, lv2, lv1])
+                    _wgrad_rows(dqkv, ln1, [(q0, q1, eq.qkvw.grad) for q0, q1, eq in rg_all], steps1, 0)
         else:
             with _Side(dqkv, ln1):
-                _wgrad_rows(dqkv, ln1, [(r0, r1, e.qkvw.grad) for r0, r1, e in rg_all])
+                _wgrad_rows(dqkv, ln1, [(r0, r1, e.qkvw.grad) for r0, r1, e in rg_all], steps1, 0)
         _gemm_rows(dqkv, [(r0, r1, wT16(e.qkvw), None, None) for r0, r1, e in rg_all], dln1, row_live=live_all)
         if kr is not None and kr.span is None:
             dx1 = kr.put(dx1, M_all, F32)
diff --git a/vl-merging_amd/ops.py b/vl-merging_amd/ops.py
--- a/vl-merging_amd/ops.py
+++ b/vl-merging_amd/ops.py
@@ -135,7 +135,20 @@
     return out
 
 
-def gemm_wgrad_grouped(dy, x, groups, accumulate=True):
+def _live_arg(live, rows, what):
+    if live is None:
+        return None, 0
+    mask, bit0 = live
+    L.require_cuda(mask)
+    if mask.dtype != torch.int64 or mask.dim() != 1 or not mask.is_contiguous() or bit0 < 0 or \
+            bit0 + -(-rows // 32) > 64 * mask.numel():
+        raise L.VlmError("%s: live mask int64 [words] covering bits %d .. %d" % (what, bit0, bit0 + -(-rows // 32)))
+    return mask.data_ptr(), int(bit0)
+
+
+def gemm_wgrad_grouped(dy, x, groups, accumulate=True, live=None):
+    if live is not None and len(live) != len(groups):
+        raise L.VlmError("gemm_wgrad_grouped: one live entry per group")
     L.require_cuda(dy, x)
     if dy.dtype != BF16 or x.dtype != BF16 or dy.shape[0] != x.shape[0]:
         raise L.VlmError("gemm_wgrad_grouped: bf16 dy [tokens, M] and x [tokens, N]")
@@ -151,6 +164,8 @@
         ldc = _ld(dW)
         prev = r1
         g.row0, g.rows, g.C, g.accumulate = r0, r1 - r0, dW.data_ptr(), int(bool(accumulate))
+    for g, lv in zip(arr, live or ()):
+        g.live, g.live_bit0 = _live_arg(lv, g.rows, "gemm_wgrad_grouped")
     ws = _scratch("splitk", SPLITK_WS_BYTES // 4, dy.device)
     rc = L.get_lib().vlm_gemm_wgrad_grouped(len(groups), arr, M, N, L.ptr(dy), _ld(dy), L.ptr(x), _ld(x), ldc, L.ptr(ws),
                                             ws.numel() * 4, L.stream_ptr())
@@ -163,8 +178,10 @@
             and sum(-(-M // 256) * (N // 256) for M, N in shapes) <= (cus if cus > 0 else 256))
 
 
-def gemm_wgrad_batch(problems, accumulate=True):
+def gemm_wgrad_batch(problems, accumulate=True, live=None):
     n = len(problems)
+    if live is not None and len(live) != n:
+        raise L.VlmError("gemm_wgrad_batch: one live entry per problem")
     if n < 1 or n > L.GEMM_MAX_GROUPS:
         raise L.VlmError("gemm_wgrad_batch: 1..%d problems" % L.GEMM_MAX_GROUPS)
     acc = [bool(accumulate)] * n if isinstance(accumulate, (bool, int)) else [bool(f) for f in accumulate]
@@ -182,6 +199,8 @@
         g.dy, g.ld_dy, g.M = dy.data_ptr(), _ld(dy), dy.shape[1]
         g.x, g.ld_x, g.N = x.data_ptr(), _ld(x), x.shape[1]
         g.dW, g.ldc, g.accumulate = dW.data_ptr(), _ld(dW), int(f)
+    for g, lv in zip(arr, live or ()):
+        g.live, g.live_bit0 = _live_arg(lv, T, "gemm_wgrad_batch")
     rc = 1
     if T >= 2048:
         ws = _scratch("splitk", SPLITK_WS_BYTES // 4, problems[0][0].device)
@@ -602,6 +621,16 @@
     L.check(L.get_lib().vlm_droppath_sites(L.ptr(u0), L.ptr(u1), L.ptr(keeps), S, seq.B, seq.n0, seq.n1, seq.base0, seq.base1,
                                            out.shape[1], L.ptr(out), L.stream_ptr()), "vlm_droppath_sites")
     return out
+
+
+def droppath_step_masks(table):
+    L.require_cuda(table)
+    if table.dtype != F32 or table.dim() != 2 or not table.is_contiguous():
+        raise L.VlmError("droppath_step_masks: contiguous f32 [S, rows] table")
+    S, rows = table.shape
+    masks = torch.empty(S, (-(-rows // 32) + 63) // 64, device=table.device, dtype=torch.int64)
+    L.check(L.get_lib().vlm_droppath_step_masks(L.ptr(table), S, rows, L.ptr(masks), L.stream_ptr()), "vlm_droppath_step_masks")
+    return masks
 
 
 def droppath_rows(u, keep, seq, out):
```

New measurement: 366.7 (median of 6 runs). No clear change (+0.2%).
